# panthuncia/BasicRenderer

Measured on AMD Instinct MI355X. Metric: shaded Mpixels/s @4K (vis-buffer+resolve), higher is better.
Workload: dtype f32; 1 GPU; bistro-class procedural frame, 3840x2160, 1 directional + 256 point lights, 22669824 instanced tris, 2017 instances (2614016 in 150 meshes), LOD DAGs from the library's cluster-LOD builder, relief slope 1.5; pixels_per_gpu=8294400, visible_clusters_rank0=10118, occlusion_culling=True, visible_clusters_phase2_rank0=0, meshlets_tested_rank0=26713, partition=single GPU, frames_in_flight=3

## Files before the change

basicrenderer_amd/capi.py:

```python
import ctypes as C
import os

_HERE = os.path.dirname(os.path.abspath(__file__))
LIB_DIR = os.path.join(_HERE, "lib")

u32, u64, f32, vp = C.c_uint32, C.c_uint64, C.c_float, C.c_void_p


class SceneParams(C.Structure):
    _fields_ = [("preset", u32), ("seed", u32), ("width", u32), ("height", u32), ("numPointLights", u32),
                ("withDirectionalLight", u32), ("lodLevels", u32), ("sizeScale", f32), ("skinnedFraction1024", u32),
                ("materialFeatures", u32), ("cameraStep", u32), ("lodBuilder", u32), ("spotLightEvery", u32), ("detail", f32), ("uniqueTriangleBudget", u32), ("reliefSlope", f32)]


class MeshInput(C.Structure):
    _fields_ = [("positions", vp), ("normals", vp), ("uvs", vp), ("colors", vp), ("vertexCount", C.c_size_t), ("indices", vp), ("indexCount", C.c_size_t),
                ("material", u32), ("reserved", u32 * 3)]


class InstanceInput(C.Structure):
    _fields_ = [("mesh", u32), ("reverseWinding", u32), ("model", (f32 * 4) * 4)]


class ViewInput(C.Structure):
# ... 39 lines not shown
        ("perMesh", vp), ("perMeshCount", u32),
        ("perMeshInstance", vp), ("perMeshInstanceCount", u32),
        ("clodOffsets", vp),
        ("meshMetadata", vp), ("meshMetadataCount", u32),
        ("lodNodes", vp), ("lodNodeCount", u32),
        ("lodGroups", vp), ("lodGroupCount", u32),
        ("lodSegments", vp), ("lodSegmentCount", u32),
        ("groupPageMap", vp), ("groupPageMapCount", u32),
        ("materials", vp), ("materialCount", u32),
        ("openpbrMaterials", vp), ("openpbrMaterialCount", u32),
        ("lights", vp), ("lightCount", u32),
        ("activeLightIndices", vp),
        ("cameras", vp), ("cameraCount", u32),
        ("cullingCameras", vp),
        ("viewRasterInfo", vp),
        ("perFrame", vp),
        ("activeDraws", vp), ("activeDrawCount", u32),
        ("skinningMatrices", vp), ("skinningMatrixCount", u32),
        ("lutOpaqueDielectricEnergyComplement", vp),
        ("lutOpaqueDielectricAvgEnergyComplement", vp),
        ("lutIdealMetalEnergyComplement", vp),
        ("lutIdealMetalAvgEnergyComplement", vp),
        ("lutFuzzLTC", vp),
        ("textures", vp), ("textureCount", u32),
        ("samplers", vp), ("samplerCount", u32),
        ("srgbToLinear", vp),
    ]


class Config(C.Structure):
    _fields_ = [("structSize", u32), ("width", u32), ("height", u32), ("maxVisibleClusters", u32),
                ("maxTraversalRecords", u32), ("enableOcclusionCulling", u32), ("enableClusteredLighting", u32),
                ("enablePunctualLights", u32), ("lightClusterSize", u32 * 3), ("phase2ExpansionFactor", u32),
                ("collectPassStatistics", u32), ("maxBvhLevels", u32), ("bandY0", u32), ("bandY1", u32),
                ("keepUniformLayerPlanes", u32), ("stripeRows", u32), ("stripeCount", u32), ("stripeIndex", u32), ("fullHeight", u32), ("dynamicBand", u32), ("reserved", u32 * 2)]


class ResourceDesc(C.Structure):
    _fields_ = [("id", u32), ("name", C.c_char_p), ("bytes", u64), ("usage", u32), ("width", u32), ("height", u32),
                ("bytesPerPixel", u32), ("tileW", u32), ("tileH", u32)]


class ResourceBinding(C.Structure):
    _fields_ = [("id", u32), ("ptr", vp), ("bytes", u64)]


class FrameUpdate(C.Structure):
    _fields_ = [("mainCameraHost", vp), ("perFrameHost", vp), ("frameIndex", u32)]


class Counters(C.Structure):
    _fields_ = [(n, u32) for n in ("instancesTested instancesVisible nodesVisited bucketRecords meshletsTested "
                                   "visibleClusters visibleClustersPhase2 droppedRecords droppedClusters "
                                   "lightPagesUsed replayNodes replayMeshlets").split()] + [("reserved", u32 * 6)]


class ComposeConfig(C.Structure):
    _fields_ = [("structSize", u32), ("width", u32), ("bandY0", u32), ("bandY1", u32), ("bytesPerPixel", u32), ("transport", u32), ("depth", u32),
                ("rank", u32), ("nRanks", u32), ("device", C.c_int32), ("path", u32), ("waitTimeoutMs", u32), ("frameHeight", u32), ("reserved", u32 * 3)]


COMPOSE_EXPORTS = ["brmi_compose_unique_id", "brmi_compose_create", "brmi_compose_staging_bytes", "brmi_compose_output_bytes", "brmi_compose_bind",
                   "brmi_compose_submit", "brmi_compose_finish", "brmi_compose_destroy", "brmi_compose_last_error",
                   "brmi_compose_alloc_shared", "brmi_compose_export", "brmi_compose_import", "brmi_compose_last_wait_status", "brmi_compose_submit_rows", "brmi_compose_wait_source", "brmi_compose_set_bounds", "brmi_compose_balance_rows"]
COMPOSE_HANDLE_BYTES = 160
_compose_lib = None


def compose_lib():
    global _compose_lib
    if _compose_lib is None:
        import torch
        path = os.path.join(LIB_DIR, "libbrmi_compose.so")
        if not os.path.exists(path):
            raise RuntimeError(f"{path} is missing: run `make compose` (or __graft_entry__.build())")
        try:
            C.CDLL(os.path.join(os.path.dirname(torch.__file__), "lib", "librccl.so"), mode=C.RTLD_GLOBAL)
        except OSError:
            pass
        lib = C.CDLL(path)
        lib.brmi_compose_unique_id.argtypes = [vp]
        lib.brmi_compose_create.argtypes = [C.POINTER(ComposeConfig), C.c_char_p, C.POINTER(vp)]
        lib.brmi_compose_staging_bytes.argtypes = [vp]
        lib.brmi_compose_staging_bytes.restype = u64
        lib.brmi_compose_output_bytes.argtypes = [vp]
        lib.brmi_compose_output_bytes.restype = u64
        lib.brmi_compose_bind.argtypes = [vp, vp, u64, vp, u64]
        lib.brmi_compose_submit.argtypes = [vp, vp, vp]
        lib.brmi_compose_finish.argtypes = [vp, vp, C.POINTER(vp)]
        lib.brmi_compose_destroy.argtypes = [vp]
        lib.brmi_compose_alloc_shared.argtypes = [vp]
        lib.brmi_compose_export.argtypes = [vp, C.c_char_p]
        lib.brmi_compose_import.argtypes = [vp, C.c_char_p, u32]
        lib.brmi_compose_last_wait_status.argtypes = [vp]
        lib.brmi_compose_submit_rows.argtypes = [vp, vp, u32, u32, vp]
        lib.brmi_compose_wait_source.argtypes = [vp, vp, vp]; lib.brmi_compose_wait_source.restype = C.c_int
        lib.brmi_compose_destroy.restype = None
        lib.brmi_compose_last_error.argtypes = [vp]
        lib.brmi_compose_last_error.restype = C.c_char_p
        _compose_lib = lib
    return _compose_lib


DECLARE_CB = C.CFUNCTYPE(None, vp, C.POINTER(ResourceDesc))

RES_NAMES = ["VISIBILITY", "LINEAR_DEPTH", "GBUF_NORMALS", "GBUF_ALBEDO", "GBUF_COAT", "GBUF_EMISSIVE", "GBUF_FUZZ",
             "GBUF_METALLIC_ROUGHNESS", "GBUF_MOTION_VECTORS", "HDR_COLOR", "VISIBLE_CLUSTERS", "LIGHT_CLUSTERS",
             "LIGHT_PAGES", "HZB", "WORKSPACE"]
RES = {n: i for i, n in enumerate(RES_NAMES)}
STAGE_NAMES = ["clear", "cull", "raster", "depth_copy", "hzb", "cull2", "raster2", "gbuffer", "light_cluster", "shade"]

_scene_lib = None
_brmi_lib = None


def scene_lib():
    global _scene_lib
    if _scene_lib is None:
        path = os.path.join(LIB_DIR, "libbrmi_scene.so")
        if not os.path.exists(path):
            raise RuntimeError(f"{path} is missing: run `make scene` (or __graft_entry__.build())")
        lib = C.CDLL(path)
        lib.brmi_scene_create.restype = vp
        lib.brmi_scene_create.argtypes = [C.POINTER(SceneParams)]
        lib.brmi_scene_create_with_dag_builder.restype = vp
        lib.brmi_scene_create_with_dag_builder.argtypes = [C.POINTER(SceneParams), vp, vp, vp]
        lib.brmi_scene_create_from_meshes.restype = vp
        lib.brmi_scene_create_from_meshes.argtypes = [C.POINTER(SceneParams), C.POINTER(MeshInput), u32, C.POINTER(InstanceInput), u32, C.POINTER(ViewInput), vp, vp, vp]
        lib.brmi_lod_build.argtypes = [vp, vp, C.c_size_t, vp, C.c_size_t, vp, C.POINTER(Dag)]
        lib.brmi_lod_release.argtypes = [vp, C.POINTER(Dag)]
        lib.brmi_lod_release.restype = None
        lib.brmi_scene_create_from_cache.restype = vp
        lib.brmi_scene_create_from_cache.argtypes = [C.POINTER(SceneParams), C.c_char_p]
        lib.brmi_scene_export_cache.argtypes = [vp, C.c_char_p]
        lib.brmi_scene_destroy.argtypes = [vp]
        lib.brmi_scene_array.argtypes = [vp, u32, C.POINTER(vp), C.POINTER(u64), C.POINTER(u32)]
        lib.brmi_scene_slab_count.argtypes = [vp]
        lib.brmi_scene_slab_count.restype = u32
        lib.brmi_scene_slab.argtypes = [vp, u32, C.POINTER(vp), C.POINTER(u64)]
        lib.brmi_scene_get_stats.argtypes = [vp, C.POINTER(SceneStats)]
        lib.brmi_scene_camera_at.argtypes = [C.POINTER(SceneParams), C.c_double, C.c_double, vp, vp]
        _scene_lib = lib
    return _scene_lib


BRMI_EXPORTS = ["brmi_abi_version", "brmi_default_config", "brmi_create", "brmi_declare", "brmi_set_scene", "brmi_setup", "brmi_set_band",
                "brmi_update", "brmi_execute", "brmi_execute_split", "brmi_destroy", "brmi_last_error", "brmi_clear_visibility", "brmi_cull",
                "brmi_raster", "brmi_depth_copy", "brmi_build_hzb", "brmi_invalidate_hzb", "brmi_set_history_source", "brmi_gbuffer", "brmi_light_clustering",
                "brmi_shade", "brmi_set_shade_slabs", "brmi_read_counters", "brmi_stage_times", "brmi_set_timed_stages", "brmi_algorithmic_bytes", "brmi_algorithmic_bytes_launched", "brmi_debug_arith", "brmi_debug_arith_in_range", "brmi_debug_read_bin_records", "brmi_debug_wide_triangles", "brmi_debug_lean_clusters", "brmi_debug_read_lean_queue", "brmi_debug_read_held"]


def brmi_lib():
    global _brmi_lib
    if _brmi_lib is None:
        import torch
        path = os.environ.get("BRMI_LIB_PATH") or os.path.join(LIB_DIR, "libbrmi.so")
        if not os.path.exists(path):
            raise RuntimeError(f"{path} is missing: the HIP extension must be built (make hip); there is no CPU fallback")
        lib = C.CDLL(path)
        lib.brmi_abi_version.restype = u32
        lib.brmi_default_config.argtypes = [C.POINTER(Config), u32, u32]
        lib.brmi_default_config.restype = None
        lib.brmi_create.argtypes = [C.POINTER(Config), C.POINTER(vp)]
        lib.brmi_declare.argtypes = [vp, DECLARE_CB, vp]
        lib.brmi_set_scene.argtypes = [vp, C.POINTER(SceneBuffers)]
        lib.brmi_setup.argtypes = [vp, C.POINTER(ResourceBinding), u32, vp]
        lib.brmi_update.argtypes = [vp, C.POINTER(FrameUpdate), vp]
        lib.brmi_execute.argtypes = [vp, vp]
        lib.brmi_execute_split.argtypes = [vp, vp, vp]
        lib.brmi_destroy.argtypes = [vp]
        lib.brmi_destroy.restype = None
        lib.brmi_last_error.argtypes = [vp]
        lib.brmi_last_error.restype = C.c_char_p
        for n in ("brmi_clear_visibility", "brmi_depth_copy", "brmi_build_hzb", "brmi_gbuffer", "brmi_light_clustering", "brmi_shade"):
            getattr(lib, n).argtypes = [vp, vp]
        lib.brmi_invalidate_hzb.argtypes = [vp]
        lib.brmi_set_history_source.argtypes = [vp, vp]
        lib.brmi_set_shade_slabs.argtypes = [vp, u32, vp, vp]
        lib.brmi_cull.argtypes = [vp, u32, vp]
        lib.brmi_raster.argtypes = [vp, u32, vp]
        lib.brmi_read_counters.argtypes = [vp, C.POINTER(Counters), vp]
        lib.brmi_stage_times.argtypes = [vp, C.POINTER(f32)]
        lib.brmi_set_timed_stages.argtypes = [vp, u32]
        lib.brmi_algorithmic_bytes.argtypes = [vp, C.POINTER(u64), C.POINTER(u64)]
        lib.brmi_algorithmic_bytes_launched.argtypes = [vp, C.POINTER(u64), C.POINTER(u64)]
        lib.brmi_debug_arith.argtypes = [vp, vp, vp, vp, vp, u32, vp]
        lib.brmi_debug_arith_in_range.argtypes = [vp, vp, vp, vp, u32, vp]
        _brmi_lib = lib
    return _brmi_lib
```

basicrenderer_amd/csrc/brmi_api.hip:

```cpp
#include <hip/hip_runtime.h>

#include <algorithm>
#include <cmath>
#include <cstdarg>
#include <cstdio>
#include <cstdlib>
#include <cstring>

#include "brmi_device.h"
#include "brmi_internal.h"

namespace brmi {

__global__ void k_debug_arith(const float* a, const float* b, float* outDiv, float* outSqrt, uint32_t* outHalf, uint32_t n) {
    const uint32_t i = blockIdx.x * blockDim.x + threadIdx.x;
    if (i >= n) return;
    outDiv[i] = a[i] / b[i];
    outSqrt[i] = sqrtf(fabsf(a[i]));
    outHalf[i] = f32_to_f16_bits(a[i]);
}

__global__ void k_debug_arith_in_range(const float* a, float* outRcp, float* outSqrt, float* outNorm, uint32_t n) {
    const uint32_t i = blockIdx.x * blockDim.x + threadIdx.x;
    if (i >= n) return;
// ... 14 lines not shown
static uint64_t align_up(uint64_t v, uint64_t a) { return (v + a - 1) / a * a; }

static const char* kResNames[BRMI_RES_COUNT] = {
    "Builtin::PrimaryCamera::VisibilityTexture", "Builtin::PrimaryCamera::LinearDepthMap", "Builtin::GBuffer::Normals", "Builtin::GBuffer::Albedo",
    "Builtin::GBuffer::Coat", "Builtin::GBuffer::Emissive", "Builtin::GBuffer::Fuzz", "Builtin::GBuffer::MetallicRoughness", "Builtin::GBuffer::MotionVectors",
    "Builtin::Color::HDRColorTarget", "Builtin::CLod::VisibleClusters", "Builtin::Light::ClusterBuffer", "Builtin::Light::PagesBuffer",
    "Builtin::PrimaryCamera::LinearDepthMap(mips)", "brmi::Workspace"};
static const uint32_t kResBpp[BRMI_RES_COUNT] = {8, 4, 16, 4, 8, 8, 8, 4, 4, 8, 0, 0, 0, 4, 0};

static void compute_sizes(brmi_pass* p) {
    const brmi_config& c = p->cfg;
    p->tilesX = (c.width + 7) / 8; p->tilesY = (c.height + 7) / 8;
    p->paddedPixels = (uint64_t)p->tilesX * p->tilesY * 64;
    p->bandY0 = c.bandY0; p->bandY1 = (c.bandY1 == 0 || c.bandY1 > c.height) ? c.height : c.bandY1;
    if (p->bandY0 >= p->bandY1) p->bandY0 = 0;
    p->stripes = c.stripeCount > 1u ? StripeMap{c.stripeRows, c.stripeCount, c.stripeIndex, c.fullHeight} : StripeMap{0u, 0u, 0u, c.height};
    { const uint32_t t0 = p->bandY0 / 8, t1 = (p->bandY1 + 7) / 8; p->bandFirstPixel = (uint64_t)t0 * p->tilesX * 64; p->bandPixelCount = (uint64_t)(t1 - t0) * p->tilesX * 64; }
    p->numLightClusters = c.lightClusterSize[0] * c.lightClusterSize[1] * c.lightClusterSize[2];
    p->lightPagePool = p->numLightClusters * BRMI_LIGHT_PAGES_PER_CLUSTER;
    if (const long v = tuning("light_page_pool", 0)) p->lightPagePool = (uint32_t)std::max(1l, v);
    for (int i = 0; i < BRMI_RES_COUNT; i++) p->resNeed[i] = 0;
    for (int i = BRMI_RES_VISIBILITY; i <= BRMI_RES_HDR_COLOR; i++) p->resNeed[i] = p->paddedPixels * kResBpp[i];
    p->resNeed[BRMI_RES_VISIBLE_CLUSTERS] = (uint64_t)c.maxVisibleClusters * 16;
    p->resNeed[BRMI_RES_LIGHT_CLUSTERS] = (uint64_t)p->numLightClusters * sizeof(brmi_light_cluster);
    p->resNeed[BRMI_RES_LIGHT_PAGES] = (uint64_t)p->lightPagePool * sizeof(brmi_light_page);
    p->hzbMipOffsets.clear(); p->hzbMipW.clear(); p->hzbMipH.clear();
    uint64_t hzbFloats = 0;
    if (c.enableOcclusionCulling) {
        uint32_t w = 1, h = 1; while (w < c.width) w <<= 1; while (h < c.height) h <<= 1;
        for (uint32_t mip = 0;; mip++) {
            p->hzbMipOffsets.push_back(hzbFloats); p->hzbMipW.push_back(w); p->hzbMipH.push_back(h);
            if (mip > 0) hzbFloats += (uint64_t)w * h;
            if (w == 1 && h == 1) break;
            w = std::max(1u, w >> 1); h = std::max(1u, h >> 1);
        }
    }
    p->hzbMipCount = (uint32_t)p->hzbMipOffsets.size();
    p->resNeed[BRMI_RES_HZB] = std::max<uint64_t>(16, hzbFloats * 4);
    Workspace& w = p->ws; uint64_t off = 0;
    auto take = [&](uint64_t bytes) { uint64_t o = off; off = align_up(off + bytes, 256); return o; };
    w.counters = take((uint64_t)(CNT_WORDS + 64) * 4);
    w.bitmask1 = take((uint64_t)p->totalWords * 4);
    w.bitmask2 = take((uint64_t)p->totalWords * 4);
    w.blockDirty = take((uint64_t)2 * (p->scanBlocks + 1));
    w.chainDirty = take(4ull + (uint64_t)((c.width + 31u) / 32u) * ((c.height + 31u) / 32u));
    w.frameClearBytes = off - w.counters;
    w.frontierA = take((uint64_t)c.maxTraversalRecords * sizeof(NodeRecord));
    w.frontierB = take((uint64_t)c.maxTraversalRecords * sizeof(NodeRecord));
    w.buckets = take((uint64_t)c.maxTraversalRecords * sizeof(BucketRecord));
    w.tempVisible = take((uint64_t)c.maxVisibleClusters * sizeof(TempVisible));
    w.wordPrefix = take((uint64_t)p->totalWords * 4);
    w.blockSums = take((uint64_t)(p->scanBlocks + 1) * 4);
    w.scanAgg = take(65 * 8);
    w.instanceBitBase = take((uint64_t)std::max<size_t>(1, p->hostInstanceBitBase.size()) * 4);
    w.segPrefix = take((uint64_t)std::max<size_t>(1, p->hostSegPrefix.size()) * 4);
    w.meshLevelWidth = take((uint64_t)std::max<size_t>(1, p->hostMeshLevelWidth.size()) * 4);
    w.flatNodes = take((uint64_t)std::max<size_t>(1, p->hostFlatNodes.size()) * sizeof(FlatNode));
    w.flatLeaves = take((uint64_t)std::max<size_t>(1, p->hostFlatLeaves.size()) * sizeof(FlatLeaf));
    w.instanceWalk = take((uint64_t)std::max<size_t>(1, p->hostInstanceWalk.size()) * sizeof(InstanceWalk));
    w.planes = take((uint64_t)2 * c.lightClusterSize[2] * 4);
    w.replayNodes = take(c.enableOcclusionCulling ? (uint64_t)c.maxTraversalRecords * sizeof(NodeRecord) : 16);
    w.replayBuckets = take(c.enableOcclusionCulling ? (uint64_t)c.maxTraversalRecords * sizeof(BucketRecord) : 16);
    w.lightVS = take((uint64_t)std::max(1u, p->scene.lightCount) * 16);
    w.lightMeta = take((uint64_t)std::max(1u, p->scene.lightCount) * 4);
    w.clusterPages = take((uint64_t)p->numLightClusters * 4);
    w.clusterHits = take((uint64_t)p->numLightClusters * 4);
    w.pageTotal = take(16);
    w.lightHitMasks = take((uint64_t)p->numLightClusters * ((std::max(1u, p->scene.lightCount) + 63u) / 64u) * 8);
    p->binsX = (c.width + 255) / 256; p->binsY = (c.height + 15) / 16;
    w.binCounts = take((uint64_t)p->binsX * p->binsY * 4 * BRMI_BIN_COUNT_STRIDE);
    w.binRecords = take((uint64_t)p->binsX * p->binsY * p->binCapacity * 64);
    w.binOverflow = take((uint64_t)CNT_STRIPE_COUNT * p->binOverflowPerStripe * 64);
    p->binItemCapacity = p->binsX * p->binsY * std::max(1u, (p->binCapacity + 31u) / 32u > 256u ? 256u : (p->binCapacity + 31u) / 32u);
    p->binItemCapacity = std::min<uint32_t>(p->binItemCapacity, 1u << 22);
    p->binScratchTiles = (uint32_t)std::max(0l, tuning("bin_scratch_tiles", p->binScratchTiles));
    w.binPlan = take((uint64_t)(16 + 3 * p->binsX * p->binsY) * 4);
    w.binItems = take((uint64_t)p->binItemCapacity * 4);
    w.binScratch = take((uint64_t)std::max(1u, p->binScratchTiles) * 4096 * 8);
    w.clusterSetup = take((uint64_t)c.maxVisibleClusters * sizeof(ClusterSetup));
    p->resolveCapacity = (uint32_t)std::min<uint64_t>((uint64_t)c.maxVisibleClusters, 1ull << 20) * BRMI_MESHLET_MAX_TRIS;
    if (const long v = tuning("resolve_capacity", 0)) p->resolveCapacity = (uint32_t)std::max(1l, v);
    w.resolveVerts = take((uint64_t)p->resolveCapacity * sizeof(ResolveVertex));
    w.resolveTris = take((uint64_t)p->resolveCapacity * sizeof(ResolveTriangle));
    w.shadeTables = take(((uint64_t)2 * c.width + 2 * c.height + 64) * 4);
    w.matWords = take((uint64_t)std::max(1u, p->scene.materialCount) * sizeof(MaterialWords));
    w.layerUniform = take(sizeof(LayerUniform));
    w.frameConst = take(4 * 64);
    w.frameSnapshot = take(sizeof(FrameSnapshot));
    w.matConst = take((uint64_t)std::max(1u, p->scene.openpbrMaterialCount) * sizeof(MatConst));
    w.objConst = take((uint64_t)std::max(1u, p->scene.perObjectCount) * OBJ_CONST_FLOATS * 4);
    p->deferredStripeCapacity = (uint32_t)((((c.dynamicBand ? p->paddedPixels : p->bandPixelCount) / 4096 + CNT_STRIPE_COUNT) / CNT_STRIPE_COUNT) * 4096);
    w.deferredPixels = take((uint64_t)3 * CNT_STRIPE_COUNT * p->deferredStripeCapacity * 4);
    w.lutF = take((uint64_t)(32768 + 1024 + 1024 + 32 + 256) * 4);
    w.shadeRows = take((uint64_t)std::max(1u, p->scene.openpbrMaterialCount) * 256 * 512);
    w.shadeAvgs = take((uint64_t)std::max(1u, p->scene.openpbrMaterialCount) * 256 * 8);
    w.ggxQuads = take(256 * 48);
    w.shadeLights = take((uint64_t)std::max(1u, p->scene.lightCount) * 64);
    w.clusterList = take((uint64_t)p->numLightClusters * 8);
    w.listEntries = take((uint64_t)p->lightPagePool * BRMI_LIGHTS_PER_PAGE * 4 + 256);
    w.listRecords = take((uint64_t)p->lightPagePool * BRMI_LIGHTS_PER_PAGE * 64 + 4096);
    const bool uvs = p->sceneHasTextures || p->sceneHasAlphaTest || p->sceneHasVertexColors;
    w.clusterUv = take(uvs ? (uint64_t)c.maxVisibleClusters * 32 : 16);
    w.resolveColors = take(p->sceneHasVertexColors ? (uint64_t)p->resolveCapacity * 4 : 16);
    w.resolveUVs = take(p->sceneHasTextures ? (uint64_t)p->resolveCapacity * 8 * p->sceneUvSets : 16);
    w.binAlpha = take(p->sceneHasAlphaTest ? (uint64_t)p->binsX * p->binsY * p->binCapacity * 48 : 16);
    w.overflowAlpha = take(p->sceneHasAlphaTest ? (uint64_t)CNT_STRIPE_COUNT * p->binOverflowPerStripe * 48 : 16);
// ... 44 lines not shown
    std::memset(cfg, 0, sizeof(*cfg));
    cfg->structSize = sizeof(brmi_config);
    cfg->width = width; cfg->height = height;
    cfg->maxVisibleClusters = 1u << 22;
    cfg->maxTraversalRecords = 1u << 22;
    cfg->enableOcclusionCulling = 0;
    cfg->enableClusteredLighting = 1;
    cfg->enablePunctualLights = 1;
    cfg->lightClusterSize[0] = 12; cfg->lightClusterSize[1] = 12; cfg->lightClusterSize[2] = 24;
    cfg->phase2ExpansionFactor = 2;
    cfg->collectPassStatistics = 0;
    cfg->maxBvhLevels = 64;
    cfg->keepUniformLayerPlanes = 0;
}

}
namespace brmi {
static bool tuning_lookup(const char* key, long* out) {
    const char* e = std::getenv("BRMI_TUNING");
    if (!e) return false;
    const size_t n = std::strlen(key);
    for (const char* q = e; *q; ) {
        while (*q == ',' || *q == ' ') q++;
        const char* end = std::strchr(q, ',');
        const size_t len = end ? (size_t)(end - q) : std::strlen(q);
        if (len > n && std::strncmp(q, key, n) == 0 && q[n] == '=') { *out = std::strtol(q + n + 1, nullptr, 0); return true; }
        q += len;
    }
    return false;
}
long tuning(const char* key, long def) { long v; return tuning_lookup(key, &v) ? v : def; }
}
extern "C" {

int brmi_create(const brmi_config* cfg, brmi_pass** out) {
    if (!cfg || !out || cfg->structSize != sizeof(brmi_config) || cfg->width == 0 || cfg->height == 0) return BRMI_ERR_INVALID;
    if (cfg->maxVisibleClusters == 0 || cfg->maxVisibleClusters > (1u << 25) - 1u || cfg->maxTraversalRecords == 0) return BRMI_ERR_INVALID;
    if (cfg->lightClusterSize[0] == 0 || cfg->lightClusterSize[1] == 0 || cfg->lightClusterSize[2] == 0) return BRMI_ERR_INVALID;
    if (cfg->lightClusterSize[2] > 62u) return BRMI_ERR_INVALID;
    if ((uint64_t)((cfg->width + 255u) / 256u) * ((cfg->height + 15u) / 16u) > 65535ull) return BRMI_ERR_INVALID;
    if (cfg->stripeCount > 1u) {
        if (cfg->stripeRows == 0u || cfg->stripeRows % 16u || cfg->stripeIndex >= cfg->stripeCount || cfg->bandY0 != 0u || (cfg->bandY1 != 0u && cfg->bandY1 != cfg->height)) return BRMI_ERR_INVALID;
        if (cfg->fullHeight == 0u || cfg->fullHeight % (cfg->stripeRows * cfg->stripeCount) || cfg->height != cfg->fullHeight / cfg->stripeCount) return BRMI_ERR_INVALID;
        if (cfg->dynamicBand) return BRMI_ERR_INVALID;
    }
    if (cfg->dynamicBand && (cfg->bandY0 % 8u || (cfg->bandY1 % 8u && cfg->bandY1 < cfg->height))) return BRMI_ERR_INVALID;
    brmi_pass* p = new brmi_pass();
    p->cfg = *cfg;
    p->totalWords = 1; p->scanBlocks = 1;
    p->forceLevelKernels = tuning("cull_level_kernels", 0) != 0;
    p->packedFlat = tuning("flat_packed", 1) != 0;
    p->flatLevelsMinDraws = (uint32_t)std::max(0l, tuning("flat_levels_min_draws", p->flatLevelsMinDraws));
    p->phase2DirectMax = (uint32_t)std::max(0l, tuning("phase2_direct_max", p->phase2DirectMax));
    p->resolveInlineMode = (int)tuning("resolve_inline", -1);
    p->wideCapacity = (uint32_t)std::min(1l << 20, std::max(0l, tuning("wide_capacity", p->wideCapacity)));
    p->wideMinTriangles = (uint32_t)std::max(0l, tuning("wide_min_triangles", p->wideMinTriangles));
    p->leanMinClusters = (uint32_t)std::max(0l, tuning("lean_min_clusters", p->leanMinClusters));
    if (p->leanMinClusters > cfg->maxVisibleClusters) p->leanMinClusters = 0u;
    p->leanMaxGeneralPct = (uint32_t)std::max(0l, std::min(100l, tuning("lean_max_general_pct", p->leanMaxGeneralPct)));
    p->leanGrid = (uint32_t)std::max(64l, tuning("lean_grid", p->leanGrid));
    p->leanQueue = (uint32_t)std::max(64l, std::min(1l << 24, tuning("lean_queue", p->leanQueue))) & ~63u;
    p->leanWideEntries = (uint32_t)std::max(1l, tuning("lean_wide_entries", p->leanWideEntries));
    p->leanEmitGrid = (uint32_t)std::max(64l, std::min(65536l, tuning("lean_emit_grid", p->leanEmitGrid))) & ~63u;
    p->wideEntries = (uint32_t)std::max(1l, tuning("wide_entries", p->wideEntries));
    p->binMinSlice = (uint32_t)std::max(32l, tuning("bin_min_slice", p->binMinSlice));
    p->binSharedSlice = (uint32_t)std::max(32l, tuning("bin_shared_slice", p->binSharedSlice));
    p->binGrid = (uint32_t)std::min(65535l, std::max(1l, tuning("bin_grid", p->binGrid)));
    p->binOverflowPerStripe = (uint32_t)std::max(0l, tuning("bin_overflow", p->binOverflowPerStripe));
    p->binCapacity = (uint32_t)std::min(65536l, std::max(1l, tuning("bin_capacity", p->binCapacity)));
    if (const long v = tuning("big_tri_area", 0)) p->bigTriArea = p->bigTriAreaAlpha = p->bigTriAreaDense = (int)std::max(1l, v);
    compute_sizes(p);
    *out = p;
    return BRMI_OK;
}

void brmi_destroy(brmi_pass* p) {
    if (!p) return;
    if (p->eventsCreated) for (int i = 0; i < BRMI_STAGE_COUNT; i++) for (uint32_t k = 0; k < brmi_pass::kEventRing; k++) { (void)hipEventDestroy(p->evStart[i][k]); (void)hipEventDestroy(p->evStop[i][k]); }
    (void)brmi_set_history_source(p, nullptr);
    for (brmi_pass* user : p->historyUsers) user->history = nullptr;
    if (p->chainReady) (void)hipEventDestroy(p->chainReady);
    if (p->geometryDone) (void)hipEventDestroy(p->geometryDone);
    if (p->cullDone) (void)hipEventDestroy(p->cullDone);
    if (p->frameDone) (void)hipEventDestroy(p->frameDone);
    if (p->phase2FeedbackHost) (void)hipHostFree(p->phase2FeedbackHost);
    delete p;
}

const char* brmi_last_error(const brmi_pass* p) { return p ? p->err.c_str() : "null pass"; }

int brmi_set_scene(brmi_pass* p, const brmi_scene_buffers* scene) {
    if (!p || !scene) return BRMI_ERR_INVALID;
    p->scene = *scene; p->haveScene = false; p->setupDone = false;
    const brmi_scene_buffers& sc = p->scene;
    if (!sc.slabs || !sc.perObject || !sc.perMesh || !sc.perMeshInstance || !sc.clodOffsets || !sc.meshMetadata || !sc.lodNodes || !sc.lodGroups ||
        !sc.lodSegments || !sc.groupPageMap || !sc.materials || !sc.openpbrMaterials || !sc.cameras || !sc.cullingCameras || !sc.viewRasterInfo || !sc.perFrame ||
        !sc.normalMatrices || (sc.activeDrawCount && !sc.activeDraws) || (sc.lightCount && (!sc.lights || !sc.activeLightIndices)))
        return fail(p, BRMI_ERR_INVALID, "brmi_set_scene: a required scene buffer is null");
    if (!sc.lutOpaqueDielectricEnergyComplement || !sc.lutOpaqueDielectricAvgEnergyComplement || !sc.lutIdealMetalEnergyComplement || !sc.lutIdealMetalAvgEnergyComplement || !sc.lutFuzzLTC)
        return fail(p, BRMI_ERR_INVALID, "brmi_set_scene: OpenPBR lookup tables must be provided");
    std::vector<brmi_clod_mesh_metadata> md; std::vector<brmi_mesh_instance_clod_offsets> offs; std::vector<brmi_lod_node> nodes; std::vector<brmi_lod_segment> segs;
    int rc;
    if ((rc = read_back(p, md, sc.meshMetadata, sc.meshMetadataCount))) return rc;
    if ((rc = read_back(p, offs, sc.clodOffsets, sc.perMeshInstanceCount))) return rc;
    if ((rc = read_back(p, nodes, sc.lodNodes, sc.lodNodeCount))) return rc;
    if ((rc = read_back(p, segs, sc.lodSegments, sc.lodSegmentCount))) return rc;
// ... 486 lines not shown
        BRMI_HIP(p, hipEventRecord(p->chainReady, static_cast<hipStream_t>(stream)));
        p->chainRecorded = true; p->chainStream = stream;
    }
    if (split) {
        if ((rc = launch_resolve_setup(p, static_cast<hipStream_t>(stream), 2u))) return rc;
        p->resolveSetupDone = true;
        if (!p->geometryDone) BRMI_HIP(p, hipEventCreateWithFlags(&p->geometryDone, hipEventDisableTiming));
        if (!p->frameDone) BRMI_HIP(p, hipEventCreateWithFlags(&p->frameDone, hipEventDisableTiming));
        BRMI_HIP(p, hipEventRecord(p->geometryDone, static_cast<hipStream_t>(stream)));
        BRMI_HIP(p, hipStreamWaitEvent(static_cast<hipStream_t>(shadeStream), p->geometryDone, 0));
        stream = shadeStream;
    }
    const bool lightsDone = p->lightGridDone;
    p->lightGridDone = false;
    p->depthFinal = p->cfg.enableOcclusionCulling != 0;
    p->shadeSharesChip = split;
    rc = brmi_gbuffer(p, stream);
    p->shadeSharesChip = false;
    p->depthFinal = false;
    if (rc) return rc;
    if (!lightsDone && (rc = brmi_light_clustering(p, stream))) return rc;
    p->shadeSharesChip = split;
    rc = brmi_shade(p, stream);
    p->shadeSharesChip = false;
    if (rc) return rc;
    if (split) { BRMI_HIP(p, hipEventRecord(p->frameDone, static_cast<hipStream_t>(stream))); p->frameDoneRecorded = true; }
    p->splitFrame = false;
    return BRMI_OK;
}

int brmi_read_counters(brmi_pass* p, brmi_counters* out, brmi_stream stream) {
    if (!p || !out) return BRMI_ERR_INVALID;
    if (!p->setupDone) return brmi::fail(p, BRMI_ERR_STATE, "brmi_read_counters: setup not done");
    hipStream_t s = static_cast<hipStream_t>(stream);
    uint32_t c[CNT_WORDS];
    BRMI_HIP(p, hipMemcpyAsync(c, p->counters(), sizeof(c), hipMemcpyDeviceToHost, s));
    BRMI_HIP(p, hipStreamSynchronize(s));
    std::memset(out, 0, sizeof(*out));
    out->instancesTested = c[CNT_INSTANCES_TESTED]; out->instancesVisible = c[CNT_INSTANCES_VISIBLE];
    out->nodesVisited = c[CNT_NODES_VISITED];
    uint32_t overflowQueued = 0;
    for (uint32_t st = 0; st < CNT_STRIPE_COUNT; st++) {
        const uint32_t* sp = c + CNT_STRIPES + st * CNT_STRIPE_WORDS;
        out->instancesTested += sp[0]; out->instancesVisible += sp[1]; out->nodesVisited += sp[2];
        overflowQueued += sp[STRIPE_OVERFLOW];
    } out->bucketRecords = c[CNT_BUCKETS]; out->meshletsTested = c[CNT_MESHLETS_TESTED];
    for (uint32_t st = 0; st < CNT_STRIPE_COUNT; st++) out->meshletsTested += c[CNT_STRIPES + st * CNT_STRIPE_WORDS + STRIPE_MESHLETS_TESTED];
    out->visibleClusters = c[CNT_VISIBLE]; out->visibleClustersPhase2 = c[CNT_VISIBLE2];
    out->droppedRecords = c[CNT_DROPPED_RECORDS]; out->droppedClusters = c[CNT_DROPPED_CLUSTERS]; out->lightPagesUsed = c[CNT_LIGHT_PAGES];
    out->reserved[0] = c[CNT_SUM_VERTS_LO]; out->reserved[2] = c[CNT_SUM_VERTS_HI];
    out->reserved[1] = std::min(c[CNT_HELD1], p->cfg.maxVisibleClusters); out->reserved[3] = std::min(c[CNT_LATE1], p->cfg.maxVisibleClusters);
    out->reserved[4] = c[CNT_RASTER_CLUSTERS]; out->reserved[5] = c[CNT_BIN_OVERFLOW] + overflowQueued;
    out->replayNodes = c[CNT_REPLAY_NODES]; out->replayMeshlets = c[CNT_REPLAY_MESHLETS];
    return BRMI_OK;
}

int brmi_set_timed_stages(brmi_pass* p, uint32_t stageMask) {
    if (!p) return BRMI_ERR_INVALID;
    p->timedStages = stageMask;
    return BRMI_OK;
}

int brmi_stage_times(brmi_pass* p, float* ms) {
    if (!p || !ms) return BRMI_ERR_INVALID;
    if (!p->eventsCreated) return brmi::fail(p, BRMI_ERR_STATE, "brmi_stage_times: collectPassStatistics is off");
    for (int i = 0; i < BRMI_STAGE_COUNT; i++) {
        ms[i] = 0.0f;
        const uint32_t perFrame = (i == BRMI_STAGE_HZB && p->executesSinceTimes != 0u && p->evCount[i] == 2u * p->executesSinceTimes) ? 2u : 1u;
        uint32_t n = std::min(p->evCount[i], brmi_pass::kEventRing);
        n -= n % perFrame;
        if (n == 0) continue;
        double sum = 0.0;
        for (uint32_t k = 0; k < n; k++) {
            const uint32_t slot = (p->evCount[i] - 1 - k) % brmi_pass::kEventRing;
            float t = 0.0f;
            BRMI_HIP(p, hipEventSynchronize(p->evStop[i][slot]));
            BRMI_HIP(p, hipEventElapsedTime(&t, p->evStart[i][slot], p->evStop[i][slot]));
            sum += t;
        }
        ms[i] = (float)(sum / (n / perFrame));
        p->evCount[i] = 0;
    }
    p->executesSinceTimes = 0;
    return BRMI_OK;
}

int brmi_algorithmic_bytes(brmi_pass* p, uint64_t* perStage, uint64_t* total) {
    if (!p || !perStage || !total) return BRMI_ERR_INVALID;
    BRMI_HIP(p, hipDeviceSynchronize());
    brmi_counters c; int rc = brmi_read_counters(p, &c, nullptr); if (rc) return rc;
    const uint64_t P = (uint64_t)p->cfg.width * (p->bandY1 - p->bandY0);
    uint64_t sumV = c.reserved[0], sumT = c.reserved[2], nClusters = c.reserved[4];
    if (c.reserved[1] != 0u) {
        uint32_t vt[2];
        BRMI_HIP(p, hipMemcpy(vt, p->counters() + CNT_DRAWN_VT, 8, hipMemcpyDeviceToHost));
        sumV = vt[0]; sumT = vt[1]; nClusters -= c.reserved[1] - c.reserved[3];
    }
    for (int i = 0; i < BRMI_STAGE_COUNT; i++) perStage[i] = 0;
    perStage[BRMI_STAGE_CLEAR] = 8 * P;
    perStage[BRMI_STAGE_CULL] = 64ull * c.meshletsTested + 16ull * (c.visibleClusters + c.visibleClustersPhase2) + 64ull * c.nodesVisited;
    perStage[BRMI_STAGE_RASTER] = 8 * P + 144ull * nClusters + 12ull * sumV + 3ull * sumT;
    if (p->cfg.enableOcclusionCulling) {
        perStage[BRMI_STAGE_DEPTH_COPY] = 12 * P;
        perStage[BRMI_STAGE_HZB] = 2 * (4 * P + 4 * P / 3);
    }
    perStage[BRMI_STAGE_GBUFFER] = (8 + 52 + 4) * P;
// ... 1 lines not shown
    *total = 0; for (int i = 0; i < BRMI_STAGE_COUNT; i++) *total += perStage[i];
    return BRMI_OK;
}

int brmi_algorithmic_bytes_launched(brmi_pass* p, uint64_t* perStage, uint64_t* total) {
    if (int rc = brmi_algorithmic_bytes(p, perStage, total)) return rc;
    if (!p->sceneHasCoat && !p->sceneHasFuzz) {
        const uint64_t P = (uint64_t)p->cfg.width * (p->bandY1 - p->bandY0);
        *total -= perStage[BRMI_STAGE_SHADE]; perStage[BRMI_STAGE_SHADE] = 44ull * P; *total += perStage[BRMI_STAGE_SHADE];
    }
    return BRMI_OK;
}

int brmi_debug_read_held(brmi_pass* p, uint32_t* held, uint32_t heldCapacity, uint32_t* heldCount, uint32_t* late, uint32_t lateCapacity, uint32_t* lateCount) {
    if (!p || !heldCount || !lateCount || !p->setupDone) return BRMI_ERR_INVALID;
    BRMI_HIP(p, hipDeviceSynchronize());
    uint32_t nh = 0, nl = 0;
    BRMI_HIP(p, hipMemcpy(&nh, p->counters() + CNT_HELD1, 4, hipMemcpyDeviceToHost));
    BRMI_HIP(p, hipMemcpy(&nl, p->counters() + CNT_LATE1, 4, hipMemcpyDeviceToHost));
    if (!p->holdEnabled) nh = nl = 0;
    nh = std::min(nh, p->cfg.maxVisibleClusters); nl = std::min(nl, p->cfg.maxVisibleClusters);
    *heldCount = nh; *lateCount = nl;
    if (held && nh) {
        std::vector<HeldRecord> rec(std::min(nh, heldCapacity));
        if (!rec.empty()) BRMI_HIP(p, hipMemcpy(rec.data(), p->wsPtr<HeldRecord>(p->ws.heldRecords), rec.size() * sizeof(HeldRecord), hipMemcpyDeviceToHost));
        for (size_t i = 0; i < rec.size(); i++) held[i] = rec[i].clusterIndex;
    }
    if (late && nl && lateCapacity) BRMI_HIP(p, hipMemcpy(late, p->wsPtr<uint32_t>(p->ws.lateList), (size_t)std::min(nl, lateCapacity) * 4, hipMemcpyDeviceToHost));
    return BRMI_OK;
}

int brmi_debug_wide_triangles(brmi_pass* p, uint32_t out[3]) {
    if (!p || !out || !p->setupDone) return BRMI_ERR_INVALID;
    BRMI_HIP(p, hipDeviceSynchronize());
    uint32_t c[3] = {0u, 0u, 0u};
    BRMI_HIP(p, hipMemcpy(&c[0], p->counters() + CNT_WIDE1, 4, hipMemcpyDeviceToHost));
    BRMI_HIP(p, hipMemcpy(&c[1], p->counters() + CNT_WIDE1B, 4, hipMemcpyDeviceToHost));
    BRMI_HIP(p, hipMemcpy(&c[2], p->counters() + CNT_WIDE2, 4, hipMemcpyDeviceToHost));
    out[0] = c[0]; out[1] = c[1]; out[2] = c[2];
    return BRMI_OK;
}

int brmi_debug_lean_clusters(brmi_pass* p, uint32_t out[4]) {
    if (!p || !out || !p->setupDone) return BRMI_ERR_INVALID;
    BRMI_HIP(p, hipDeviceSynchronize());
    uint32_t c = 0u, heads[64 * 32];
    BRMI_HIP(p, hipMemcpy(&c, p->counters() + CNT_GENERAL1, 4, hipMemcpyDeviceToHost));
    BRMI_HIP(p, hipMemcpy(heads, p->counters() + CNT_BIG1, sizeof(heads), hipMemcpyDeviceToHost));
    out[0] = p->leanLastLaunch ? 1u : 0u; out[1] = c; out[2] = out[3] = 0u;
    for (uint32_t s = 0; s < 64u; s++) { out[2] += heads[s * 32u]; out[3] += heads[s * 32u + 1u]; }
    return BRMI_OK;
}

int brmi_debug_read_lean_queue(brmi_pass* p, uint32_t stripe, uint32_t* runs, uint32_t maxRuns, void* entries, uint32_t maxEntries, uint32_t counts[2]) {
    if (!p || !counts || !p->setupDone || stripe >= 64u || p->leanMinClusters == 0u) return BRMI_ERR_INVALID;
    BRMI_HIP(p, hipDeviceSynchronize());
    uint32_t head[2];
    BRMI_HIP(p, hipMemcpy(head, p->counters() + CNT_BIG1 + stripe * 32u, 8, hipMemcpyDeviceToHost));
    const uint32_t cap = p->leanQueue / 64u;
    counts[0] = std::min(head[0], cap); counts[1] = std::min(head[1], cap);
    if (runs) BRMI_HIP(p, hipMemcpy(runs, p->wsPtr<uint8_t>(p->ws.bigRuns) + (size_t)stripe * cap * 8u, (size_t)std::min(maxRuns, counts[1]) * 8u, hipMemcpyDeviceToHost));
    if (entries) BRMI_HIP(p, hipMemcpy(entries, p->wsPtr<uint8_t>(p->ws.bigQueue) + (size_t)stripe * cap * 96u, (size_t)std::min(maxEntries, counts[0]) * 96u, hipMemcpyDeviceToHost));
    return BRMI_OK;
}

int brmi_debug_read_bin_records(brmi_pass* p, void* dst, uint64_t bytes) {
    if (!p || !dst || !p->setupDone) return BRMI_ERR_INVALID;
    BRMI_HIP(p, hipDeviceSynchronize());
    if ((bytes >> 62) & 1ull) { bytes &= ~(1ull << 62); BRMI_HIP(p, hipMemset(p->wsPtr<uint8_t>(p->ws.binRecords), 0, bytes)); return BRMI_OK; }
    BRMI_HIP(p, hipMemcpy(dst, p->wsPtr<uint8_t>(p->ws.binRecords), bytes, hipMemcpyDeviceToHost));
    return BRMI_OK;
}

int brmi_debug_arith(const float* a, const float* b, float* outDiv, float* outSqrt, uint32_t* outHalfBits, uint32_t n, brmi_stream stream) {
    if (!a || !b || !outDiv || !outSqrt || !outHalfBits) return BRMI_ERR_INVALID;
    if (n == 0) return BRMI_OK;
    hipLaunchKernelGGL(k_debug_arith, dim3((n + 255) / 256), dim3(256), 0, static_cast<hipStream_t>(stream), a, b, outDiv, outSqrt, outHalfBits, n);
    return hipGetLastError() == hipSuccess ? BRMI_OK : BRMI_ERR_HIP;
}

int brmi_debug_arith_in_range(const float* a, float* outRcp, float* outSqrt, float* outRsqrt, uint32_t n, brmi_stream stream) {
    if (!a || !outRcp || !outSqrt || !outRsqrt) return BRMI_ERR_INVALID;
    if (n == 0) return BRMI_OK;
    hipLaunchKernelGGL(k_debug_arith_in_range, dim3((n + 255) / 256), dim3(256), 0, static_cast<hipStream_t>(stream), a, outRcp, outSqrt, outRsqrt, n);
    return hipGetLastError() == hipSuccess ? BRMI_OK : BRMI_ERR_HIP;
}

}
```

basicrenderer_amd/csrc/brmi_cull.hip:

```cpp
#include <type_traits>
#include "brmi_device.h"
#include "brmi_internal.h"
#include "brmi_lightgrid.h"
#include "brmi_texture.h"

namespace brmi {

struct CullArgs {
    brmi_scene_buffers sc;
    uint32_t* counters;
    const uint32_t* instanceBitBase;
    const uint32_t* segPrefix;
    uint32_t recordCapacity, visibleCapacity, factor, phase;
    uint32_t occlusion;
    uint32_t frontier0Counter, bucketCounter;
    NodeRecord* replayNodes; BucketRecord* replayBuckets;
    HzbDesc hzb;
    uint32_t bandActive; float bandTop[3], bandBottom[3];
    const float4* bandPlanes;
    StripeMap stripes;
    const uint32_t* meshLevelWidth; uint32_t levelKernelsWidthLo;
    const FlatNode* flatNodes; const FlatLeaf* flatLeaves; const InstanceWalk* instanceWalk;
    uint32_t* feedback;
    uint32_t wideFlat;
// ... 243 lines not shown
#pragma unroll
            for (int o = 32; o > 0; o >>= 1) waveMax = max(waveMax, (uint32_t)__shfl_xor((int)waveMax, o));
            for (uint32_t k = 0; k < waveMax; k++) {
                const bool emit = k < nChunks;
                const uint32_t slot = wave_append(&a.counters[a.bucketCounter], emit);
                if (emit) {
                    if (slot < a.recordCapacity) {
                        const uint32_t first = segFirst + k * a.factor;
                        const uint32_t cnt = min(a.factor, segCount - k * a.factor);
                        BucketRecord b;
                        b.instanceIndex = instIndex; b.groupIdPacked = (replay ? 0x80000000u : 0u) | (ownerGroup & 0x7FFFFFFFu);
                        b.meshletIndexAndCount = (cnt << 16) | (first & 0xFFFFu);
                        b.pageSlabDescriptorIndex = slabDesc; b.pageSlabByteOffset = slabOff;
                        b.firstBit = firstBit + k * a.factor; b.pad0 = 0; b.pad1 = 0;
                        buckets[slot] = b;
                    } else atomicAdd(&a.counters[CNT_DROPPED_RECORDS], 1u);
                }
            }
        }
        {
            uint32_t waveMax = isInternal ? childCount : 0u;
#pragma unroll
            for (int o = 32; o > 0; o >>= 1) waveMax = max(waveMax, (uint32_t)__shfl_xor((int)waveMax, o));
            for (uint32_t k = 0; k < waveMax; k++) {
                bool emit = false;
                uint32_t childId = 0;
                if (isInternal && k < childCount) {
                    childId = childBase + k;
                    const brmi_lod_node* ch = sc.lodNodes + (lodNodesBase + childId);
                    const f3 cc = skinned ? instC : f3{ch->cullCenterAndRadius[0], ch->cullCenterAndRadius[1], ch->cullCenterAndRadius[2]};
                    const float cr = skinned ? instR : ch->cullCenterAndRadius[3];
                    const f3 ccVS = to_view_space(cc, model, view);
                    emit = replay || !sphere_culled(a, cam, ccVS, cr * scale);
                    if (emit && ch->isLeaf == BRMI_NODE_INTERNAL) {
                        const f3 wc = xyz(mul_point(f3{ch->lodCenterAndRadius[0], ch->lodCenterAndRadius[1], ch->lodCenterAndRadius[2]}, model));
                        const float e = projected_error(wc, ch->lodCenterAndRadius[3] * scale, ch->maxQuadricError, scale, camPos, zNear, ortho);
                        if (e < threshold) emit = false;
                    }
                }
                const uint32_t slot = wave_append(nextCount, emit);
                if (emit) {
                    if (slot < a.recordCapacity) frontierOut[slot] = NodeRecord{instIndex, (replay ? 0x80000000u : 0u) | (1u << 30) | (childId & 0x3FFFFFFFu)};
                    else atomicAdd(&a.counters[CNT_DROPPED_RECORDS], 1u);
                }
            }
        }
    }
}

#ifndef BRMI_HIER_STAGE_WIDE
#define BRMI_HIER_STAGE_WIDE 128
#endif
constexpr uint32_t HIER_CAP_MAX = 1024;
struct NoSide {};
struct SideJobs { ulonglong2* vis2; uint64_t n2; uint32_t walkBlocks, clearBlocks; ClusterArgs lc; };
template <bool REPLAY, uint32_t HIER_CAP, uint32_t HIER_STAGE, bool SIDE = false>
__global__ void __launch_bounds__(64) k_cull_hierarchy(CullArgs a, BucketRecord* buckets, const uint32_t* meshLevelWidth, uint32_t widthLo, uint32_t widthHi, uint32_t spillAbove, NodeRecord* spillOut,
                                                    typename std::conditional<SIDE, SideJobs, NoSide>::type sj) {
    uint32_t walkBlocks = gridDim.x;
    if constexpr (SIDE) {
        walkBlocks = sj.walkBlocks;
        if (blockIdx.x >= sj.walkBlocks + sj.clearBlocks) { lc_count_wave(sj.lc, blockIdx.x - sj.walkBlocks - sj.clearBlocks, threadIdx.x); return; }
        if (blockIdx.x >= sj.walkBlocks) {
            const uint64_t stride = (uint64_t)sj.clearBlocks * 64u;
            for (uint64_t i = (uint64_t)(blockIdx.x - sj.walkBlocks) * 64u + threadIdx.x; i < sj.n2; i += stride) sj.vis2[i] = make_ulonglong2(BRMI_VIS_EMPTY, BRMI_VIS_EMPTY);
            return;
        }
    }
    __shared__ uint32_t frontier[2][HIER_CAP];
    __shared__ uint32_t counts[2];
    __shared__ uint32_t childOff[65], childFirst[64];
    __shared__ BucketRecord stage[HIER_STAGE];
    const brmi_scene_buffers& sc = a.sc;
    const uint32_t lane = threadIdx.x;
    const uint32_t viewId = sc.perFrame->mainCameraIndex;
    const brmi_camera* cam = sc.cameras + viewId;
    const brmi_culling_camera* lodCam = sc.cullingCameras + viewId;
    const bool ortho = cam->isOrtho != 0;
    const f3 camPos{lodCam->positionWorldSpace[0], lodCam->positionWorldSpace[1], lodCam->positionWorldSpace[2]};
    const float zNear = lodCam->zNear, threshold = lodCam->errorOverDistanceThreshold;
    const m4 view = load_m4(&cam->view[0][0]);
    const uint32_t seeds = REPLAY ? min(a.counters[CNT_REPLAY_NODES], a.recordCapacity) : sc.activeDrawCount;
    uint32_t nTested = 0, nVisible = 0, nNodes = 0;
    uint32_t staged = 0;
    auto flush = [&]() {
        if (staged == 0u) return;
        uint32_t baseSlot = 0;
        if (lane == 0) baseSlot = atomicAdd(&a.counters[a.bucketCounter], staged);
        baseSlot = (uint32_t)__shfl((int)baseSlot, 0);
        __syncthreads();
        for (uint32_t k = lane; k < staged; k += 64u) {
            if (baseSlot + k < a.recordCapacity) buckets[baseSlot + k] = stage[k];
            else atomicAdd(&a.counters[CNT_DROPPED_RECORDS], 1u);
        }
        __syncthreads();
        staged = 0u;
    };
    uint32_t firstSeed = blockIdx.x, seedStride = walkBlocks;
    if (!REPLAY && a.packedFlat) {
        const uint32_t packedWaves = (seeds + 7u) >> 3;
        if (blockIdx.x < packedWaves) {
            const uint32_t g8 = lane & ~7u, j = lane & 7u;
            const uint32_t seed = blockIdx.x * 8u + (lane >> 3);
            const bool haveSeed = seed < seeds;
            const uint32_t instIndex = haveSeed ? sc.activeDraws[seed] : 0u;
            brmi_per_mesh_instance inst{}; InstanceWalk iw{0u, 0u, 0u, 0u};
            if (haveSeed) { inst = sc.perMeshInstance[instIndex]; iw = a.instanceWalk[instIndex]; }
            const bool small = haveSeed && iw.flatCount >= 1u && iw.flatCount <= 8u;
            const brmi_per_object* obj = sc.perObject + (small ? inst.perObjectBufferIndex : 0u);
            const bool mine = small && j < iw.flatCount;
            FlatNode fn{}; FlatLeaf fl{};
            if (mine) { fn = a.flatNodes[iw.flatBase + j]; fl = a.flatLeaves[iw.flatBase + j]; }
            m4 model = load_m4(&obj->model[0][0]);
            m4 prevModel = model;
            if (a.occlusion && mine && ((fn.info & 1u))) prevModel = load_m4(&obj->prevModel[0][0]);
            const float scale = max_axis_scale(model);
            const f3 instC{inst.boundingSphere[0], inst.boundingSphere[1], inst.boundingSphere[2]}; const float instR = inst.boundingSphere[3];
            bool instVisible = false;
            {
                const f3 c = to_view_space(instC, model, view);
                const float r = instR * scale;
                const bool bad = isnan(c.x) || isnan(c.y) || isnan(c.z) || isinf(c.x) || isinf(c.y) || isinf(c.z) || isnan(r) || isinf(r);
                instVisible = small && !bad && !sphere_culled(a, cam, c, r);
            }
            nTested += (uint32_t)__popcll(__ballot(small && j == 0u)); nVisible += (uint32_t)__popcll(__ballot(instVisible && j == 0u));
            const bool skinned = iw.skinned != 0u;
            const bool internal = (fn.info & 1u);
            const f3 cullC = skinned ? instC : f3{fn.cull[0], fn.cull[1], fn.cull[2]};
            const float cullR = skinned ? instR : fn.cull[3];
            const f3 cVS = to_view_space(cullC, model, view);
            const float rW = cullR * scale;
            const bool inFrustum = mine && instVisible && !sphere_culled(a, cam, cVS, rW);
            bool pre = inFrustum, expand = false, hidden = false, leafOk = false;
            uint32_t slabDesc = 0, slabOff = 0;
            if (inFrustum && internal) {
                const f3 lc = xyz(mul_point(f3{fn.lod[0], fn.lod[1], fn.lod[2]}, model));
                const float e = projected_error(lc, fn.lod[3] * scale, fn.maxQuadricError, scale, camPos, zNear, ortho);
                pre = e >= threshold;
                if (pre) { hidden = a.occlusion && occlusion_test_prev(a, cam, cullC, cullR, prevModel); expand = !hidden; }
            } else if (inFrustum) {
                const f3 gc = xyz(mul_point(f3{fl.group[0], fl.group[1], fl.group[2]}, model));
                const float eod = projected_error(gc, fl.group[3] * scale, fn.maxQuadricError, scale, camPos, zNear, ortho);
                bool ok = eod >= threshold;
                if (ok && ((fn.info >> 1) & 1u)) {
                    const f3 cc = xyz(mul_point(f3{fl.child[0], fl.child[1], fl.child[2]}, model));
                    const float ce = projected_error(cc, fl.child[3] * scale, fl.childParentError, scale, camPos, zNear, ortho);
                    if (!(ce < threshold)) ok = false;
                }
                if (ok && ((fn.info >> 2) & 1u)) {
                    const brmi_group_page_map_entry pe = sc.groupPageMap[fn.pageMapIndex];
                    slabDesc = pe.slabDescriptorIndex; slabOff = pe.slabByteOffset;
                    leafOk = slabDesc != 0u;
                }
            }
            const uint64_t expandM = __ballot(expand);
            const uint32_t parentLane = g8 | ((fn.info >> 8) & 7u);
            uint64_t reached = __ballot(mine && instVisible && j == 0u);
            for (;;) {
                const bool r = mine && instVisible && (j == 0u || (pre && ((reached >> parentLane) & 1ull) && ((expandM >> parentLane) & 1ull)));
                const uint64_t next = __ballot(r);
                if (next == reached) break;
                reached = next;
            }
            const bool here = (reached >> lane) & 1ull;
            nNodes += here ? 1u : 0u;
            const bool replayIt = a.occlusion && here && hidden;
            const uint64_t replayM = __ballot(replayIt);
            const bool emitLeaf = here && leafOk;
            const uint32_t segFirst = fn.segFirstCount & 0xFFFFu, segCount = fn.segFirstCount >> 16;
            const uint32_t nChunks = emitLeaf ? (segCount + a.factor - 1u) / a.factor : 0u;
            uint32_t incl = nChunks;
#pragma unroll
            for (int o = 1; o < 64; o <<= 1) { const uint32_t v = (uint32_t)__shfl_up((int)incl, o); if (lane >= (uint32_t)o) incl += v; }
            const uint32_t nBuckets = (uint32_t)__shfl((int)incl, 63), nReplay = (uint32_t)__popcll(replayM);
            uint32_t replayBase = 0, bucketBase = 0;
            if (lane == 0) {
                if (nReplay != 0u) replayBase = atomicAdd(&a.counters[CNT_REPLAY_NODES], nReplay);
                if (nBuckets != 0u) bucketBase = atomicAdd(&a.counters[a.bucketCounter], nBuckets);
            }
            replayBase = (uint32_t)__shfl((int)replayBase, 0); bucketBase = (uint32_t)__shfl((int)bucketBase, 0);
            if (replayIt) {
                const uint32_t slot = replayBase + (uint32_t)__popcll(replayM & ((1ull << lane) - 1ull));
                if (slot < a.recordCapacity) a.replayNodes[slot] = NodeRecord{instIndex, 0x80000000u | (1u << 30) | (fn.nodeId & 0x3FFFFFFFu)};
                else atomicAdd(&a.counters[CNT_DROPPED_RECORDS], 1u);
            }
            for (uint32_t k = 0; k < nChunks; k++) {
                const uint32_t slot = bucketBase + (incl - nChunks) + k;
                if (slot >= a.recordCapacity) { atomicAdd(&a.counters[CNT_DROPPED_RECORDS], 1u); continue; }
                BucketRecord b;
                b.instanceIndex = instIndex; b.groupIdPacked = fn.ownerGroup & 0x7FFFFFFFu;
                b.meshletIndexAndCount = (min(a.factor, segCount - k * a.factor) << 16) | ((segFirst + k * a.factor) & 0xFFFFu);
                b.pageSlabDescriptorIndex = slabDesc; b.pageSlabByteOffset = slabOff;
                b.firstBit = iw.bitBase + fn.firstBitRel + k * a.factor; b.pad0 = 0; b.pad1 = 0;
                buckets[slot] = b;
            }
            firstSeed = seeds;
        } else { firstSeed = blockIdx.x - packedWaves; seedStride = walkBlocks - packedWaves; }
    }
    for (uint32_t seed = firstSeed; seed < seeds; seed += seedStride) {
        uint32_t instIndex, startNode;
        if (REPLAY) { const NodeRecord rec = a.replayNodes[seed]; instIndex = rec.instanceIndex; startNode = rec.nodeIdPacked & 0x3FFFFFFFu; }
        else instIndex = sc.activeDraws[seed];
        const brmi_per_mesh_instance inst = sc.perMeshInstance[instIndex];
        if (!REPLAY) {
            const InstanceWalk iw = a.instanceWalk[instIndex];
            if (a.packedFlat && iw.flatCount >= 1u && iw.flatCount <= 8u) continue;
            if (iw.flatCount > 256u && a.wideFlat) continue;
            if (iw.flatCount != 0u && iw.flatCount <= 256u) {
                constexpr uint32_t FLAT_CHUNKS = 4;
                const uint32_t chunks = (iw.flatCount + 63u) >> 6;
                const brmi_per_object* obj = sc.perObject + inst.perObjectBufferIndex;
                uint32_t nodeIdA[FLAT_CHUNKS] = {}, parentA[FLAT_CHUNKS] = {}, ownerGroupA[FLAT_CHUNKS] = {}, segFirstCountA[FLAT_CHUNKS] = {}, firstBitRelA[FLAT_CHUNKS] = {};
                const m4 model = load_m4(&obj->model[0][0]);
                const m4 prevModel = a.occlusion ? load_m4(&obj->prevModel[0][0]) : model;
                const float scale = max_axis_scale(model);
                const f3 instC{inst.boundingSphere[0], inst.boundingSphere[1], inst.boundingSphere[2]}; const float instR = inst.boundingSphere[3];
                {
                    const f3 c = to_view_space(instC, model, view);
                    const float r = instR * scale;
                    const bool bad = isnan(c.x) || isnan(c.y) || isnan(c.z) || isinf(c.x) || isinf(c.y) || isinf(c.z) || isnan(r) || isinf(r);
                    nTested++;
                    if (bad || sphere_culled(a, cam, c, r)) continue;
                    nVisible++;
                }
                const bool skinned = iw.skinned != 0u;
                uint64_t preM[FLAT_CHUNKS] = {}, expandM[FLAT_CHUNKS] = {}, hiddenM[FLAT_CHUNKS] = {}, leafM[FLAT_CHUNKS] = {}, reached[FLAT_CHUNKS] = {};
                uint32_t slabDescA[FLAT_CHUNKS] = {}, slabOffA[FLAT_CHUNKS] = {};
#pragma unroll
                for (uint32_t c = 0; c < FLAT_CHUNKS; c++) if (c < chunks) {
                    const bool mine = c * 64u + lane < iw.flatCount;
                    FlatNode fn{}; FlatLeaf fl{};
                    if (mine) { fn = a.flatNodes[iw.flatBase + c * 64u + lane]; fl = a.flatLeaves[iw.flatBase + c * 64u + lane]; }
                    nodeIdA[c] = fn.nodeId; parentA[c] = fn.info >> 8; ownerGroupA[c] = fn.ownerGroup; segFirstCountA[c] = fn.segFirstCount; firstBitRelA[c] = fn.firstBitRel;
                    const bool internal = (fn.info & 1u);
                    const f3 cullC = skinned ? instC : f3{fn.cull[0], fn.cull[1], fn.cull[2]};
                    const float cullR = skinned ? instR : fn.cull[3];
                    const f3 cVS = to_view_space(cullC, model, view);
                    const float rW = cullR * scale;
                    const bool inFrustum = mine && !sphere_culled(a, cam, cVS, rW);
                    bool pre = inFrustum, expand = false, hidden = false, leafOk = false;
                    if (inFrustum && internal) {
                        const f3 lc = xyz(mul_point(f3{fn.lod[0], fn.lod[1], fn.lod[2]}, model));
                        const float e = projected_error(lc, fn.lod[3] * scale, fn.maxQuadricError, scale, camPos, zNear, ortho);
                        pre = e >= threshold;
                        if (pre) { hidden = a.occlusion && occlusion_test_prev(a, cam, cullC, cullR, prevModel); expand = !hidden; }
                    } else if (inFrustum) {
                        const f3 gc = xyz(mul_point(f3{fl.group[0], fl.group[1], fl.group[2]}, model));
                        const float eod = projected_error(gc, fl.group[3] * scale, fn.maxQuadricError, scale, camPos, zNear, ortho);
                        bool ok = eod >= threshold;
                        if (ok && ((fn.info >> 1) & 1u)) {
// ... 40 lines not shown
                    for (int o = 1; o < 64; o <<= 1) { const uint32_t v = (uint32_t)__shfl_up((int)incl, o); if (lane >= (uint32_t)o) incl += v; }
                    bucketRank[c] = nBuckets + incl - chunksOfLeaf[c];
                    nBuckets += (uint32_t)__shfl((int)incl, 63);
                }
                uint32_t replayBase = 0, bucketBase = 0;
                if (lane == 0) {
                    if (nReplay != 0u) replayBase = atomicAdd(&a.counters[CNT_REPLAY_NODES], nReplay);
                    if (nBuckets != 0u) bucketBase = atomicAdd(&a.counters[a.bucketCounter], nBuckets);
                }
                replayBase = (uint32_t)__shfl((int)replayBase, 0); bucketBase = (uint32_t)__shfl((int)bucketBase, 0);
#pragma unroll
                for (uint32_t c = 0; c < FLAT_CHUNKS; c++) if (c < chunks) {
                    if (a.occlusion && ((reached[c] & hiddenM[c]) >> lane) & 1ull) {
                        const uint32_t slot = replayBase + replayRank[c];
                        if (slot < a.recordCapacity) a.replayNodes[slot] = NodeRecord{instIndex, 0x80000000u | (1u << 30) | (nodeIdA[c] & 0x3FFFFFFFu)};
                        else atomicAdd(&a.counters[CNT_DROPPED_RECORDS], 1u);
                    }
                    const uint32_t segFirst = segFirstCountA[c] & 0xFFFFu, segCount = segFirstCountA[c] >> 16;
                    for (uint32_t k = 0; k < chunksOfLeaf[c]; k++) {
                        const uint32_t slot = bucketBase + bucketRank[c] + k;
                        if (slot >= a.recordCapacity) { atomicAdd(&a.counters[CNT_DROPPED_RECORDS], 1u); continue; }
                        BucketRecord b;
                        b.instanceIndex = instIndex; b.groupIdPacked = ownerGroupA[c] & 0x7FFFFFFFu;
                        b.meshletIndexAndCount = (min(a.factor, segCount - k * a.factor) << 16) | ((segFirst + k * a.factor) & 0xFFFFu);
                        b.pageSlabDescriptorIndex = slabDescA[c]; b.pageSlabByteOffset = slabOffA[c];
                        b.firstBit = iw.bitBase + firstBitRelA[c] + k * a.factor; b.pad0 = 0; b.pad1 = 0;
                        buckets[slot] = b;
                    }
                }
                continue;
            }
        }
        const uint32_t mdIndex = sc.clodOffsets[instIndex].clodMeshMetadataIndex;
        const uint32_t width = meshLevelWidth[mdIndex];
        if (width < widthLo || width > widthHi) continue;
        const bool spill = width > spillAbove;
        const brmi_clod_mesh_metadata md = sc.meshMetadata[mdIndex];
        const brmi_per_object* obj = sc.perObject + inst.perObjectBufferIndex;
        const m4 model = load_m4(&obj->model[0][0]);
        const float scale = max_axis_scale(model);
        const f3 instC{inst.boundingSphere[0], inst.boundingSphere[1], inst.boundingSphere[2]}; const float instR = inst.boundingSphere[3];
        if (!REPLAY) {
            const f3 c = to_view_space(instC, model, view);
            const float r = instR * scale;
            const bool bad = isnan(c.x) || isnan(c.y) || isnan(c.z) || isinf(c.x) || isinf(c.y) || isinf(c.z) || isnan(r) || isinf(r);
            const bool visible = !bad && !sphere_culled(a, cam, c, r);
            nTested++;
            if (!visible) continue;
            nVisible++;
            startNode = md.rootNode;
        }
        const bool skinned = (sc.perMesh[inst.perMeshBufferIndex].vertexFlags & BRMI_VERTEX_SKINNED) != 0;
        const uint32_t bitBase = a.instanceBitBase[instIndex];
        __syncthreads();
        if (lane == 0) { frontier[0][0] = startNode; counts[0] = 1u; counts[1] = 0u; }
        __syncthreads();
        for (uint32_t level = 0; level < 64u; level++) {
            const uint32_t cur = level & 1u, nxt = cur ^ 1u;
            const uint32_t n = min(counts[cur], HIER_CAP);
            if (n == 0u) break;
            if (spill && n > HIER_CAP / BRMI_BVH_MAX_CHILDREN) {
                uint32_t baseSlot = 0;
                if (lane == 0) baseSlot = atomicAdd(&a.counters[CNT_FRONTIER0], n);
                baseSlot = (uint32_t)__shfl((int)baseSlot, 0);
                for (uint32_t k = lane; k < n; k += 64u) {
                    if (baseSlot + k < a.recordCapacity) spillOut[baseSlot + k] = NodeRecord{instIndex, (REPLAY ? 0x80000000u : 0u) | (1u << 30) | (frontier[cur][k] & 0x3FFFFFFFu)};
                    else atomicAdd(&a.counters[CNT_DROPPED_RECORDS], 1u);
                }
                break;
            }
            for (uint32_t base = 0; base < n; base += 64u) {
                const bool have = base + lane < n;
                bool isInternal = false, emitLeaf = false, occluded = false;
                uint32_t nodeId = 0, childBase = 0, childCount = 0, segFirst = 0, segCount = 0, ownerGroup = 0, slabDesc = 0, slabOff = 0, firstBit = 0;
                if (have) {
                    nodeId = frontier[cur][base + lane];
                    nNodes++;
                    const brmi_lod_node node = sc.lodNodes[md.lodNodesBase + nodeId];
                    const f3 cullC = skinned ? instC : f3{node.cullCenterAndRadius[0], node.cullCenterAndRadius[1], node.cullCenterAndRadius[2]};
                    const float cullR = skinned ? instR : node.cullCenterAndRadius[3];
                    const f3 cVS = to_view_space(cullC, model, view);
                    const float rW = cullR * scale;
                    const bool culled = !REPLAY && sphere_culled(a, cam, cVS, rW);
                    if (!culled) {
                        if (node.isLeaf != BRMI_NODE_INTERNAL) {
                            const brmi_lod_group* g = sc.lodGroups + (md.groupsBase + node.ownerGroupId);
                            const f3 gc = xyz(mul_point(f3{g->centerAndRadius[0], g->centerAndRadius[1], g->centerAndRadius[2]}, model));
                            const float gr = g->centerAndRadius[3] * scale;
                            const float eod = projected_error(gc, gr, node.maxQuadricError, scale, camPos, zNear, ortho);
                            bool ok = eod >= threshold;
                            if (ok && refined_child_suppresses(sc, md.groupsBase, node.countMinusOne - 1u, node.countMinusOne != 0u, model, scale, camPos, zNear, threshold, ortho)) ok = false;
                            if (ok) {
                                const brmi_lod_segment seg = sc.lodSegments[md.segmentsBase + node.indexOrOffset];
                                const brmi_group_page_map_entry pe = sc.groupPageMap[md.pageMapBase + seg.pageIndex];
                                if (seg.meshletCount != 0u && pe.slabDescriptorIndex != 0u) {
                                    emitLeaf = true;
                                    segFirst = seg.firstMeshletInPage; segCount = seg.meshletCount; ownerGroup = node.ownerGroupId;
                                    slabDesc = pe.slabDescriptorIndex; slabOff = pe.slabByteOffset;
                                    firstBit = bitBase + a.segPrefix[md.segmentsBase + node.indexOrOffset];
                                }
                            }
                        } else {
                            const f3 lc = xyz(mul_point(f3{node.lodCenterAndRadius[0], node.lodCenterAndRadius[1], node.lodCenterAndRadius[2]}, model));
                            const float lr = node.lodCenterAndRadius[3] * scale;
                            const float nodeEod = projected_error(lc, lr, node.maxQuadricError, scale, camPos, zNear, ortho);
                            if (nodeEod >= threshold) {
                                if (a.occlusion && occlusion_test(a, cam, REPLAY, cullC, cullR, cVS, rW, obj)) occluded = !REPLAY;
                                else { isInternal = true; childBase = node.indexOrOffset; childCount = min(node.countMinusOne + 1u, BRMI_BVH_MAX_CHILDREN); }
                            }
// ... 7 lines not shown
                        else atomicAdd(&a.counters[CNT_DROPPED_RECORDS], 1u);
                    }
                }
                {
                    const uint32_t nChunks = emitLeaf ? (segCount + a.factor - 1u) / a.factor : 0u;
                    uint32_t incl = nChunks;
#pragma unroll
                    for (int o = 1; o < 64; o <<= 1) { const uint32_t v = (uint32_t)__shfl_up((int)incl, o); if (lane >= (uint32_t)o) incl += v; }
                    const uint32_t total = (uint32_t)__shfl((int)incl, 63);
                    if (total != 0u) {
                        if (staged + total > HIER_STAGE) flush();
                        if (total <= HIER_STAGE) {
                            const uint32_t baseSlot = staged + (incl - nChunks);
                            for (uint32_t k = 0; k < nChunks; k++) {
                                const uint32_t first = segFirst + k * a.factor;
                                const uint32_t cnt = min(a.factor, segCount - k * a.factor);
                                BucketRecord b;
                                b.instanceIndex = instIndex; b.groupIdPacked = (REPLAY ? 0x80000000u : 0u) | (ownerGroup & 0x7FFFFFFFu);
                                b.meshletIndexAndCount = (cnt << 16) | (first & 0xFFFFu);
                                b.pageSlabDescriptorIndex = slabDesc; b.pageSlabByteOffset = slabOff;
                                b.firstBit = firstBit + k * a.factor; b.pad0 = 0; b.pad1 = 0;
                                stage[baseSlot + k] = b;
                            }
                            staged += total;
                        } else {
                            uint32_t baseSlot = 0;
                            if (lane == 0) baseSlot = atomicAdd(&a.counters[a.bucketCounter], total);
                            baseSlot = (uint32_t)__shfl((int)baseSlot, 0) + (incl - nChunks);
                            for (uint32_t k = 0; k < nChunks; k++) {
                                const uint32_t slot = baseSlot + k;
                                if (slot < a.recordCapacity) {
                                    const uint32_t first = segFirst + k * a.factor;
                                    const uint32_t cnt = min(a.factor, segCount - k * a.factor);
                                    BucketRecord b;
                                    b.instanceIndex = instIndex; b.groupIdPacked = (REPLAY ? 0x80000000u : 0u) | (ownerGroup & 0x7FFFFFFFu);
                                    b.meshletIndexAndCount = (cnt << 16) | (first & 0xFFFFu);
                                    b.pageSlabDescriptorIndex = slabDesc; b.pageSlabByteOffset = slabOff;
                                    b.firstBit = firstBit + k * a.factor; b.pad0 = 0; b.pad1 = 0;
                                    buckets[slot] = b;
                                } else atomicAdd(&a.counters[CNT_DROPPED_RECORDS], 1u);
                            }
                        }
                    }
                }
                {
                    const uint32_t myChildren = isInternal ? childCount : 0u;
                    uint32_t incl = myChildren;
#pragma unroll
                    for (int o = 1; o < 64; o <<= 1) { const uint32_t v = (uint32_t)__shfl_up((int)incl, o); if (lane >= (uint32_t)o) incl += v; }
                    const uint32_t total = (uint32_t)__shfl((int)incl, 63);
                    if (total != 0u) {
                        childOff[lane] = incl - myChildren; childFirst[lane] = childBase;
                        if (lane == 63) childOff[64] = total;
                        __syncthreads();
                        for (uint32_t task = lane; task < ((total + 63u) & ~63u); task += 64u) {
                            bool emit = false;
                            uint32_t childId = 0;
                            if (task < total) {
                                uint32_t parent = 0;
#pragma unroll
                                for (uint32_t step = 32; step > 0; step >>= 1) if (childOff[parent + step] <= task) parent += step;
                                childId = childFirst[parent] + (task - childOff[parent]);
                                const brmi_lod_node* ch = sc.lodNodes + (md.lodNodesBase + childId);
                                const f3 cc = skinned ? instC : f3{ch->cullCenterAndRadius[0], ch->cullCenterAndRadius[1], ch->cullCenterAndRadius[2]};
                                const float cr = skinned ? instR : ch->cullCenterAndRadius[3];
                                const f3 ccVS = to_view_space(cc, model, view);
                                emit = REPLAY || !sphere_culled(a, cam, ccVS, cr * scale);
                                if (emit && ch->isLeaf == BRMI_NODE_INTERNAL) {
                                    const f3 wc = xyz(mul_point(f3{ch->lodCenterAndRadius[0], ch->lodCenterAndRadius[1], ch->lodCenterAndRadius[2]}, model));
                                    const float e = projected_error(wc, ch->lodCenterAndRadius[3] * scale, ch->maxQuadricError, scale, camPos, zNear, ortho);
                                    if (e < threshold) emit = false;
                                }
                            }
                            const uint32_t slot = wave_append(&counts[nxt], emit);
                            if (emit) {
                                if (slot < HIER_CAP) frontier[nxt][slot] = childId;
                                else atomicAdd(&a.counters[CNT_DROPPED_RECORDS], 1u);
                            }
                        }
                        __syncthreads();
                    }
                }
            }
            __syncthreads();
            if (lane == 0) counts[cur] = 0u;
            __syncthreads();
        }
    }
    flush();
#pragma unroll
    for (int o = 32; o > 0; o >>= 1) nNodes += (uint32_t)__shfl_xor((int)nNodes, o);
    if (lane == 0) {
        uint32_t* stripe = a.counters + CNT_STRIPES + (blockIdx.x & (CNT_STRIPE_COUNT - 1u)) * CNT_STRIPE_WORDS;
        if (nTested) atomicAdd(&stripe[0], nTested);
        if (nVisible) atomicAdd(&stripe[1], nVisible);
        if (nNodes) atomicAdd(&stripe[2], nNodes);
    }
}

constexpr uint32_t FLAT_WIDE_MAX = 8192;
__global__ void __launch_bounds__(1024) k_cull_flat_wide(CullArgs a, BucketRecord* buckets) {
    __shared__ uint8_t verdict[FLAT_WIDE_MAX];
    __shared__ uint16_t parentOf[FLAT_WIDE_MAX], recordsOf[FLAT_WIDE_MAX];
    __shared__ uint32_t waveSum[2][16], changed, bases[2];
    const brmi_scene_buffers& sc = a.sc;
    const uint32_t t = threadIdx.x, lane = t & 63u, wave = t >> 6;
    const uint32_t viewId = sc.perFrame->mainCameraIndex;
    const brmi_camera* cam = sc.cameras + viewId;
    const brmi_culling_camera* lodCam = sc.cullingCameras + viewId;
    const bool ortho = cam->isOrtho != 0;
    const f3 camPos{lodCam->positionWorldSpace[0], lodCam->positionWorldSpace[1], lodCam->positionWorldSpace[2]};
    const float zNear = lodCam->zNear, threshold = lodCam->errorOverDistanceThreshold;
    const m4 view = load_m4(&cam->view[0][0]);
    uint32_t nTested = 0, nVisible = 0, nNodes = 0;
    for (uint32_t seed = blockIdx.x; seed < sc.activeDrawCount; seed += gridDim.x) {
        const uint32_t instIndex = sc.activeDraws[seed];
        const InstanceWalk iw = a.instanceWalk[instIndex];
        if (iw.flatCount <= 256u || iw.flatCount > FLAT_WIDE_MAX) continue;
        const brmi_per_mesh_instance inst = sc.perMeshInstance[instIndex];
        const brmi_per_object* obj = sc.perObject + inst.perObjectBufferIndex;
        const m4 model = load_m4(&obj->model[0][0]);
        const m4 prevModel = a.occlusion ? load_m4(&obj->prevModel[0][0]) : model;
        const float scale = max_axis_scale(model);
        const f3 instC{inst.boundingSphere[0], inst.boundingSphere[1], inst.boundingSphere[2]}; const float instR = inst.boundingSphere[3];
        {
            const f3 c = to_view_space(instC, model, view);
            const float r = instR * scale;
            const bool bad = isnan(c.x) || isnan(c.y) || isnan(c.z) || isinf(c.x) || isinf(c.y) || isinf(c.z) || isnan(r) || isinf(r);
            if (t == 0) nTested++;
            if (bad || sphere_culled(a, cam, c, r)) continue;
            if (t == 0) nVisible++;
        }
        const bool skinned = iw.skinned != 0u;
        __syncthreads();
        for (uint32_t node = t; node < iw.flatCount; node += 1024u) {
            const FlatNode fn = a.flatNodes[iw.flatBase + node];
            const bool internal = (fn.info & 1u);
            const f3 cullC = skinned ? instC : f3{fn.cull[0], fn.cull[1], fn.cull[2]};
            const float cullR = skinned ? instR : fn.cull[3];
            const f3 cVS = to_view_space(cullC, model, view);
            const float rW = cullR * scale;
            const bool inFrustum = !sphere_culled(a, cam, cVS, rW);
            bool pre = inFrustum, expand = false, hidden = false, leafOk = false;
            uint32_t records = 0;
            if (inFrustum && internal) {
                const f3 lc = xyz(mul_point(f3{fn.lod[0], fn.lod[1], fn.lod[2]}, model));
                const float e = projected_error(lc, fn.lod[3] * scale, fn.maxQuadricError, scale, camPos, zNear, ortho);
                pre = e >= threshold;
                if (pre) { hidden = a.occlusion && occlusion_test_prev(a, cam, cullC, cullR, prevModel); expand = !hidden; }
            } else if (inFrustum) {
// ... 197 lines not shown
        if (nChunks != 0u) {
            const uint32_t segFirst = fn.segFirstCount & 0xFFFFu, segCount = fn.segFirstCount >> 16;
            for (uint32_t k = 0; k < nChunks; k++, slot[1]++) {
                if (slot[1] >= a.recordCapacity) { atomicAdd(&a.counters[CNT_DROPPED_RECORDS], 1u); continue; }
                BucketRecord b;
                b.instanceIndex = instIndex; b.groupIdPacked = fn.ownerGroup & 0x7FFFFFFFu;
                b.meshletIndexAndCount = (min(a.factor, segCount - k * a.factor) << 16) | ((segFirst + k * a.factor) & 0xFFFFu);
                b.pageSlabDescriptorIndex = slabDesc; b.pageSlabByteOffset = slabOff;
                b.firstBit = iw.bitBase + fn.firstBitRel + k * a.factor; b.pad0 = 0; b.pad1 = 0;
                buckets[slot[1]] = b;
            }
        }
        if (hidden) {
            if (slot[2] < a.recordCapacity) a.replayNodes[slot[2]] = NodeRecord{instIndex, 0x80000000u | (1u << 30) | (fn.nodeId & 0x3FFFFFFFu)};
            else atomicAdd(&a.counters[CNT_DROPPED_RECORDS], 1u);
        }
    }
#pragma unroll
    for (int o = 32; o > 0; o >>= 1) { nNodes += (uint32_t)__shfl_xor((int)nNodes, o); nTested += (uint32_t)__shfl_xor((int)nTested, o); nVisible += (uint32_t)__shfl_xor((int)nVisible, o); }
    if (lane == 0) {
        uint32_t* stripe = a.counters + CNT_STRIPES + ((blockIdx.x * 4u + wave) & (CNT_STRIPE_COUNT - 1u)) * CNT_STRIPE_WORDS;
        if (nTested) atomicAdd(&stripe[0], nTested);
        if (nVisible) atomicAdd(&stripe[1], nVisible);
        if (nNodes) atomicAdd(&stripe[2], nNodes);
    }
}

BRMI_DEV float4 skinned_meshlet_bounds(const brmi_scene_buffers& sc, const brmi_meshlet_descriptor* desc, const brmi_page_header* hdr, const uint8_t* page, uint32_t slot, float4 staticBounds) {
    const uint32_t boneCount = desc->boneCount;
    if (slot == 0xFFFFFFFFu || boneCount == 0u || sc.skinningMatrices == nullptr) return staticBounds;
    const uint32_t* boneList = reinterpret_cast<const uint32_t*>(page + hdr->boneIndexStreamOffset + desc->boneListOffset * 4u);
    const f3 c0{staticBounds.x, staticBounds.y, staticBounds.z};
    f3 mc{0.0f, 0.0f, 0.0f}; float mr = 0.0f; bool init = false;
    for (uint32_t b = 0; b < boneCount; b++) {
        const m4 m = load_bone_skin_matrix(sc.skinningMatrices, slot, boneList[b]);
        const f3 tc = xyz(mul_point(c0, m));
        const float tr = staticBounds.w * max_axis_scale(m);
        if (!init) { mc = tc; mr = tr; init = true; continue; }
        const f3 delta = tc - mc;
        const float dist = length3(delta);
        if (dist + tr <= mr) continue;
        if (dist + mr <= tr) { mc = tc; mr = tr; continue; }
        const float newRadius = 0.5f * (dist + mr + tr);
        const float t = (newRadius - mr) / max2(dist, 1e-12f);
        mc = mc + delta * t;
        mr = newRadius;
    }
    if (!init) return staticBounds;
    return make_float4(mc.x, mc.y, mc.z, mr * (1.0f + 1e-5f));
}

struct LcRide { uint32_t mainBlocks; ClusterArgs lc; };
struct ClearRide { uint32_t mainBlocks; ulonglong2* vis2; uint64_t n2; uint32_t clearBlocks; };
template <int SIDE>
__global__ void __launch_bounds__(256) k_cull_clusters(CullArgs a, const BucketRecord* buckets, TempVisible* temp, uint32_t* bitmask, uint8_t* blockDirty,
                                                       typename std::conditional<SIDE == 1, LcRide, typename std::conditional<SIDE == 2, ClearRide, NoSide>::type>::type ride) {
    uint32_t mainBlocks = gridDim.x;
    if constexpr (SIDE == 1) {
        mainBlocks = ride.mainBlocks;
        if (blockIdx.x >= ride.mainBlocks) { lc_fill_block(ride.lc, blockIdx.x - ride.mainBlocks, threadIdx.x); return; }
    }
    if constexpr (SIDE == 2) {
        mainBlocks = ride.mainBlocks;
        if (blockIdx.x >= ride.mainBlocks) {
            const uint64_t stride = (uint64_t)ride.clearBlocks * 256u;
            for (uint64_t i = (uint64_t)(blockIdx.x - ride.mainBlocks) * 256u + threadIdx.x; i < ride.n2; i += stride) ride.vis2[i] = make_ulonglong2(BRMI_VIS_EMPTY, BRMI_VIS_EMPTY);
            return;
        }
    }
    const brmi_scene_buffers& sc = a.sc;
    const uint32_t bucketCount = min(a.counters[a.bucketCounter], a.recordCapacity);
    if (a.feedback && blockIdx.x == 0u && threadIdx.x == 0u) __hip_atomic_store(a.feedback + (a.phase == 1u ? 2 : 4), bucketCount, __ATOMIC_RELAXED, __HIP_MEMORY_SCOPE_SYSTEM);
    const uint32_t viewId = sc.perFrame->mainCameraIndex;
    const brmi_camera* cam = sc.cameras + viewId;
    const brmi_culling_camera* lodCam = sc.cullingCameras + viewId;
    const bool ortho = cam->isOrtho != 0;
    const f3 camPos{lodCam->positionWorldSpace[0], lodCam->positionWorldSpace[1], lodCam->positionWorldSpace[2]};
    const float zNear = lodCam->zNear, threshold = lodCam->errorOverDistanceThreshold;
    const m4 view = load_m4(&cam->view[0][0]);
    uint32_t* tempCount = &a.counters[a.phase == 2 ? CNT_TEMP_VISIBLE2 : CNT_TEMP_VISIBLE];
    const uint64_t totalLanes = (uint64_t)bucketCount * a.factor;
    const uint64_t rounded = (totalLanes + 255ull) & ~255ull;
    __shared__ uint32_t waveSurv[4], waveOccl[4], blockSlots[2];
    for (uint64_t idx = (uint64_t)blockIdx.x * blockDim.x + threadIdx.x; idx < rounded; idx += (uint64_t)mainBlocks * blockDim.x) {
        bool survives = false, occluded = false, tested = false;
        uint4 packed = make_uint4(0, 0, 0, 0);
        uint32_t bit = 0;
        uint4 againLo = make_uint4(0u, 0u, 0u, 0u); uint2 againHi = make_uint2(0u, 0u);
        if (idx < totalLanes) {
            const uint32_t bi = (uint32_t)(idx / a.factor), m = (uint32_t)(idx % a.factor);
            const BucketRecord b = buckets[bi];
            const uint32_t count = b.meshletIndexAndCount >> 16, first = b.meshletIndexAndCount & 0xFFFFu;
            if (m < count && b.pageSlabDescriptorIndex != 0u) {
                tested = true;
                const bool replay = (b.groupIdPacked >> 31) != 0;
                const uint32_t lm = first + m;
                const uint8_t* slab = sc.slabs[b.pageSlabDescriptorIndex];
                const brmi_page_header* hdr = reinterpret_cast<const brmi_page_header*>(slab + b.pageSlabByteOffset);
                if (lm < hdr->meshletCount) {
                    const brmi_meshlet_descriptor* desc = reinterpret_cast<const brmi_meshlet_descriptor*>(slab + b.pageSlabByteOffset + hdr->descriptorOffset + lm * 64u);
                    float4 bounds = *reinterpret_cast<const float4*>(desc->bounds);
                    const uint32_t triAndRefined = desc->triangleCountAndRefinedGroup;
                    const brmi_per_mesh_instance inst = sc.perMeshInstance[b.instanceIndex];
                    if ((sc.perMesh[inst.perMeshBufferIndex].vertexFlags & BRMI_VERTEX_SKINNED) != 0u)
                        bounds = skinned_meshlet_bounds(sc, desc, hdr, slab + b.pageSlabByteOffset, inst.skinningInstanceSlot, bounds);
                    const brmi_clod_mesh_metadata* md = sc.meshMetadata + sc.clodOffsets[b.instanceIndex].clodMeshMetadataIndex;
                    const m4 model = load_m4(&sc.perObject[inst.perObjectBufferIndex].model[0][0]);
                    const float scale = max_axis_scale(model);
                    const f3 cVS = to_view_space(f3{bounds.x, bounds.y, bounds.z}, model, view);
                    const float rW = bounds.w * scale;
                    survives = replay || !sphere_outside_frustum(cVS, rW, cam->clippingPlanes);
                    if (survives) {
                        const int refined = (int)(triAndRefined >> 16) - 1;
                        if (refined_child_suppresses(sc, md->groupsBase, (uint32_t)refined, refined >= 0, model, scale, camPos, zNear, threshold, ortho)) survives = false;
                    }
                    if (survives && a.bandActive) {
                        if (dot3(f3{a.bandTop[0], a.bandTop[1], a.bandTop[2]}, cVS) < -rW || dot3(f3{a.bandBottom[0], a.bandBottom[1], a.bandBottom[2]}, cVS) < -rW) survives = false;
                    }
                    if (survives && stripe_on(a.stripes) && stripe_rejects(a.stripes, cam, cVS, rW)) survives = false;
                    if (survives && a.occlusion &&
                        occlusion_test(a, cam, replay, f3{bounds.x, bounds.y, bounds.z}, bounds.w, cVS, rW, sc.perObject + inst.perObjectBufferIndex)) {
                        survives = false;
                        if (!replay) {
                            occluded = true;
                            againLo = make_uint4(b.instanceIndex, 0x80000000u | (b.groupIdPacked & 0x7FFFFFFFu), (1u << 16) | (lm & 0xFFFFu), b.pageSlabDescriptorIndex);
                            againHi = make_uint2(b.pageSlabByteOffset, b.firstBit + m);
                        }
                    }
                    if (survives) {
                        packed = pack_visible_cluster(viewId, b.instanceIndex, lm, b.groupIdPacked & 0x7FFFFFFFu, b.pageSlabDescriptorIndex, b.pageSlabByteOffset);
                        bit = b.firstBit + m;
                    }
                }
            }
        }
        {
            const uint64_t tm = __ballot(tested);
            if (tm != 0ull && (threadIdx.x & 63u) == 0u) atomicAdd(&a.counters[CNT_STRIPES + (blockIdx.x & (CNT_STRIPE_COUNT - 1u)) * CNT_STRIPE_WORDS + STRIPE_MESHLETS_TESTED], (uint32_t)__popcll(tm));
        }
        occluded = occluded && a.occlusion && a.phase == 1u;
        const uint64_t survM = __ballot(survives), occlM = __ballot(occluded);
        const uint32_t wv = threadIdx.x >> 6;
        __syncthreads();
        if ((threadIdx.x & 63u) == 0u) { waveSurv[wv] = (uint32_t)__popcll(survM); waveOccl[wv] = (uint32_t)__popcll(occlM); }
        __syncthreads();
        if (threadIdx.x < 2u) {
            const uint32_t* ws = threadIdx.x == 0u ? waveSurv : waveOccl;
            const uint32_t total = ws[0] + ws[1] + ws[2] + ws[3];
            blockSlots[threadIdx.x] = total ? atomicAdd(threadIdx.x == 0u ? tempCount : &a.counters[CNT_REPLAY_MESHLETS], total) : 0u;
        }
        __syncthreads();
        uint32_t slot = blockSlots[0] + lane_rank(survM), rs = blockSlots[1] + lane_rank(occlM);
        for (uint32_t w = 0; w < wv; w++) { slot += waveSurv[w]; rs += waveOccl[w]; }
        if (occluded) {
            if (rs < a.recordCapacity) { uint4* dst = reinterpret_cast<uint4*>(&a.replayBuckets[rs]); dst[0] = againLo; dst[1] = make_uint4(againHi.x, againHi.y, 0u, 0u); }
            else atomicAdd(&a.counters[CNT_DROPPED_RECORDS], 1u);
        }
        if (survives) {
            if (slot < a.visibleCapacity) {
                TempVisible t; t.packed = packed; t.bit = bit; t.pad0 = t.pad1 = t.pad2 = 0;
                temp[slot] = t;
                atomicOr(&bitmask[bit >> 5], 1u << (bit & 31u));
                blockDirty[bit >> 16] = 1;
            } else atomicAdd(&a.counters[CNT_DROPPED_CLUSTERS], 1u);
        }
    }
}

constexpr uint32_t SCAN_BLOCK_WORDS = 2048;

__global__ void __launch_bounds__(256) k_scan_reduce(const uint32_t* bitmask, uint32_t totalWords, uint32_t* blockSums, const uint8_t* blockDirty) {
    __shared__ uint32_t partial[4];
    if (blockDirty[blockIdx.x] == 0) { if (threadIdx.x == 0) blockSums[blockIdx.x] = 0u; return; }
    const uint32_t base = blockIdx.x * SCAN_BLOCK_WORDS;
    uint32_t s = 0;
    for (uint32_t i = threadIdx.x; i < SCAN_BLOCK_WORDS; i += 256) { const uint32_t w = base + i; if (w < totalWords) s += __popc(bitmask[w]); }
#pragma unroll
    for (int o = 32; o > 0; o >>= 1) s += __shfl_xor((int)s, o);
    if ((threadIdx.x & 63u) == 0) partial[threadIdx.x >> 6] = s;
    __syncthreads();
    if (threadIdx.x == 0) blockSums[blockIdx.x] = partial[0] + partial[1] + partial[2] + partial[3];
}

__global__ void __launch_bounds__(1024) k_scan_blocks(uint32_t* blockSums, uint32_t nBlocks, uint32_t* counters, uint32_t outIndex, uint32_t capacity, uint32_t usedIndex, uint32_t* hostFeedback) {
    __shared__ uint32_t waveTotals[16];
    __shared__ uint32_t carry;
    if (threadIdx.x == 0) carry = 0;
    __syncthreads();
    for (uint32_t base = 0; base < nBlocks; base += 1024) {
        const uint32_t i = base + threadIdx.x;
        const uint32_t v = i < nBlocks ? blockSums[i] : 0u;
        uint32_t incl = v;
#pragma unroll
        for (int o = 1; o < 64; o <<= 1) { const uint32_t t = (uint32_t)__shfl_up((int)incl, o); if ((threadIdx.x & 63u) >= (uint32_t)o) incl += t; }
        if ((threadIdx.x & 63u) == 63u) waveTotals[threadIdx.x >> 6] = incl;
        __syncthreads();
        uint32_t waveBase = 0;
        for (uint32_t w = 0; w < (threadIdx.x >> 6); w++) waveBase += waveTotals[w];
        const uint32_t c = carry;
        if (i < nBlocks) blockSums[i] = c + waveBase + incl - v;
        __syncthreads();
        if (threadIdx.x == 1023) carry = c + waveBase + incl;
        __syncthreads();
    }
    if (threadIdx.x == 0) {
        const uint32_t placed = min(carry, capacity - (usedIndex == 0xFFFFFFFFu ? 0u : min(counters[usedIndex], capacity)));
        counters[outIndex] = placed;
        if (hostFeedback) __hip_atomic_store(hostFeedback, placed, __ATOMIC_RELAXED, __HIP_MEMORY_SCOPE_SYSTEM);
    }
}

__global__ void __launch_bounds__(256) k_scan_words(const uint32_t* bitmask, uint32_t totalWords, const uint32_t* blockSums, uint32_t* wordPrefix, const uint8_t* blockDirty) {
    __shared__ uint32_t waveTotals[4];
    __shared__ uint32_t carry;
    if (blockDirty[blockIdx.x] == 0) return;
    if (threadIdx.x == 0) carry = blockSums[blockIdx.x];
    __syncthreads();
    const uint32_t base = blockIdx.x * SCAN_BLOCK_WORDS;
    for (uint32_t chunk = 0; chunk < SCAN_BLOCK_WORDS; chunk += 256) {
        const uint32_t w = base + chunk + threadIdx.x;
        const uint32_t v = w < totalWords ? __popc(bitmask[w]) : 0u;
        uint32_t incl = v;
#pragma unroll
        for (int o = 1; o < 64; o <<= 1) { const uint32_t t = (uint32_t)__shfl_up((int)incl, o); if ((threadIdx.x & 63u) >= (uint32_t)o) incl += t; }
        if ((threadIdx.x & 63u) == 63u) waveTotals[threadIdx.x >> 6] = incl;
        __syncthreads();
        uint32_t waveBase = 0;
        for (uint32_t k = 0; k < (threadIdx.x >> 6); k++) waveBase += waveTotals[k];
        const uint32_t c = carry;
        if (w < totalWords) wordPrefix[w] = c + waveBase + incl - v;
        __syncthreads();
        if (threadIdx.x == 255) carry = c + waveBase + incl;
        __syncthreads();
    }
}

constexpr uint32_t SCAN_CHAIN_BLOCKS = 64;
__global__ void __launch_bounds__(256) k_scan_chained(const uint32_t* bitmask, uint32_t totalWords, unsigned long long* agg, uint32_t epoch, uint32_t* wordPrefix,
                                                     uint32_t* counters, uint32_t outIndex, uint32_t capacity, uint32_t usedIndex, uint32_t* hostFeedback) {
    __shared__ uint32_t waveTotals[4];
    __shared__ uint32_t blockPrefix, ticket;
    if (threadIdx.x == 0) ticket = (uint32_t)__hip_atomic_fetch_add(&agg[SCAN_CHAIN_BLOCKS], 1ull, __ATOMIC_RELAXED, __HIP_MEMORY_SCOPE_AGENT);
    __syncthreads();
    const uint32_t block = ticket;
    const uint32_t base = block * SCAN_BLOCK_WORDS + threadIdx.x * 8u;
    uint32_t pc[8], sum = 0;
#pragma unroll
    for (uint32_t k = 0; k < 8u; k++) { const uint32_t w = base + k; pc[k] = w < totalWords ? (uint32_t)__popc(bitmask[w]) : 0u; sum += pc[k]; }
    uint32_t incl = sum;
#pragma unroll
    for (int o = 1; o < 64; o <<= 1) { const uint32_t t = (uint32_t)__shfl_up((int)incl, o); if ((threadIdx.x & 63u) >= (uint32_t)o) incl += t; }
    if ((threadIdx.x & 63u) == 63u) waveTotals[threadIdx.x >> 6] = incl;
    __syncthreads();
    uint32_t waveBase = 0, blockSum = 0;
    for (uint32_t k = 0; k < 4u; k++) { if (k < (threadIdx.x >> 6)) waveBase += waveTotals[k]; blockSum += waveTotals[k]; }
    if (threadIdx.x == 0) __hip_atomic_store(&agg[block], ((unsigned long long)epoch << 32) | blockSum, __ATOMIC_RELAXED, __HIP_MEMORY_SCOPE_AGENT);
    if (threadIdx.x < 64u) {
        uint32_t mine = 0;
        if (threadIdx.x < block) {
            unsigned long long v;
            do { v = __hip_atomic_load(&agg[threadIdx.x], __ATOMIC_RELAXED, __HIP_MEMORY_SCOPE_AGENT); } while ((uint32_t)(v >> 32) != epoch);
            mine = (uint32_t)v;
        }
#pragma unroll
        for (int o = 32; o > 0; o >>= 1) mine += (uint32_t)__shfl_xor((int)mine, o);
        if (threadIdx.x == 0) blockPrefix = mine;
    }
    __syncthreads();
    uint32_t run = blockPrefix + waveBase + incl - sum;
#pragma unroll
    for (uint32_t k = 0; k < 8u; k++) { const uint32_t w = base + k; if (w < totalWords) wordPrefix[w] = run; run += pc[k]; }
    if (block == gridDim.x - 1u && threadIdx.x == 0) {
        __hip_atomic_store(&agg[SCAN_CHAIN_BLOCKS], 0ull, __ATOMIC_RELAXED, __HIP_MEMORY_SCOPE_AGENT);
        const uint32_t placed = min(blockPrefix + blockSum, capacity - (usedIndex == 0xFFFFFFFFu ? 0u : min(counters[usedIndex], capacity)));
        counters[outIndex] = placed;
        if (hostFeedback) __hip_atomic_store(hostFeedback, placed, __ATOMIC_RELAXED, __HIP_MEMORY_SCOPE_SYSTEM);
    }
}

#ifndef BRMI_LOCAL_RANK_WORDS
#define BRMI_LOCAL_RANK_WORDS 8192
#endif
constexpr uint32_t LOCAL_RANK_WORDS = BRMI_LOCAL_RANK_WORDS;
struct LocalRank { uint32_t totalWords, outIndex, usedIndex; uint32_t* hostFeedback; };
struct DrawLists {
    uint32_t* drawList; HeldRecord* held; uint32_t countAll;
    const MeshletBox* boxes; const uint32_t* pageBoxBase; const float* objConst; uint32_t maxTexels; BoxViewport vp; HzbDesc hzb;
};
template <bool LOCAL_RANK, bool HOLD>
__global__ void __launch_bounds__(256) k_scatter_visible(const TempVisible* temp, uint32_t* counters, uint32_t tempCountIndex, const uint32_t* bitmask,
                                                        const uint32_t* wordPrefix, uint4* visible, uint32_t baseIndexCounter, uint32_t capacity, uint32_t visibleCapacity,
                                                        brmi_scene_buffers sc, ClusterSetup* setup, uint32_t resolveCapacity, ClusterUv* clusterUv, LocalRank lr, DrawLists dl) {
    const uint8_t* const* slabs = sc.slabs;
    const uint32_t n = min(counters[tempCountIndex], visibleCapacity);
    const uint32_t base = baseIndexCounter == 0xFFFFFFFFu ? 0u : counters[baseIndexCounter];
    const uint32_t rounded = (n + 63u) & ~63u;
    __shared__ uint32_t prefixLds[LOCAL_RANK ? LOCAL_RANK_WORDS : 1];
    __shared__ uint32_t waveTotals[4];
    if (LOCAL_RANK) {
        if (blockIdx.x != 0u && blockIdx.x * blockDim.x >= rounded) return;
        const uint32_t span = (lr.totalWords + 255u) / 256u;
        const uint32_t w0 = threadIdx.x * span, w1 = min(w0 + span, lr.totalWords);
        uint32_t sum = 0;
        for (uint32_t w = w0; w < w1; w++) sum += __popc(bitmask[w]);
        uint32_t incl = sum;
#pragma unroll
        for (int o = 1; o < 64; o <<= 1) { const uint32_t t = (uint32_t)__shfl_up((int)incl, o); if ((threadIdx.x & 63u) >= (uint32_t)o) incl += t; }
        if ((threadIdx.x & 63u) == 63u) waveTotals[threadIdx.x >> 6] = incl;
        __syncthreads();
        uint32_t waveBase = 0, all = 0;
        for (uint32_t w = 0; w < 4; w++) { if (w < (threadIdx.x >> 6)) waveBase += waveTotals[w]; all += waveTotals[w]; }
        uint32_t run = waveBase + incl - sum;
        for (uint32_t w = w0; w < w1; w++) { prefixLds[w] = run; run += __popc(bitmask[w]); }
        if (blockIdx.x == 0u && threadIdx.x == 0u) {
            const uint32_t placed = min(all, capacity - (lr.usedIndex == 0xFFFFFFFFu ? 0u : min(counters[lr.usedIndex], capacity)));
            counters[lr.outIndex] = placed;
            if (lr.hostFeedback) __hip_atomic_store(lr.hostFeedback, placed, __ATOMIC_RELAXED, __HIP_MEMORY_SCOPE_SYSTEM);
        }
        __syncthreads();
    }
    __shared__ unsigned long long blockBase;
    __shared__ uint32_t waveV[4], waveT[4], waveD[4], waveH[4], blockDraw, blockHeld;
    unsigned long long drawnVT = 0ull;
    if (blockIdx.x == 0u && threadIdx.x == 0u) { const uint32_t room = base < capacity ? capacity - base : 0u; atomicAdd(&counters[CNT_RASTER_CLUSTERS], min(n, room)); if (resolveCapacity == 0u && n != 0u) atomicOr(&counters[CNT_RESOLVE_SPILL], 1u); }
    const uint32_t rounded256 = (n + 255u) & ~255u;
    for (uint32_t i = blockIdx.x * blockDim.x + threadIdx.x; i < rounded256; i += gridDim.x * blockDim.x) {
        uint32_t verts = 0, tris = 0, placed = 0, dst = 0;
        TempVisible t{};
        const uint8_t* slab = nullptr; uint32_t pageOff = 0;
        const brmi_page_header* hdr = nullptr; const brmi_meshlet_descriptor* desc = nullptr;
        uint32_t held = 0u, boxIndex = 0xFFFFFFFFu, perObject = 0u;
        if (i < n) {
            t = temp[i];
            const uint32_t w = t.bit >> 5, b = t.bit & 31u;
            const uint32_t rank = (LOCAL_RANK ? prefixLds[w] : wordPrefix[w]) + __popc(bitmask[w] & ((1u << b) - 1u));
            dst = base + rank;
            if (dst < capacity) {
                visible[dst] = t.packed;
                slab = slabs[vc_slab(t.packed)];
                pageOff = vc_page_offset(t.packed);
                hdr = reinterpret_cast<const brmi_page_header*>(slab + pageOff);
                desc = reinterpret_cast<const brmi_meshlet_descriptor*>(slab + pageOff + hdr->descriptorOffset + vc_meshlet(t.packed) * 64u);
                verts = min((desc->bitsAndVertexCount >> 24) & 0xFFu, BRMI_MESHLET_MAX_VERTS);
                tris = min(desc->triangleCountAndRefinedGroup & 0xFFFFu, BRMI_MESHLET_MAX_TRIS);
                placed = 1;
                if (HOLD) {
                    const brmi_per_mesh_instance inst = sc.perMeshInstance[vc_instance(t.packed)];
                    perObject = inst.perObjectBufferIndex;
                    const uint32_t boxBase = dl.pageBoxBase[(size_t)vc_slab(t.packed) * 1024u + (pageOff >> 18)];
                    if (boxBase != 0xFFFFFFFFu && (sc.perMesh[inst.perMeshBufferIndex].vertexFlags & BRMI_VERTEX_SKINNED) == 0u) {
                        boxIndex = boxBase + vc_meshlet(t.packed);
                        const MeshletBox bx = dl.boxes[boxIndex];
                        const float* oc = dl.objConst + (size_t)perObject * OBJ_CONST_FLOATS;
                        if (bx.valid && box_behind_chain(dl.hzb, bx, oc + 36, oc + 52, dl.vp, dl.maxTexels)) held = 1u;
                    }
                }
            }
        }
        uint32_t inclV = verts, inclT = tris;
#pragma unroll
        for (int o = 1; o < 64; o <<= 1) {
            const uint32_t v = (uint32_t)__shfl_up((int)inclV, o), tt = (uint32_t)__shfl_up((int)inclT, o);
            if ((threadIdx.x & 63u) >= (uint32_t)o) { inclV += v; inclT += tt; }
        }
        const bool isHeld = HOLD && placed != 0u && held != 0u, isDraw = HOLD && placed != 0u && !isHeld;
        const uint64_t drawM = __ballot(isDraw), heldM = __ballot(isHeld);
        __syncthreads();
        if ((threadIdx.x & 63u) == 63u) { waveV[threadIdx.x >> 6] = inclV; waveT[threadIdx.x >> 6] = inclT; waveD[threadIdx.x >> 6] = (uint32_t)__popcll(drawM); waveH[threadIdx.x >> 6] = (uint32_t)__popcll(heldM); }
        __syncthreads();
        if (threadIdx.x == 0u) {
            const unsigned long long totV = (unsigned long long)waveV[0] + waveV[1] + waveV[2] + waveV[3], totT = (unsigned long long)waveT[0] + waveT[1] + waveT[2] + waveT[3];
            blockBase = (totV | totT) ? atomicAdd(reinterpret_cast<unsigned long long*>(&counters[CNT_SUM_VERTS_LO]), totV | (totT << 32)) : 0ull;
        }
        if (HOLD && threadIdx.x == 64u) { const uint32_t tot = waveD[0] + waveD[1] + waveD[2] + waveD[3]; blockDraw = tot ? atomicAdd(&counters[CNT_DRAW1], tot) : 0u; }
        if (HOLD && threadIdx.x == 128u) { const uint32_t tot = waveH[0] + waveH[1] + waveH[2] + waveH[3]; blockHeld = tot ? atomicAdd(&counters[CNT_HELD1], tot) : 0u; }
        __syncthreads();
        if (dl.countAll && placed) drawnVT += (unsigned long long)verts | ((unsigned long long)tris << 32);
        if (isDraw || isHeld) {
            uint32_t slot = (isDraw ? blockDraw : blockHeld) + lane_rank(isDraw ? drawM : heldM);
            for (uint32_t w = 0; w < (threadIdx.x >> 6); w++) slot += isDraw ? waveD[w] : waveH[w];
            if (isDraw) { dl.drawList[slot] = dst; drawnVT += (unsigned long long)verts | ((unsigned long long)tris << 32); }
            else dl.held[slot] = HeldRecord{dst, boxIndex, perObject, verts | (tris << 16)};
        }
        unsigned long long baseV = (uint32_t)blockBase, baseT = blockBase >> 32;
        for (uint32_t w = 0; w < (threadIdx.x >> 6); w++) { baseV += waveV[w]; baseT += waveT[w]; }
        if (placed) {
            const uint32_t instanceIndex = vc_instance(t.packed);
            const brmi_per_mesh_instance inst = sc.perMeshInstance[instanceIndex];
            const brmi_per_object* obj = sc.perObject + inst.perObjectBufferIndex;
            ClusterSetup cs;
            cs.posBase = slab + pageOff + hdr->positionBitstreamOffset + desc->positionBitOffset;
            cs.triBase = slab + pageOff + hdr->triangleStreamOffset + desc->triangleByteOffset;
            cs.nrmBase = slab + pageOff + hdr->normalArrayOffset + desc->vertexAttributeOffset * 4u;
            const brmi_per_mesh* pm = sc.perMesh + inst.perMeshBufferIndex;
            cs.counts = verts | (tris << 8) | ((hdr->compressedPositionQuantExp & 0xFFu) << 16) | (((obj->objectFlags & BRMI_OBJECT_FLAG_REVERSE_WINDING) != 0 ? 1u : 0u) << 24)
                      | ((pm->vertexFlags & BRMI_VERTEX_SKINNED) ? BRMI_CS_SKINNED : 0u) | ((hdr->attributeMask & BRMI_PAGE_ATTRIBUTE_JOINTS) ? BRMI_CS_JOINTS : 0u)
                      | ((hdr->attributeMask & BRMI_PAGE_ATTRIBUTE_WEIGHTS) ? BRMI_CS_WEIGHTS : 0u);
            if (clusterUv) {
                const uint32_t mflags = sc.materials[pm->materialDataIndex].materialFlags;
                const bool layerTextures = openpbr_has_textures(sc.openpbrMaterials + sc.materials[pm->materialDataIndex].openPBRMaterialDataIndex);
                cs.counts |= ((mflags & BRMI_MATERIAL_ALPHA_TEST) ? BRMI_CS_ALPHA : 0u) | (((mflags & BRMI_MATERIAL_ANY_TEXTURE) || layerTextures) ? BRMI_CS_TEXTURED : 0u);
                ClusterUv cu{nullptr, nullptr, nullptr, 0, 0u};
                if (hdr->attributeMask & BRMI_PAGE_ATTRIBUTE_COLOR) { cs.counts |= BRMI_CS_COLOR; cu.color = slab + pageOff + hdr->colorArrayOffset + desc->vertexAttributeOffset * 4u; }
                if (hdr->uvSetCount != 0u) {
                    cu.desc = slab + pageOff + hdr->uvDescriptorOffset + (vc_meshlet(t.packed) * hdr->uvSetCount) * 32u;
                    cu.stream = slab + pageOff + *reinterpret_cast<const uint32_t*>(slab + pageOff + hdr->uvBitstreamDirectoryOffset);
                    cu.directory = (int32_t)hdr->uvBitstreamDirectoryOffset - (int32_t)(hdr->uvDescriptorOffset + (vc_meshlet(t.packed) * hdr->uvSetCount) * 32u);
                    cu.setCount = hdr->uvSetCount;
                }
                clusterUv[dst] = cu;
            }
            cs.jointDelta = (int32_t)(hdr->jointArrayOffset + desc->vertexAttributeOffset * 32u) - (int32_t)(hdr->normalArrayOffset + desc->vertexAttributeOffset * 4u);
            cs.weightDelta = (int32_t)(hdr->weightArrayOffset + desc->vertexAttributeOffset * 32u) - (int32_t)(hdr->normalArrayOffset + desc->vertexAttributeOffset * 4u);
            cs.perObjectIndex = inst.perObjectBufferIndex; cs.instanceIndex = instanceIndex; cs.viewId = vc_view(t.packed);
            cs.materialDataIndex = pm->materialDataIndex; cs.normalMatrixIndex = obj->normalMatrixBufferIndex;
            const unsigned long long v0 = baseV + (inclV - verts), t0 = baseT + (inclT - tris);
            const bool fits = v0 + verts <= resolveCapacity && t0 + tris <= resolveCapacity;
            cs.vertBase = fits ? (uint32_t)v0 : BRMI_ARENA_NONE; cs.triBase32 = fits ? (uint32_t)t0 : BRMI_ARENA_NONE;
            if (!fits && resolveCapacity != 0u) atomicOr(&counters[CNT_RESOLVE_SPILL], 1u);
            setup[dst] = cs;
        }
    }
    if (HOLD || dl.countAll) {
#pragma unroll
        for (int o = 32; o > 0; o >>= 1) drawnVT += (unsigned long long)__shfl_xor((long long)drawnVT, o);
        if ((threadIdx.x & 63u) == 0u && drawnVT != 0ull) atomicAdd(reinterpret_cast<unsigned long long*>(&counters[CNT_DRAWN_VT]), drawnVT);
    }
}

static inline uint32_t grid_for(uint64_t items, uint32_t block, uint32_t maxBlocks) {
    uint64_t g = (items + block - 1) / block;
    if (g < 1) g = 1;
    if (g > maxBlocks) g = maxBlocks;
    return (uint32_t)g;
}

__global__ void k_seed_phase2(uint32_t* counters, uint32_t capacity) { seed_phase2(counters, capacity, threadIdx.x); }

int launch_cull(brmi_pass* p, uint32_t phase, hipStream_t s) {
    if (int rc = ensure_frame_constants(p, s)) return rc;
    if (phase != 1 && phase != 2) return fail(p, BRMI_ERR_INVALID, "brmi_cull: phase %u (1 or 2)", phase);
    if (phase == 2 && !p->cfg.enableOcclusionCulling) return fail(p, BRMI_ERR_STATE, "brmi_cull: phase 2 needs a pass created with enableOcclusionCulling");
    if (phase == 2 && !p->hzbValid) return fail(p, BRMI_ERR_STATE, "brmi_cull: phase 2 needs brmi_build_hzb on the phase-1 depth first");
    CullArgs a;
    a.sc = p->scene; a.counters = p->counters();
    a.instanceBitBase = p->wsPtr<uint32_t>(p->ws.instanceBitBase); a.segPrefix = p->wsPtr<uint32_t>(p->ws.segPrefix);
    a.flatNodes = p->wsPtr<FlatNode>(p->ws.flatNodes); a.flatLeaves = p->wsPtr<FlatLeaf>(p->ws.flatLeaves); a.instanceWalk = p->wsPtr<InstanceWalk>(p->ws.instanceWalk);
    a.recordCapacity = p->cfg.maxTraversalRecords; a.visibleCapacity = p->cfg.maxVisibleClusters;
    uint32_t f = p->cfg.phase2ExpansionFactor; f = f < 1 ? 1 : (f > 64 ? 64 : f);
    { uint32_t n = 1; for (uint32_t c = 2; c <= 64; c <<= 1) if (c <= f) n = c; f = n; }
    a.factor = f; a.phase = phase; a.packedFlat = 0u; a.wideFlat = 0u;
    a.feedback = p->ensureFeedback() ? p->phase2FeedbackDev : nullptr;

    const bool symmetricPerspective = p->camHost.isOrtho == 0 && p->camHost.projection[2][0] == 0.0f && p->camHost.projection[2][1] == 0.0f &&
                                      p->camHost.projection[3][0] == 0.0f && p->camHost.projection[3][1] == 0.0f;
    a.bandActive = ((p->bandY0 != 0 || p->bandY1 != p->cfg.height) && symmetricPerspective) ? 1u : 0u;
    for (int k = 0; k < 3; k++) { a.bandTop[k] = p->bandPlaneTop[k]; a.bandBottom[k] = p->bandPlaneBottom[k]; }
    a.bandPlanes = reinterpret_cast<const float4*>(p->wsPtr<m4>(p->ws.frameConst) + 3);
    a.stripes = p->stripes;
    const brmi_pass* chain = p->chainOwner(phase);
    a.occlusion = (p->cfg.enableOcclusionCulling && chain->hzbValid && p->camHost.isOrtho == 0) ? 1u : 0u;
    a.replayNodes = p->wsPtr<NodeRecord>(p->ws.replayNodes); a.replayBuckets = p->wsPtr<BucketRecord>(p->ws.replayBuckets);
    a.hzb = chain->hzbDesc();
    if (phase == 1) {
        const uint32_t lastVisible = p->phase2FeedbackHost ? reinterpret_cast<volatile uint32_t*>(p->phase2FeedbackHost)[3] : 0u;
        const uint32_t lastPhase2 = p->phase2FeedbackHost ? reinterpret_cast<volatile uint32_t*>(p->phase2FeedbackHost)[0] : 0xFFFFFFFFu;
        p->holdThisFrame = p->holdEnabled && a.occlusion != 0u && (p->holdMinClusters == 0u || (lastVisible != 0xFFFFFFFFu && lastVisible >= p->holdMinClusters) ||
                                                                  (p->holdStillMax != 0u && lastPhase2 < p->holdStillMax && lastVisible != 0xFFFFFFFFu && lastVisible >= p->holdFloor));
    }
    a.frontier0Counter = phase == 1 ? (uint32_t)CNT_FRONTIER0 : (uint32_t)CNT_REPLAY_NODES;
    a.bucketCounter = CNT_BUCKETS;
    NodeRecord* fa = p->wsPtr<NodeRecord>(p->ws.frontierA); NodeRecord* fb = p->wsPtr<NodeRecord>(p->ws.frontierB);
    BucketRecord* buckets = phase == 1 ? p->wsPtr<BucketRecord>(p->ws.buckets) : a.replayBuckets;
    TempVisible* temp = p->wsPtr<TempVisible>(p->ws.tempVisible);
    uint32_t* bitmask = p->wsPtr<uint32_t>(phase == 1 ? p->ws.bitmask1 : p->ws.bitmask2);
    uint8_t* blockDirty = p->wsPtr<uint8_t>(p->ws.blockDirty) + (phase == 1 ? 0u : p->scanBlocks + 1u);
    uint32_t* wordPrefix = p->wsPtr<uint32_t>(p->ws.wordPrefix); uint32_t* blockSums = p->wsPtr<uint32_t>(p->ws.blockSums);

    const uint32_t maxBlocks = 1024;
    bool lightGridRides = false;
    bool flatLevels = false;
    const bool hierarchy = p->minLevelWidth <= HIER_CAP_MAX && !p->forceLevelKernels;
    const bool levelKernels = p->maxLevelWidth > p->spillWidth || p->forceLevelKernels;
    const uint32_t* meshWidth = p->wsPtr<uint32_t>(p->ws.meshLevelWidth);
    const bool spillMode = hierarchy && levelKernels;
    a.meshLevelWidth = meshWidth; a.levelKernelsWidthLo = 0u;
    if (spillMode) a.frontier0Counter = CNT_FRONTIER0;
    const uint32_t widthAll = spillMode ? 0xFFFFFFFFu : 0u, spillAbove = spillMode ? p->spillWidth : 0xFFFFFFFFu;
    if (phase == 1) {
        if (!p->frameStateCleared) BRMI_HIP(p, hipMemsetAsync(p->counters(), 0, p->ws.frameClearBytes, s));
        p->frameStateCleared = false;
        a.packedFlat = (hierarchy && !p->hostFlatNodes.empty() && p->packedFlat) ? 1u : 0u;
        a.wideFlat = (hierarchy && p->anyWideFlat && !p->splitFrame) ? 1u : 0u;
        const uint32_t draws = p->scene.activeDrawCount, minDraws = std::max(1u, p->flatLevelsMinDraws);
        flatLevels = hierarchy && p->allMeshesFlat && !p->forceLevelKernels && (draws >= minDraws || (p->splitFrame && p->maxLevelWidth > 256u && draws >= std::max(1u, minDraws / 4u)));
        if (flatLevels) {
            if (p->clearVisibilityWithTraversal && (p->bandPixelCount & 1ull) == 0ull) { p->clearVisibilityWithTraversal = false; p->clearVisibilityWithClusterCull = true; }
            else if (p->clearVisibilityWithTraversal) flatLevels = false;
        }
        if (flatLevels) {
            hipLaunchKernelGGL(k_cull_flat_level<true>, dim3(grid_for(p->scene.activeDrawCount, 256, 8192)), dim3(256), 0, s, a, 0u, (const NodeRecord*)nullptr, fb, buckets);
            for (uint32_t level = 1; level < p->flatMaxDepth; level++)
                hipLaunchKernelGGL(k_cull_flat_level<false>, dim3(2048), dim3(256), 0, s, a, level, (level & 1u) ? fb : fa, (level & 1u) ? fa : fb, buckets);
            BRMI_LAUNCH_CHECK(p, "k_cull_flat_level");
        }
        const dim3 hgrid(std::min(std::max(1u, p->scene.activeDrawCount), 16384u) + (a.packedFlat ? (p->scene.activeDrawCount + 7u) / 8u : 0u));
        if (hierarchy && !flatLevels) {
            const bool wide = p->maxLevelWidth > 256u;
            const uint32_t widthHi = spillMode ? widthAll : (wide ? HIER_CAP_MAX : 256u);
            if (p->clearVisibilityWithTraversal) {
                SideJobs sj{reinterpret_cast<ulonglong2*>(static_cast<unsigned long long*>(p->res[BRMI_RES_VISIBILITY]) + p->bandFirstPixel), p->bandPixelCount >> 1, hgrid.x, p->clearRiderBlocks, cluster_args_of(p)};
                const dim3 grid(hgrid.x + sj.clearBlocks + p->numLightClusters);
                if (wide) hipLaunchKernelGGL((k_cull_hierarchy<false, 1024, BRMI_HIER_STAGE_WIDE, true>), grid, dim3(64), 0, s, a, buckets, meshWidth, 0u, widthHi, spillAbove, fa, sj);
                else hipLaunchKernelGGL((k_cull_hierarchy<false, 256, 128, true>), grid, dim3(64), 0, s, a, buckets, meshWidth, 0u, widthHi, spillAbove, fa, sj);
                p->clearVisibilityWithTraversal = false; lightGridRides = true;
            } else if (wide) hipLaunchKernelGGL((k_cull_hierarchy<false, 1024, BRMI_HIER_STAGE_WIDE>), hgrid, dim3(64), 0, s, a, buckets, meshWidth, 0u, widthHi, spillAbove, fa, NoSide{});
            else hipLaunchKernelGGL((k_cull_hierarchy<false, 256, 128>), hgrid, dim3(64), 0, s, a, buckets, meshWidth, 0u, widthHi, spillAbove, fa, NoSide{});
        }
        if (a.wideFlat && !flatLevels) hipLaunchKernelGGL(k_cull_flat_wide, dim3(std::min(std::max(1u, p->scene.activeDrawCount), 4096u)), dim3(1024), 0, s, a, buckets);
        if (levelKernels && !spillMode && !flatLevels) hipLaunchKernelGGL(k_cull_instances, dim3(grid_for(p->scene.activeDrawCount, 256, maxBlocks)), dim3(256), 0, s, a, fa);
        BRMI_LAUNCH_CHECK(p, "k_cull_instances");
    } else {
        if (!p->phase2Seeded) hipLaunchKernelGGL(k_seed_phase2, dim3(1), dim3(128), 0, s, p->counters(), a.recordCapacity);
        p->phase2Seeded = false;
        const NoSide none{};
        if (hierarchy && p->maxLevelWidth <= 256u) hipLaunchKernelGGL((k_cull_hierarchy<true, 256, 128>), dim3(2048), dim3(64), 0, s, a, buckets, meshWidth, 0u, 256u, spillAbove, fa, none);
        else if (hierarchy) hipLaunchKernelGGL((k_cull_hierarchy<true, 1024, BRMI_HIER_STAGE_WIDE>), dim3(2048), dim3(64), 0, s, a, buckets, meshWidth, 0u, spillMode ? widthAll : HIER_CAP_MAX, spillAbove, fa, none);
    }
    const uint32_t travGrid = grid_for(std::min<uint64_t>(p->cfg.maxTraversalRecords, (uint64_t)p->scene.lodNodeCount * 4 + 4096), 256, maxBlocks);
    const uint32_t levelLaunches = spillMode ? std::min(p->maxLevels, std::max(1u, p->spillLevels)) : p->maxLevels;
    const bool flatCoversPhase1 = phase == 1 && hierarchy && spillMode && p->allMeshesFlat && a.wideFlat != 0u && !p->forceLevelKernels;
    for (uint32_t level = 0; level < levelLaunches && levelKernels && !flatCoversPhase1 && !flatLevels; level++) {
        const NodeRecord* in = level == 0 ? ((phase == 1 || spillMode) ? fa : a.replayNodes) : ((level & 1u) ? fb : fa);
        hipLaunchKernelGGL(k_traverse, dim3(travGrid), dim3(256), 0, s, a, level, in, (level & 1u) ? fa : fb, buckets);
        BRMI_LAUNCH_CHECK(p, "k_traverse");
    }
    uint32_t smallGrid = phase == 1 ? 512u : 128u, scatterGrid = smallGrid;
    if (p->phase2FeedbackHost) {
        const uint32_t lastBuckets = reinterpret_cast<volatile uint32_t*>(p->phase2FeedbackHost)[phase == 1 ? 2 : 4];
        const uint32_t lastVisible = reinterpret_cast<volatile uint32_t*>(p->phase2FeedbackHost)[phase == 1 ? 3 : 0];
        smallGrid = std::max(smallGrid, grid_for((uint64_t)std::min<uint32_t>(lastBuckets, p->cfg.maxTraversalRecords) * f, 256, 8192));
        scatterGrid = std::max(scatterGrid, grid_for(std::min<uint32_t>(lastVisible, p->cfg.maxVisibleClusters), 256, 8192));
    }
    if (lightGridRides) {
        hipLaunchKernelGGL(k_cull_clusters<1>, dim3(smallGrid + (p->numLightClusters + 3u) / 4u), dim3(256), 0, s, a, buckets, temp, bitmask, blockDirty, LcRide{smallGrid, cluster_args_of(p)});
        p->lightGridDone = true;
    } else if (phase == 1 && p->clearVisibilityWithClusterCull) {
        const uint32_t clearBlocks = 2048;
        hipLaunchKernelGGL(k_cull_clusters<2>, dim3(smallGrid + clearBlocks), dim3(256), 0, s, a, buckets, temp, bitmask, blockDirty,
                           ClearRide{smallGrid, reinterpret_cast<ulonglong2*>(static_cast<unsigned long long*>(p->res[BRMI_RES_VISIBILITY]) + p->bandFirstPixel), p->bandPixelCount >> 1, clearBlocks});
        p->clearVisibilityWithClusterCull = false;
    } else hipLaunchKernelGGL(k_cull_clusters<0>, dim3(smallGrid), dim3(256), 0, s, a, buckets, temp, bitmask, blockDirty, NoSide{});
    BRMI_LAUNCH_CHECK(p, "k_cull_clusters");
    const uint32_t outIndex = phase == 1 ? CNT_VISIBLE : CNT_VISIBLE2, usedIndex = phase == 1 ? 0xFFFFFFFFu : (uint32_t)CNT_VISIBLE;
    if (phase == 2 && p->phase2DirectMax != 0u) (void)p->ensureFeedback();
    uint32_t* feedback = phase == 2 ? p->phase2FeedbackDev : (p->phase2FeedbackDev ? p->phase2FeedbackDev + 3 : nullptr);
    const bool localRank = p->totalWords <= LOCAL_RANK_WORDS && !p->forceLevelKernels;
    if (localRank) {
    } else {
        if (p->scanBlocks <= SCAN_CHAIN_BLOCKS) {
            if (++p->scanEpoch == 0u) p->scanEpoch = 1u;
            hipLaunchKernelGGL(k_scan_chained, dim3(p->scanBlocks), dim3(256), 0, s, bitmask, p->totalWords, p->wsPtr<unsigned long long>(p->ws.scanAgg), p->scanEpoch, wordPrefix,
                               p->counters(), outIndex, p->cfg.maxVisibleClusters, usedIndex, feedback);
        } else {
            hipLaunchKernelGGL(k_scan_reduce, dim3(p->scanBlocks), dim3(256), 0, s, bitmask, p->totalWords, blockSums, blockDirty);
            hipLaunchKernelGGL(k_scan_blocks, dim3(1), dim3(1024), 0, s, blockSums, p->scanBlocks, p->counters(), outIndex, p->cfg.maxVisibleClusters, usedIndex, feedback);
            hipLaunchKernelGGL(k_scan_words, dim3(p->scanBlocks), dim3(256), 0, s, bitmask, p->totalWords, blockSums, wordPrefix, blockDirty);
        }
    }
    if (phase == 1) p->inlineResolve = resolve_inline_frame(p);
    const uint32_t arenaCapacity = p->inlineResolve ? 0u : p->resolveCapacity;
    auto scatter = [&](auto kernel) {
        hipLaunchKernelGGL(kernel, dim3(scatterGrid), dim3(256), 0, s, temp, p->counters(), (uint32_t)(phase == 1 ? CNT_TEMP_VISIBLE : CNT_TEMP_VISIBLE2), bitmask, wordPrefix,
                           static_cast<uint4*>(p->res[BRMI_RES_VISIBLE_CLUSTERS]), phase == 1 ? 0xFFFFFFFFu : (uint32_t)CNT_VISIBLE, p->cfg.maxVisibleClusters, p->cfg.maxVisibleClusters, p->scene, p->wsPtr<ClusterSetup>(p->ws.clusterSetup), arenaCapacity,
                           (p->sceneHasTextures || p->sceneHasAlphaTest || p->sceneHasVertexColors) ? p->wsPtr<ClusterUv>(p->ws.clusterUv) : nullptr, LocalRank{p->totalWords, outIndex, usedIndex, feedback},
                           (phase == 1 && p->holdThisFrame) ? DrawLists{p->wsPtr<uint32_t>(p->ws.drawList), p->wsPtr<HeldRecord>(p->ws.heldRecords), 0u, p->wsPtr<MeshletBox>(p->ws.meshletBoxes), p->wsPtr<uint32_t>(p->ws.pageBoxBase),
                                                                      p->wsPtr<float>(p->ws.objConst), p->holdMaxTexels, BoxViewport{(float)p->cfg.width, (float)p->cfg.height, 0.0f, 0.0f, 0, (int)p->bandY0, (int)p->cfg.width - 1, (int)p->bandY1 - 1}, a.hzb}
                                                          : DrawLists{nullptr, nullptr, p->holdThisFrame ? 1u : 0u, nullptr, nullptr, nullptr, 0u, BoxViewport{}, HzbDesc{}});
// ... 45 lines not shown
```

basicrenderer_amd/csrc/brmi_internal.h:

```cpp
#ifndef BRMI_INTERNAL_H
#define BRMI_INTERNAL_H

#include <hip/hip_runtime.h>

#include <string>
#include <vector>

#include "brmi.h"
#include "brmi_device.h"

#ifndef BRMI_BIN_COUNT_STRIDE
#define BRMI_BIN_COUNT_STRIDE 32
#endif
namespace brmi {

enum CounterIndex : uint32_t {
    CNT_VISIBLE = 3,
    CNT_VISIBLE2,
    CNT_DROPPED_RECORDS,
    CNT_DROPPED_CLUSTERS,
    CNT_INSTANCES_TESTED,
    CNT_INSTANCES_VISIBLE,
    CNT_NODES_VISITED,
    CNT_MESHLETS_TESTED,
    CNT_LIGHT_PAGES,
    CNT_SUM_VERTS_LO = 14, CNT_SUM_VERTS_HI,
    CNT_SUM_TRIS_LO, CNT_SUM_TRIS_HI,
    CNT_RASTER_CLUSTERS,
    CNT_BIN_OVERFLOW,
    CNT_DEFERRED_PIXELS_B,
    CNT_DEFERRED_PIXELS,
    CNT_RESOLVE_SPILL,
    CNT_RESERVED_37,
    CNT_DEFERRED_DROPPED,
    CNT_TILE_OVERFLOW,
    CNT_FRONTIER0 = 32,
    CNT_STRIPES = 128,
    CNT_STRIPE_COUNT = 64, CNT_STRIPE_WORDS = 32,
    STRIPE_DEFERRED_A = 4, STRIPE_DEFERRED_B = 8,
    STRIPE_OVERFLOW = 3,
    STRIPE_MESHLETS_TESTED = 12,
    CNT_BUCKETS = 128 + 64 * 32,
    CNT_TEMP_VISIBLE = CNT_BUCKETS + 32,
    CNT_TEMP_VISIBLE2 = CNT_BUCKETS + 64,
    CNT_REPLAY_NODES = CNT_BUCKETS + 96,
    CNT_REPLAY_MESHLETS = CNT_BUCKETS + 128,
    CNT_DRAW1 = CNT_BUCKETS + 160,
    CNT_HELD1 = CNT_BUCKETS + 192,
    CNT_LATE1 = CNT_BUCKETS + 224,
    CNT_DRAWN_VT = CNT_BUCKETS + 256,
    CNT_WIDE1 = CNT_BUCKETS + 288, CNT_WIDE1B = CNT_BUCKETS + 320, CNT_WIDE2 = CNT_BUCKETS + 352,
    CNT_GENERAL1 = CNT_BUCKETS + 384,
    CNT_BIG1 = CNT_BUCKETS + 416,
    CNT_WORDS = CNT_BUCKETS + 416 + 64 * 32
};
static_assert((CNT_DRAWN_VT & 1u) == 0u, "64-bit counter");

__device__ inline void seed_phase2(uint32_t* counters, uint32_t capacity, uint32_t t) {
    if (t == 0) { counters[CNT_REPLAY_NODES] = min(counters[CNT_REPLAY_NODES], capacity); counters[CNT_BUCKETS] = min(counters[CNT_REPLAY_MESHLETS], capacity); counters[CNT_TEMP_VISIBLE2] = 0; counters[CNT_VISIBLE2] = 0; }
    if (t < CNT_STRIPES - CNT_FRONTIER0) counters[CNT_FRONTIER0 + t] = 0;
    if (t < CNT_STRIPE_COUNT) {
        uint32_t* q = &counters[CNT_STRIPES + t * CNT_STRIPE_WORDS + STRIPE_OVERFLOW];
        if (*q) atomicAdd(&counters[CNT_BIN_OVERFLOW], *q);
        *q = 0u;
    }
}

struct FlatNode {
    float cull[4], lod[4]; float maxQuadricError;
    uint32_t nodeId;
    uint32_t info;
    uint32_t ownerGroup;
    uint32_t segFirstCount;
    uint32_t pageMapIndex;
    uint32_t firstBitRel;
    uint32_t children;
};
struct FlatLeaf { float group[4], child[4]; float childParentError, pad[3]; };
// ... 55 lines not shown
#pragma unroll
    for (int s = 0; s < 2; s++) {
        const float px = s ? bx.hi[0] : bx.lo[0], py = s ? bx.hi[1] : bx.lo[1], pz = s ? bx.hi[2] : bx.lo[2];
#pragma unroll
        for (int c = 0; c < 3; c++) {
            X[s][c] = px * mvpRows[0 + col[c]]; Y[s][c] = py * mvpRows[4 + col[c]]; Z[s][c] = pz * mvpRows[8 + col[c]] + mvpRows[12 + col[c]];
            magC = fmaxf(magC, fmaxf(fmaxf(fabsf(X[s][c]), fabsf(Y[s][c])), fmaxf(fabsf(pz * mvpRows[8 + col[c]]), fabsf(mvpRows[12 + col[c]]))));
        }
        X[s][3] = px * mvzRow[0]; Y[s][3] = py * mvzRow[1]; Z[s][3] = pz * mvzRow[2] + mvzRow[3];
        mag = fmaxf(mag, fmaxf(fmaxf(fabsf(X[s][3]), fabsf(Y[s][3])), fabsf(pz * mvzRow[2])));
    }
    float sx0 = 3.0e38f, sy0 = 3.0e38f, sx1 = -3.0e38f, sy1 = -3.0e38f, d = 3.0e38f, w = 3.0e38f;
#pragma unroll
    for (int k = 0; k < 8; k++) {
        const int i = k & 1, j = (k >> 1) & 1, l = k >> 2;
        const float cx = (X[i][0] + Y[j][0]) + Z[l][0], cy = (X[i][1] + Y[j][1]) + Z[l][1], cw = (X[i][2] + Y[j][2]) + Z[l][2];
        const float inv = __builtin_amdgcn_rcpf(cw);
        const float sx = (cx * inv + 1.0f) * 0.5f * vp.width + vp.minX, sy = (1.0f - cy * inv) * 0.5f * vp.height + vp.minY;
        sx0 = fminf(sx0, sx); sx1 = fmaxf(sx1, sx); sy0 = fminf(sy0, sy); sy1 = fmaxf(sy1, sy);
        d = fminf(d, -((X[i][3] + Y[j][3]) + Z[l][3])); w = fminf(w, cw);
    }
    if (!(w > 1e-6f && d > 0.0f && fabsf(sx0) < 1.0e9f && fabsf(sx1) < 1.0e9f && fabsf(sy0) < 1.0e9f && fabsf(sy1) < 1.0e9f)) return false;
    const float guard = 0.25f + magC * __builtin_amdgcn_rcpf(w) * 9.5367431640625e-7f * (vp.width + vp.height);
    const int x0 = max((int)floorf(fmaxf(sx0 - guard, -1.0e9f)), vp.x0), y0 = max((int)floorf(fmaxf(sy0 - guard, -1.0e9f)), vp.y0);
    const int x1 = min((int)floorf(fminf(sx1 + guard, 1.0e9f)), vp.x1), y1 = min((int)floorf(fminf(sy1 + guard, 1.0e9f)), vp.y1);
    const float nearSafe = d - (d * 7.62939453125e-6f + mag * 3.814697265625e-6f);
    if (!(nearSafe > 0.0f)) return false;
    if (x0 > x1 || y0 > y1) return true;
    uint32_t mip = 1u;
    while (mip + 1u < hzb.mipCount && (((x1 >> mip) - (x0 >> mip) + 1) > (int)maxTexels || ((y1 >> mip) - (y0 >> mip) + 1) > (int)maxTexels)) mip++;
    if (mip >= hzb.mipCount) return false;
    const uint32_t mw = max(hzb.paddedW >> mip, 1u), mh = max(hzb.paddedH >> mip, 1u);
    if (((x1 >> mip) - (x0 >> mip) + 1) > (int)maxTexels || ((y1 >> mip) - (y0 >> mip) + 1) > (int)maxTexels) return false;
    const float* m = hzb.mips + hzb.mipOffset[mip];
    const int tx0 = x0 >> mip, tx1 = min(x1 >> mip, (int)mw - 1), ty1 = min(y1 >> mip, (int)mh - 1);
    for (int y = y0 >> mip; y <= ty1; y += BRMI_BOX_ROWS) {
        float farthest = 0.0f;
#pragma unroll
        for (int r = 0; r < BRMI_BOX_ROWS; r++) {
            const int yy = min(y + r, ty1);
            for (int x = tx0; x <= tx1; x++) farthest = fmaxf(farthest, m[(size_t)yy * mw + (uint32_t)x]);
        }
        if (!(farthest < nearSafe)) return false;
    }
    return true;
}

struct FrameSnapshot { brmi_per_frame perFrame; brmi_camera camera; };

struct LayerUniform { unsigned long long coatWord, fuzzWord, coatFilledWord, fuzzFilledWord; uint32_t coatUniform, fuzzUniform, coatFilled, fuzzFilled; };

struct Workspace {
    uint64_t counters, frontierA, frontierB, buckets, tempVisible, bitmask1, bitmask2, blockDirty, chainDirty, wordPrefix, blockSums,
             instanceBitBase, segPrefix, meshLevelWidth, scanAgg, flatNodes, flatLeaves, instanceWalk, planes, replayNodes, replayBuckets, lightVS, lightMeta, clusterPages, clusterHits, pageTotal, lightHitMasks, binCounts, binRecords, binOverflow, binPlan, binItems, binScratch, clusterSetup, resolveVerts, resolveTris, matWords, shadeTables, lutF, frameConst, objConst, matConst, deferredPixels,
             frameSnapshot, clusterUv, binAlpha, overflowAlpha, resolveUVs, resolveColors, alphaMats, shadeRows, shadeAvgs, ggxQuads, shadeLights, clusterList, listEntries, listRecords, layerUniform,
             meshletBoxes, pageBoxBase, pageRefs, drawList, heldRecords, lateList, wideQueue, wideAlpha, generalList, bigQueue, bigRuns, frameClearBytes, total;
};

}

struct brmi_pass {
    brmi_config cfg{};
    brmi_scene_buffers scene{};
    bool haveScene = false, setupDone = false, updated = false;
    void* res[BRMI_RES_COUNT] = {};
    uint64_t resBytes[BRMI_RES_COUNT] = {};
    uint64_t resNeed[BRMI_RES_COUNT] = {};
    uint32_t tilesX = 0, tilesY = 0;
    uint64_t paddedPixels = 0;
    uint32_t bandY0 = 0, bandY1 = 0;
    brmi::StripeMap stripes{0, 0, 0, 0};
    uint32_t frameHeight() const { return stripes.count > 1u ? stripes.fullHeight : cfg.height; }
    float bandPlaneTop[3] = {0, 0, 0}, bandPlaneBottom[3] = {0, 0, 0};
    uint64_t bandFirstPixel = 0, bandPixelCount = 0;
    uint32_t maxLevels = 1;
    static constexpr uint32_t spillWidth = 1024;
    uint32_t spillLevels = 0;
    uint32_t minLevelWidth = 0;
    std::vector<uint32_t> hostMeshLevelWidth;
    uint32_t maxLevelWidth = 0;
    std::vector<brmi::PageRef> hostPageRefs; std::vector<uint32_t> hostPageBoxBase; uint32_t totalBoxes = 0;
    bool holdEnabled = false;
    bool holdThisFrame = false;
    uint32_t holdMinClusters = 16384;
    uint32_t lateDirectMax = 128;
    uint32_t holdFloor = 512;
    uint32_t holdStillMax = 8;
    uint32_t holdMaxTexels = 8;
    uint32_t retestMaxTexels = 8;
    uint32_t chainStripLo = 0xFFFFFFFFu, chainStripHi = 0u;
    uint32_t wideCapacity = 16384;
    uint32_t wideEntries = 128;
    uint32_t leanMinClusters = 32768, leanMaxGeneralPct = 40, leanGrid = 24576, leanEmitGrid = 4096, leanWideEntries = 16, leanQueue = 1u << 20;
    bool leanActive = false, leanLastLaunch = false; uint32_t leanRetryIn = 0;
    uint32_t wideMinTriangles = 4;
    bool chainBuiltInRaster = false;
    bool sceneHasVertexColors = false;
    uint32_t sceneUvSets = 1;
    bool sceneHasAlphaTest = false, sceneHasTextures = false, sceneHasParallax = false;
    bool sceneHasCoat = true, sceneHasFuzz = true;
    std::vector<float> sliceStartHost; float sliceKey[3] = {0, 0, 0}; uint32_t sliceKeyN[2] = {0, 0};
    uint32_t* phase2FeedbackHost = nullptr; uint32_t* phase2FeedbackDev = nullptr;
    bool ensureFeedback() {
        if (phase2FeedbackHost) return true;
        if (hipHostMalloc(reinterpret_cast<void**>(&phase2FeedbackHost), 64, hipHostMallocMapped) != hipSuccess) { phase2FeedbackHost = nullptr; return false; }
        phase2FeedbackHost[0] = 0xFFFFFFFFu; phase2FeedbackHost[1] = 0u;
        for (int k = 2; k < 16; k++) phase2FeedbackHost[k] = 0u;
        if (hipHostGetDevicePointer(reinterpret_cast<void**>(&phase2FeedbackDev), phase2FeedbackHost, 0) != hipSuccess) { (void)hipHostFree(phase2FeedbackHost); phase2FeedbackHost = nullptr; phase2FeedbackDev = nullptr; return false; }
        return true;
    }
    uint32_t phase2DirectMax = 128;
    static constexpr uint32_t clearRiderBlocks = 8192;
    bool splitFrame = false;
    uint32_t shadeSlabs = 0; brmi_slab_fn shadeSlabFn = nullptr; void* shadeSlabUser = nullptr;
    bool frameWaitsIssued = false;
    bool anyWideFlat = false, allMeshesFlat = false;
    uint32_t flatMaxDepth = 1;
    uint32_t flatLevelsMinDraws = 16384;
    uint32_t scanEpoch = 0;
    bool packedFlat = true;
    static constexpr uint32_t shadeGridShared = 10240;
    static constexpr uint32_t gbufferGridShared = 4096;
    bool shadeSharesChip = false;
    bool lightGridDone = false;
    bool clearVisibilityWithClusterCull = false;
    bool clearFrameStateWithConstants = false, clearVisibilityWithTraversal = false;
    bool seedInHzbTail = false, phase2Seeded = false;
    bool fuseFrameClear = false, frameStateCleared = false;
    bool forceLevelKernels = false;
    uint64_t totalBits = 0; uint32_t totalWords = 0, scanBlocks = 0;
    uint32_t numLightClusters = 0, lightPagePool = 0;
    uint32_t binOverflowPerStripe = 1u << 14;
    uint32_t binMinSlice = 1024, binSharedSlice = 512, binGrid = 1024;
    uint32_t binScratchTiles = 2048, binItemCapacity = 0;
    uint32_t binsX = 0, binsY = 0, binCapacity = 16384;
    uint32_t deferredStripeCapacity = 0;
    uint32_t resolveCapacity = 0;
    static constexpr uint32_t rasterGrid = 8192;
    int bigTriAreaDense = 32; uint32_t denseClusterCount = 6144;
    int bigTriArea = 32, bigTriAreaAlpha = 32;
    uint32_t hzbMipCount = 0; std::vector<uint64_t> hzbMipOffsets; std::vector<uint32_t> hzbMipW, hzbMipH;
    bool hzbValid = false;
    brmi_pass* history = nullptr;
    hipEvent_t chainReady = nullptr;
    bool chainRecorded = false;
    brmi_stream chainStream = nullptr;
    hipEvent_t cullDone = nullptr;
    hipEvent_t geometryDone = nullptr, frameDone = nullptr;
    bool frameDoneRecorded = false;
    std::vector<brmi_pass*> historyUsers;
    bool layerPlanesDirty = false;
    bool layerPlanesUniform = false;
    bool chainDirtyTracked = false;
    int resolveInlineMode = -1;
    bool inlineResolve = false;
    bool resolveSetupDone = false;
    bool depthFinal = false;
    const brmi_pass* chainOwner(uint32_t phase) const { return (phase == 1 && history) ? history : this; }
    brmi::HzbDesc hzbDesc() const;
    std::vector<uint32_t> hostInstanceBitBase, hostSegPrefix;
    std::vector<brmi::FlatNode> hostFlatNodes; std::vector<brmi::FlatLeaf> hostFlatLeaves; std::vector<brmi::InstanceWalk> hostInstanceWalk;
    brmi::Workspace ws{};
    brmi_camera camHost{};
    brmi_per_frame pfHost{};
// ... 42 lines not shown
```

basicrenderer_amd/renderer.py:

```python
import ctypes as C

import numpy as np

from . import capi


class BrmiError(RuntimeError):
    pass


def detile(flat, width, height, tile=8):
    tx, ty = (width + tile - 1) // tile, (height + tile - 1) // tile
    rest = flat.shape[1:]
    a = flat.reshape((ty, tx, tile, tile) + rest)
    a = np.transpose(a, (0, 3, 1, 2) + tuple(range(4, 4 + len(rest)))).reshape((ty * tile, tx * tile) + rest)
    return np.ascontiguousarray(a[:height, :width])


def tile(img, tile=8):
    height, width = img.shape[:2]
    tx, ty = (width + tile - 1) // tile, (height + tile - 1) // tile
    rest = img.shape[2:]
    pad = np.zeros((ty * tile, tx * tile) + rest, dtype=img.dtype)
    pad[:height, :width] = img
# ... 96 lines not shown
        src = getattr(self, "_cam_scene", self.scene)
        cam, pf = src.camera_host(), src.per_frame_host()
        upd = capi.FrameUpdate(cam.ctypes.data, pf.ctypes.data, frame_index)
        self._check(self.lib.brmi_update(self._h, C.byref(upd), self._s()), "brmi_update")

    def execute(self, shading_stream=None):
        if shading_stream is None:
            self._check(self.lib.brmi_execute(self._h, self._s()), "brmi_execute")
        else:
            self._check(self.lib.brmi_execute_split(self._h, self._s(), C.c_void_p(shading_stream.cuda_stream)), "brmi_execute_split")
        err, self._slab_error = getattr(self, "_slab_error", None), None
        if err is not None:
            raise BrmiError(f"the shade-slab hook raised during execute: {err!r}") from err

    def stage(self, name, *args):
        fn = getattr(self.lib, "brmi_" + name)
        self._check(fn(self._h, *[capi.u32(a) for a in args], self._s()), "brmi_" + name)
        err, self._slab_error = getattr(self, "_slab_error", None), None
        if err is not None:
            raise BrmiError(f"the shade-slab hook raised during brmi_{name}: {err!r}") from err

    def counters(self):
        c = capi.Counters()
        self._check(self.lib.brmi_read_counters(self._h, C.byref(c), self._s()), "brmi_read_counters")
        return c

    def stage_times(self):
        ms = (capi.f32 * len(capi.STAGE_NAMES))()
        self._check(self.lib.brmi_stage_times(self._h, ms), "brmi_stage_times")
        return dict(zip(capi.STAGE_NAMES, [float(x) for x in ms]))

    def set_timed_stages(self, names=None):
        mask = 0xFFFFFFFF if names is None else sum(1 << capi.STAGE_NAMES.index(n) for n in names)
        self._check(self.lib.brmi_set_timed_stages(self._h, mask), "brmi_set_timed_stages")

    def algorithmic_bytes(self):
        per = (capi.u64 * len(capi.STAGE_NAMES))()
        total = capi.u64()
        self._check(self.lib.brmi_algorithmic_bytes(self._h, per, C.byref(total)), "brmi_algorithmic_bytes")
        return dict(zip(capi.STAGE_NAMES, [int(x) for x in per])), int(total.value)

    def held_clusters(self):
        nh, nl = capi.u32(), capi.u32()
        self._check(self.lib.brmi_debug_read_held(self._h, None, 0, C.byref(nh), None, 0, C.byref(nl)), "brmi_debug_read_held")
        held, late = np.zeros(max(1, nh.value), dtype=np.uint32), np.zeros(max(1, nl.value), dtype=np.uint32)
        self._check(self.lib.brmi_debug_read_held(self._h, held.ctypes.data_as(C.POINTER(capi.u32)), len(held), C.byref(nh), late.ctypes.data_as(C.POINTER(capi.u32)), len(late), C.byref(nl)), "brmi_debug_read_held")
        return held[: nh.value], late[: nl.value]

    def lean_clusters(self):
        out = (capi.u32 * 4)()
        self._check(self.lib.brmi_debug_lean_clusters(self._h, out), "brmi_debug_lean_clusters")
        return tuple(int(v) for v in out)

    def wide_triangles(self):
        out = (capi.u32 * 3)()
        self._check(self.lib.brmi_debug_wide_triangles(self._h, out), "brmi_debug_wide_triangles")
        return tuple(int(x) for x in out)

    def algorithmic_bytes_launched(self):
        per = (capi.u64 * len(capi.STAGE_NAMES))()
        total = capi.u64()
        self._check(self.lib.brmi_algorithmic_bytes_launched(self._h, per, C.byref(total)), "brmi_algorithmic_bytes_launched")
        return dict(zip(capi.STAGE_NAMES, [int(x) for x in per])), int(total.value)

    def _img(self, rid, dtype, comps=1):
        self.torch.cuda.synchronize(self.device)
        raw = self.res[capi.RES[rid]].cpu().numpy()
        a = raw.view(dtype)
        n = a.size // comps
        a = a.reshape((n, comps)) if comps > 1 else a.reshape((n,))
        return detile(a, self.W, self.H)

    def visibility(self):
        return self._img("VISIBILITY", np.uint64)

    def depth(self):
        return self._img("LINEAR_DEPTH", np.float32)

    def hdr(self):
        return self._img("HDR_COLOR", np.uint64)

    def gbuffer(self):
        return dict(normals=self._img("GBUF_NORMALS", np.float32, 4), albedo=self._img("GBUF_ALBEDO", np.uint32),
                    coat=self._img("GBUF_COAT", np.uint64), emissive=self._img("GBUF_EMISSIVE", np.uint64),
                    fuzz=self._img("GBUF_FUZZ", np.uint64), mr=self._img("GBUF_METALLIC_ROUGHNESS", np.uint32),
                    motion=self._img("GBUF_MOTION_VECTORS", np.uint32))

    def visible_clusters(self):
        c = self.counters()
        n = c.visibleClusters + c.visibleClustersPhase2
        self.torch.cuda.synchronize(self.device)
        raw = self.res[capi.RES["VISIBLE_CLUSTERS"]][: n * 16].cpu().numpy()
        return raw.view(np.uint32).reshape(n, 4)

    def invalidate_hzb(self):
        self._check(self.lib.brmi_invalidate_hzb(self._h), "brmi_invalidate_hzb")

    def set_shade_slabs(self, slabs, callback=None):
        if callback is None or slabs <= 1:
            self._slab_cb = None
            self._check(self.lib.brmi_set_shade_slabs(self._h, capi.u32(0), None, None), "brmi_set_shade_slabs")
            return
        proto = C.CFUNCTYPE(None, C.c_void_p, C.c_uint32, C.c_uint32, C.c_void_p)

        def trampoline(user, r0, r1, stream):
            try:
# ... 49 lines not shown
```

include/brmi.h:

```cpp
#ifndef BRMI_H
#define BRMI_H

#include <stdint.h>
#include "brmi_types.h"

#ifdef __cplusplus
extern "C" {
#endif

#define BRMI_ABI_VERSION 1u

typedef enum brmi_status {
    BRMI_OK            = 0,
    BRMI_ERR_INVALID   = -1,
    BRMI_ERR_HIP       = -2,
    BRMI_ERR_CAPACITY  = -3,
    BRMI_ERR_STATE     = -4
} brmi_status;

typedef struct brmi_pass brmi_pass;
typedef void* brmi_stream;

typedef struct brmi_config {
    uint32_t structSize;
// ... 51 lines not shown
typedef enum brmi_resource_id {
    BRMI_RES_VISIBILITY = 0,
    BRMI_RES_LINEAR_DEPTH,
    BRMI_RES_GBUF_NORMALS,
    BRMI_RES_GBUF_ALBEDO,
    BRMI_RES_GBUF_COAT,
    BRMI_RES_GBUF_EMISSIVE,
    BRMI_RES_GBUF_FUZZ,
    BRMI_RES_GBUF_METALLIC_ROUGHNESS,
    BRMI_RES_GBUF_MOTION_VECTORS,
    BRMI_RES_HDR_COLOR,
    BRMI_RES_VISIBLE_CLUSTERS,
    BRMI_RES_LIGHT_CLUSTERS,
    BRMI_RES_LIGHT_PAGES,
    BRMI_RES_HZB,
    BRMI_RES_WORKSPACE,
    BRMI_RES_COUNT
} brmi_resource_id;

typedef enum brmi_usage {
    BRMI_USAGE_SHADER_RESOURCE  = 1u << 0,
    BRMI_USAGE_UNORDERED_ACCESS = 1u << 1,
    BRMI_USAGE_INTERNAL         = 1u << 2
} brmi_usage;

typedef struct brmi_resource_desc {
    uint32_t    id;
    const char* name;
    uint64_t    bytes;
    uint32_t    usage;
    uint32_t    width, height;
    uint32_t    bytesPerPixel;
    uint32_t    tileW, tileH;
} brmi_resource_desc;

typedef void (*brmi_declare_cb)(void* user, const brmi_resource_desc* desc);

typedef struct brmi_resource_binding { uint32_t id; void* ptr; uint64_t bytes; } brmi_resource_binding;

typedef struct brmi_frame_update {
    const brmi_camera*    mainCameraHost;
    const brmi_per_frame* perFrameHost;
    uint32_t              frameIndex;
} brmi_frame_update;

typedef struct brmi_counters {
    uint32_t instancesTested, instancesVisible;
    uint32_t nodesVisited, bucketRecords;
    uint32_t meshletsTested, visibleClusters, visibleClustersPhase2;
    uint32_t droppedRecords, droppedClusters;
    uint32_t lightPagesUsed;
    uint32_t replayNodes, replayMeshlets;
    uint32_t reserved[6];
} brmi_counters;

enum brmi_stage {
    BRMI_STAGE_CLEAR = 0, BRMI_STAGE_CULL, BRMI_STAGE_RASTER, BRMI_STAGE_DEPTH_COPY, BRMI_STAGE_HZB,
    BRMI_STAGE_CULL2, BRMI_STAGE_RASTER2, BRMI_STAGE_GBUFFER, BRMI_STAGE_LIGHT_CLUSTER, BRMI_STAGE_SHADE,
    BRMI_STAGE_COUNT
};

uint32_t    brmi_abi_version(void);
int         brmi_create(const brmi_config* cfg, brmi_pass** out);
int         brmi_declare(brmi_pass* pass, brmi_declare_cb cb, void* user);
int         brmi_set_scene(brmi_pass* pass, const brmi_scene_buffers* scene);
int         brmi_setup(brmi_pass* pass, const brmi_resource_binding* b, uint32_t n, brmi_stream stream);
int         brmi_update(brmi_pass* pass, const brmi_frame_update* upd, brmi_stream stream);
int         brmi_execute(brmi_pass* pass, brmi_stream stream);
int         brmi_execute_split(brmi_pass* pass, brmi_stream geometryStream, brmi_stream shadingStream);
void        brmi_destroy(brmi_pass* pass);
const char* brmi_last_error(const brmi_pass* pass);

int brmi_set_band(brmi_pass* pass, uint32_t bandY0, uint32_t bandY1);

int brmi_clear_visibility(brmi_pass* pass, brmi_stream stream);
int brmi_cull(brmi_pass* pass, uint32_t phase, brmi_stream stream);
int brmi_raster(brmi_pass* pass, uint32_t phase, brmi_stream stream);
int brmi_depth_copy(brmi_pass* pass, brmi_stream stream);
int brmi_build_hzb(brmi_pass* pass, brmi_stream stream);
int brmi_invalidate_hzb(brmi_pass* pass);
int brmi_set_history_source(brmi_pass* pass, brmi_pass* source);
int brmi_gbuffer(brmi_pass* pass, brmi_stream stream);
int brmi_light_clustering(brmi_pass* pass, brmi_stream stream);
int brmi_shade(brmi_pass* pass, brmi_stream stream);
typedef void (*brmi_slab_fn)(void* user, uint32_t row0, uint32_t row1, brmi_stream stream);
int brmi_set_shade_slabs(brmi_pass* pass, uint32_t slabs, brmi_slab_fn fn, void* user);

int brmi_read_counters(brmi_pass* pass, brmi_counters* out, brmi_stream stream);
int brmi_stage_times(brmi_pass* pass, float* msOut );
int brmi_set_timed_stages(brmi_pass* pass, uint32_t stageMask);
int brmi_algorithmic_bytes(brmi_pass* pass, uint64_t* perStage , uint64_t* total);
int brmi_algorithmic_bytes_launched(brmi_pass* pass, uint64_t* perStage , uint64_t* total);

int brmi_debug_arith(const float* a, const float* b, float* outDiv, float* outSqrt, uint32_t* outHalfBits, uint32_t n, brmi_stream stream);

int brmi_debug_wide_triangles(brmi_pass* pass, uint32_t out[3]);
int brmi_debug_lean_clusters(brmi_pass* pass, uint32_t out[4]);
int brmi_debug_read_lean_queue(brmi_pass* pass, uint32_t stripe, uint32_t* runs, uint32_t maxRuns, void* entries, uint32_t maxEntries, uint32_t counts[2]);

int brmi_debug_read_held(brmi_pass* pass, uint32_t* held, uint32_t heldCapacity, uint32_t* heldCount, uint32_t* late, uint32_t lateCapacity, uint32_t* lateCount);

int brmi_debug_read_bin_records(brmi_pass* pass, void* dst, uint64_t bytes);

int brmi_debug_arith_in_range(const float* a, float* outRcp, float* outSqrt, float* outRsqrt, uint32_t n, brmi_stream stream);

#ifdef __cplusplus
}
#endif
#endif
```

Before: 17370 Mpixels/s.

## Fuse small phase-2 cull, scan and scatter into one persistent kernel

When the previous frame's phase-2 bucket and visible counts are small, the occlusion phase-2 hierarchy walk, cluster cull, prefix scan and visible scatter are run in a single small-grid kernel. The stages are separated by a grid-wide epoch barrier with a timeout. The hierarchy walk and cluster cull are factored into device functions so the fused kernel can reuse them, with wave-level sync when four walks share one block. This is meant to remove several kernel launches and their serialization for a nearly empty second phase. In exchange the work runs on very few blocks, and a barrier timeout drops the remaining work and is counted in droppedWaits.

Result: slower. 16200 Mpixels/s (-6.7%).

```diff
diff --git a/basicrenderer_amd/capi.py b/basicrenderer_amd/capi.py
--- a/basicrenderer_amd/capi.py
+++ b/basicrenderer_amd/capi.py
@@ -115,7 +115,7 @@
 class Counters(C.Structure):
     _fields_ = [(n, u32) for n in ("instancesTested instancesVisible nodesVisited bucketRecords meshletsTested "
                                    "visibleClusters visibleClustersPhase2 droppedRecords droppedClusters "
-                                   "lightPagesUsed replayNodes replayMeshlets").split()] + [("reserved", u32 * 6)]
+                                   "lightPagesUsed replayNodes replayMeshlets").split()] + [("reserved", u32 * 6), ("droppedWaits", u32)]
 
 
 class ComposeConfig(C.Structure):
@@ -210,7 +210,7 @@
 BRMI_EXPORTS = ["brmi_abi_version", "brmi_default_config", "brmi_create", "brmi_declare", "brmi_set_scene", "brmi_setup", "brmi_set_band",
                 "brmi_update", "brmi_execute", "brmi_execute_split", "brmi_destroy", "brmi_last_error", "brmi_clear_visibility", "brmi_cull",
                 "brmi_raster", "brmi_depth_copy", "brmi_build_hzb", "brmi_invalidate_hzb", "brmi_set_history_source", "brmi_gbuffer", "brmi_light_clustering",
-                "brmi_shade", "brmi_set_shade_slabs", "brmi_read_counters", "brmi_stage_times", "brmi_set_timed_stages", "brmi_algorithmic_bytes", "brmi_algorithmic_bytes_launched", "brmi_debug_arith", "brmi_debug_arith_in_range", "brmi_debug_read_bin_records", "brmi_debug_wide_triangles", "brmi_debug_lean_clusters", "brmi_debug_read_lean_queue", "brmi_debug_read_held"]
+                "brmi_shade", "brmi_set_shade_slabs", "brmi_read_counters", "brmi_stage_times", "brmi_set_timed_stages", "brmi_algorithmic_bytes", "brmi_algorithmic_bytes_launched", "brmi_debug_arith", "brmi_debug_arith_in_range", "brmi_debug_read_bin_records", "brmi_debug_wide_triangles", "brmi_debug_lean_clusters", "brmi_debug_phase2_small", "brmi_debug_read_lean_queue", "brmi_debug_read_held"]
 
 
 def brmi_lib():
diff --git a/basicrenderer_amd/csrc/brmi_api.hip b/basicrenderer_amd/csrc/brmi_api.hip
--- a/basicrenderer_amd/csrc/brmi_api.hip
+++ b/basicrenderer_amd/csrc/brmi_api.hip
@@ -90,6 +90,7 @@
     w.wordPrefix = take((uint64_t)p->totalWords * 4);
     w.blockSums = take((uint64_t)(p->scanBlocks + 1) * 4);
     w.scanAgg = take(65 * 8);
+    w.phase2Barrier = take(128);
     w.instanceBitBase = take((uint64_t)std::max<size_t>(1, p->hostInstanceBitBase.size()) * 4);
     w.segPrefix = take((uint64_t)std::max<size_t>(1, p->hostSegPrefix.size()) * 4);
     w.meshLevelWidth = take((uint64_t)std::max<size_t>(1, p->hostMeshLevelWidth.size()) * 4);
@@ -240,6 +241,9 @@
     p->packedFlat = tuning("flat_packed", 1) != 0;
     p->flatLevelsMinDraws = (uint32_t)std::max(0l, tuning("flat_levels_min_draws", p->flatLevelsMinDraws));
     p->phase2DirectMax = (uint32_t)std::max(0l, tuning("phase2_direct_max", p->phase2DirectMax));
+    p->phase2FusedMax = (uint32_t)std::max(0l, tuning("phase2_fused_max", p->phase2FusedMax));
+    p->phase2FusedMode = (int)tuning("phase2_fused", -1);
+    p->phase2FusedGrid = (uint32_t)std::min(64l, std::max(1l, tuning("phase2_fused_grid", p->phase2FusedGrid)));
     p->resolveInlineMode = (int)tuning("resolve_inline", -1);
     p->wideCapacity = (uint32_t)std::min(1l << 20, std::max(0l, tuning("wide_capacity", p->wideCapacity)));
     p->wideMinTriangles = (uint32_t)std::max(0l, tuning("wide_min_triangles", p->wideMinTriangles));
@@ -832,6 +836,7 @@
     out->reserved[1] = std::min(c[CNT_HELD1], p->cfg.maxVisibleClusters); out->reserved[3] = std::min(c[CNT_LATE1], p->cfg.maxVisibleClusters);
     out->reserved[4] = c[CNT_RASTER_CLUSTERS]; out->reserved[5] = c[CNT_BIN_OVERFLOW] + overflowQueued;
     out->replayNodes = c[CNT_REPLAY_NODES]; out->replayMeshlets = c[CNT_REPLAY_MESHLETS];
+    out->droppedWaits = c[CNT_DROPPED_WAITS];
     return BRMI_OK;
 }
 
@@ -939,6 +944,15 @@
     return BRMI_OK;
 }
 
+int brmi_debug_phase2_small(brmi_pass* p, uint32_t out[4]) {
+    if (!p || !out || !p->setupDone) return BRMI_ERR_INVALID;
+    BRMI_HIP(p, hipDeviceSynchronize());
+    uint32_t dropped = 0u;
+    BRMI_HIP(p, hipMemcpy(&dropped, p->counters() + CNT_DROPPED_WAITS, 4, hipMemcpyDeviceToHost));
+    out[0] = p->phase2SmallLast ? 1u : 0u; out[1] = p->phase2SmallLaunches; out[2] = dropped; out[3] = p->phase2FusedGrid;
+    return BRMI_OK;
+}
+
 int brmi_debug_read_lean_queue(brmi_pass* p, uint32_t stripe, uint32_t* runs, uint32_t maxRuns, void* entries, uint32_t maxEntries, uint32_t counts[2]) {
     if (!p || !counts || !p->setupDone || stripe >= 64u || p->leanMinClusters == 0u) return BRMI_ERR_INVALID;
     BRMI_HIP(p, hipDeviceSynchronize());
diff --git a/basicrenderer_amd/csrc/brmi_cull.hip b/basicrenderer_amd/csrc/brmi_cull.hip
--- a/basicrenderer_amd/csrc/brmi_cull.hip
+++ b/basicrenderer_amd/csrc/brmi_cull.hip
@@ -319,27 +319,22 @@
 #define BRMI_HIER_STAGE_WIDE 128
 #endif
 constexpr uint32_t HIER_CAP_MAX = 1024;
-struct NoSide {};
-struct SideJobs { ulonglong2* vis2; uint64_t n2; uint32_t walkBlocks, clearBlocks; ClusterArgs lc; };
-template <bool REPLAY, uint32_t HIER_CAP, uint32_t HIER_STAGE, bool SIDE = false>
-__global__ void __launch_bounds__(64) k_cull_hierarchy(CullArgs a, BucketRecord* buckets, const uint32_t* meshLevelWidth, uint32_t widthLo, uint32_t widthHi, uint32_t spillAbove, NodeRecord* spillOut,
-                                                    typename std::conditional<SIDE, SideJobs, NoSide>::type sj) {
-    uint32_t walkBlocks = gridDim.x;
-    if constexpr (SIDE) {
-        walkBlocks = sj.walkBlocks;
-        if (blockIdx.x >= sj.walkBlocks + sj.clearBlocks) { lc_count_wave(sj.lc, blockIdx.x - sj.walkBlocks - sj.clearBlocks, threadIdx.x); return; }
-        if (blockIdx.x >= sj.walkBlocks) {
-            const uint64_t stride = (uint64_t)sj.clearBlocks * 64u;
-            for (uint64_t i = (uint64_t)(blockIdx.x - sj.walkBlocks) * 64u + threadIdx.x; i < sj.n2; i += stride) sj.vis2[i] = make_ulonglong2(BRMI_VIS_EMPTY, BRMI_VIS_EMPTY);
-            return;
-        }
-    }
-    __shared__ uint32_t frontier[2][HIER_CAP];
-    __shared__ uint32_t counts[2];
-    __shared__ uint32_t childOff[65], childFirst[64];
-    __shared__ BucketRecord stage[HIER_STAGE];
+template <uint32_t HIER_CAP, uint32_t HIER_STAGE>
+struct HierLds {
+    uint32_t frontier[2][HIER_CAP];
+    uint32_t counts[2];
+    uint32_t childOff[65], childFirst[64];
+    BucketRecord stage[HIER_STAGE];
+};
+template <bool WAVE_SYNC> BRMI_DEV void hier_sync() {
+    if constexpr (WAVE_SYNC) { __builtin_amdgcn_fence(__ATOMIC_RELEASE, "workgroup"); __builtin_amdgcn_wave_barrier(); __builtin_amdgcn_fence(__ATOMIC_ACQUIRE, "workgroup"); }
+    else __syncthreads();
+}
+template <bool REPLAY, uint32_t HIER_CAP, uint32_t HIER_STAGE, bool WAVE_SYNC>
+BRMI_DEV void hierarchy_walk(const CullArgs& a, BucketRecord* buckets, const uint32_t* meshLevelWidth, uint32_t widthLo, uint32_t widthHi, uint32_t spillAbove, NodeRecord* spillOut,
+                             HierLds<HIER_CAP, HIER_STAGE>& lds, const uint32_t walkBlock, const uint32_t walkBlocks, const uint32_t lane) {
+    auto& frontier = lds.frontier; auto& counts = lds.counts; auto& childOff = lds.childOff; auto& childFirst = lds.childFirst; auto& stage = lds.stage;
     const brmi_scene_buffers& sc = a.sc;
-    const uint32_t lane = threadIdx.x;
     const uint32_t viewId = sc.perFrame->mainCameraIndex;
     const brmi_camera* cam = sc.cameras + viewId;
     const brmi_culling_camera* lodCam = sc.cullingCameras + viewId;
@@ -355,20 +350,20 @@
         uint32_t baseSlot = 0;
         if (lane == 0) baseSlot = atomicAdd(&a.counters[a.bucketCounter], staged);
         baseSlot = (uint32_t)__shfl((int)baseSlot, 0);
-        __syncthreads();
+        hier_sync<WAVE_SYNC>();
         for (uint32_t k = lane; k < staged; k += 64u) {
             if (baseSlot + k < a.recordCapacity) buckets[baseSlot + k] = stage[k];
             else atomicAdd(&a.counters[CNT_DROPPED_RECORDS], 1u);
         }
-        __syncthreads();
+        hier_sync<WAVE_SYNC>();
         staged = 0u;
     };
-    uint32_t firstSeed = blockIdx.x, seedStride = walkBlocks;
+    uint32_t firstSeed = walkBlock, seedStride = walkBlocks;
     if (!REPLAY && a.packedFlat) {
         const uint32_t packedWaves = (seeds + 7u) >> 3;
-        if (blockIdx.x < packedWaves) {
+        if (walkBlock < packedWaves) {
             const uint32_t g8 = lane & ~7u, j = lane & 7u;
-            const uint32_t seed = blockIdx.x * 8u + (lane >> 3);
+            const uint32_t seed = walkBlock * 8u + (lane >> 3);
             const bool haveSeed = seed < seeds;
             const uint32_t instIndex = haveSeed ? sc.activeDraws[seed] : 0u;
             brmi_per_mesh_instance inst{}; InstanceWalk iw{0u, 0u, 0u, 0u};
@@ -462,7 +457,7 @@
                 buckets[slot] = b;
             }
             firstSeed = seeds;
-        } else { firstSeed = blockIdx.x - packedWaves; seedStride = walkBlocks - packedWaves; }
+        } else { firstSeed = walkBlock - packedWaves; seedStride = walkBlocks - packedWaves; }
     }
     for (uint32_t seed = firstSeed; seed < seeds; seed += seedStride) {
         uint32_t instIndex, startNode;
@@ -609,9 +604,9 @@
         }
         const bool skinned = (sc.perMesh[inst.perMeshBufferIndex].vertexFlags & BRMI_VERTEX_SKINNED) != 0;
         const uint32_t bitBase = a.instanceBitBase[instIndex];
-        __syncthreads();
+        hier_sync<WAVE_SYNC>();
         if (lane == 0) { frontier[0][0] = startNode; counts[0] = 1u; counts[1] = 0u; }
-        __syncthreads();
+        hier_sync<WAVE_SYNC>();
         for (uint32_t level = 0; level < 64u; level++) {
             const uint32_t cur = level & 1u, nxt = cur ^ 1u;
             const uint32_t n = min(counts[cur], HIER_CAP);
@@ -725,7 +720,7 @@
                     if (total != 0u) {
                         childOff[lane] = incl - myChildren; childFirst[lane] = childBase;
                         if (lane == 63) childOff[64] = total;
-                        __syncthreads();
+                        hier_sync<WAVE_SYNC>();
                         for (uint32_t task = lane; task < ((total + 63u) & ~63u); task += 64u) {
                             bool emit = false;
                             uint32_t childId = 0;
@@ -751,24 +746,43 @@
                                 else atomicAdd(&a.counters[CNT_DROPPED_RECORDS], 1u);
                             }
                         }
-                        __syncthreads();
-                    }
-                }
-            }
-            __syncthreads();
+                        hier_sync<WAVE_SYNC>();
+                    }
+                }
+            }
+            hier_sync<WAVE_SYNC>();
             if (lane == 0) counts[cur] = 0u;
-            __syncthreads();
+            hier_sync<WAVE_SYNC>();
         }
     }
     flush();
 #pragma unroll
     for (int o = 32; o > 0; o >>= 1) nNodes += (uint32_t)__shfl_xor((int)nNodes, o);
     if (lane == 0) {
-        uint32_t* stripe = a.counters + CNT_STRIPES + (blockIdx.x & (CNT_STRIPE_COUNT - 1u)) * CNT_STRIPE_WORDS;
+        uint32_t* stripe = a.counters + CNT_STRIPES + (walkBlock & (CNT_STRIPE_COUNT - 1u)) * CNT_STRIPE_WORDS;
         if (nTested) atomicAdd(&stripe[0], nTested);
         if (nVisible) atomicAdd(&stripe[1], nVisible);
         if (nNodes) atomicAdd(&stripe[2], nNodes);
     }
+}
+
+struct NoSide {};
+struct SideJobs { ulonglong2* vis2; uint64_t n2; uint32_t walkBlocks, clearBlocks; ClusterArgs lc; };
+template <bool REPLAY, uint32_t HIER_CAP, uint32_t HIER_STAGE, bool SIDE = false>
+__global__ void __launch_bounds__(64) k_cull_hierarchy(CullArgs a, BucketRecord* buckets, const uint32_t* meshLevelWidth, uint32_t widthLo, uint32_t widthHi, uint32_t spillAbove, NodeRecord* spillOut,
+                                                    typename std::conditional<SIDE, SideJobs, NoSide>::type sj) {
+    uint32_t walkBlocks = gridDim.x;
+    if constexpr (SIDE) {
+        walkBlocks = sj.walkBlocks;
+        if (blockIdx.x >= sj.walkBlocks + sj.clearBlocks) { lc_count_wave(sj.lc, blockIdx.x - sj.walkBlocks - sj.clearBlocks, threadIdx.x); return; }
+        if (blockIdx.x >= sj.walkBlocks) {
+            const uint64_t stride = (uint64_t)sj.clearBlocks * 64u;
+            for (uint64_t i = (uint64_t)(blockIdx.x - sj.walkBlocks) * 64u + threadIdx.x; i < sj.n2; i += stride) sj.vis2[i] = make_ulonglong2(BRMI_VIS_EMPTY, BRMI_VIS_EMPTY);
+            return;
+        }
+    }
+    __shared__ HierLds<HIER_CAP, HIER_STAGE> lds;
+    hierarchy_walk<REPLAY, HIER_CAP, HIER_STAGE, false>(a, buckets, meshLevelWidth, widthLo, widthHi, spillAbove, spillOut, lds, blockIdx.x, walkBlocks, threadIdx.x);
 }
 
 constexpr uint32_t FLAT_WIDE_MAX = 8192;
@@ -1072,25 +1086,10 @@
 
 struct LcRide { uint32_t mainBlocks; ClusterArgs lc; };
 struct ClearRide { uint32_t mainBlocks; ulonglong2* vis2; uint64_t n2; uint32_t clearBlocks; };
-template <int SIDE>
-__global__ void __launch_bounds__(256) k_cull_clusters(CullArgs a, const BucketRecord* buckets, TempVisible* temp, uint32_t* bitmask, uint8_t* blockDirty,
-                                                       typename std::conditional<SIDE == 1, LcRide, typename std::conditional<SIDE == 2, ClearRide, NoSide>::type>::type ride) {
-    uint32_t mainBlocks = gridDim.x;
-    if constexpr (SIDE == 1) {
-        mainBlocks = ride.mainBlocks;
-        if (blockIdx.x >= ride.mainBlocks) { lc_fill_block(ride.lc, blockIdx.x - ride.mainBlocks, threadIdx.x); return; }
-    }
-    if constexpr (SIDE == 2) {
-        mainBlocks = ride.mainBlocks;
-        if (blockIdx.x >= ride.mainBlocks) {
-            const uint64_t stride = (uint64_t)ride.clearBlocks * 256u;
-            for (uint64_t i = (uint64_t)(blockIdx.x - ride.mainBlocks) * 256u + threadIdx.x; i < ride.n2; i += stride) ride.vis2[i] = make_ulonglong2(BRMI_VIS_EMPTY, BRMI_VIS_EMPTY);
-            return;
-        }
-    }
+BRMI_DEV void cull_clusters_block(const CullArgs& a, const BucketRecord* buckets, TempVisible* temp, uint32_t* bitmask, uint8_t* blockDirty, const uint32_t block, const uint32_t mainBlocks) {
     const brmi_scene_buffers& sc = a.sc;
     const uint32_t bucketCount = min(a.counters[a.bucketCounter], a.recordCapacity);
-    if (a.feedback && blockIdx.x == 0u && threadIdx.x == 0u) __hip_atomic_store(a.feedback + (a.phase == 1u ? 2 : 4), bucketCount, __ATOMIC_RELAXED, __HIP_MEMORY_SCOPE_SYSTEM);
+    if (a.feedback && block == 0u && threadIdx.x == 0u) __hip_atomic_store(a.feedback + (a.phase == 1u ? 2 : 4), bucketCount, __ATOMIC_RELAXED, __HIP_MEMORY_SCOPE_SYSTEM);
     const uint32_t viewId = sc.perFrame->mainCameraIndex;
     const brmi_camera* cam = sc.cameras + viewId;
     const brmi_culling_camera* lodCam = sc.cullingCameras + viewId;
@@ -1102,7 +1101,7 @@
     const uint64_t totalLanes = (uint64_t)bucketCount * a.factor;
     const uint64_t rounded = (totalLanes + 255ull) & ~255ull;
     __shared__ uint32_t waveSurv[4], waveOccl[4], blockSlots[2];
-    for (uint64_t idx = (uint64_t)blockIdx.x * blockDim.x + threadIdx.x; idx < rounded; idx += (uint64_t)mainBlocks * blockDim.x) {
+    for (uint64_t idx = (uint64_t)block * blockDim.x + threadIdx.x; idx < rounded; idx += (uint64_t)mainBlocks * blockDim.x) {
         bool survives = false, occluded = false, tested = false;
         uint4 packed = make_uint4(0, 0, 0, 0);
         uint32_t bit = 0;
@@ -1156,7 +1155,7 @@
         }
         {
             const uint64_t tm = __ballot(tested);
-            if (tm != 0ull && (threadIdx.x & 63u) == 0u) atomicAdd(&a.counters[CNT_STRIPES + (blockIdx.x & (CNT_STRIPE_COUNT - 1u)) * CNT_STRIPE_WORDS + STRIPE_MESHLETS_TESTED], (uint32_t)__popcll(tm));
+            if (tm != 0ull && (threadIdx.x & 63u) == 0u) atomicAdd(&a.counters[CNT_STRIPES + (block & (CNT_STRIPE_COUNT - 1u)) * CNT_STRIPE_WORDS + STRIPE_MESHLETS_TESTED], (uint32_t)__popcll(tm));
         }
         occluded = occluded && a.occlusion && a.phase == 1u;
         const uint64_t survM = __ballot(survives), occlM = __ballot(occluded);
@@ -1185,6 +1184,25 @@
             } else atomicAdd(&a.counters[CNT_DROPPED_CLUSTERS], 1u);
         }
     }
+}
+
+template <int SIDE>
+__global__ void __launch_bounds__(256) k_cull_clusters(CullArgs a, const BucketRecord* buckets, TempVisible* temp, uint32_t* bitmask, uint8_t* blockDirty,
+                                                       typename std::conditional<SIDE == 1, LcRide, typename std::conditional<SIDE == 2, ClearRide, NoSide>::type>::type ride) {
+    uint32_t mainBlocks = gridDim.x;
+    if constexpr (SIDE == 1) {
+        mainBlocks = ride.mainBlocks;
+        if (blockIdx.x >= ride.mainBlocks) { lc_fill_block(ride.lc, blockIdx.x - ride.mainBlocks, threadIdx.x); return; }
+    }
+    if constexpr (SIDE == 2) {
+        mainBlocks = ride.mainBlocks;
+        if (blockIdx.x >= ride.mainBlocks) {
+            const uint64_t stride = (uint64_t)ride.clearBlocks * 256u;
+            for (uint64_t i = (uint64_t)(blockIdx.x - ride.mainBlocks) * 256u + threadIdx.x; i < ride.n2; i += stride) ride.vis2[i] = make_ulonglong2(BRMI_VIS_EMPTY, BRMI_VIS_EMPTY);
+            return;
+        }
+    }
+    cull_clusters_block(a, buckets, temp, bitmask, blockDirty, blockIdx.x, mainBlocks);
 }
 
 constexpr uint32_t SCAN_BLOCK_WORDS = 2048;
@@ -1255,6 +1273,22 @@
     }
 }
 
+BRMI_DEV void scan_block_popcounts(const uint32_t* bitmask, uint32_t totalWords, uint32_t block, uint32_t* waveTotals, uint32_t (&pc)[8], uint32_t& before, uint32_t& blockSum) {
+    const uint32_t base = block * SCAN_BLOCK_WORDS + threadIdx.x * 8u;
+    uint32_t sum = 0;
+#pragma unroll
+    for (uint32_t k = 0; k < 8u; k++) { const uint32_t w = base + k; pc[k] = w < totalWords ? (uint32_t)__popc(bitmask[w]) : 0u; sum += pc[k]; }
+    uint32_t incl = sum;
+#pragma unroll
+    for (int o = 1; o < 64; o <<= 1) { const uint32_t t = (uint32_t)__shfl_up((int)incl, o); if ((threadIdx.x & 63u) >= (uint32_t)o) incl += t; }
+    if ((threadIdx.x & 63u) == 63u) waveTotals[threadIdx.x >> 6] = incl;
+    __syncthreads();
+    uint32_t waveBase = 0;
+    blockSum = 0;
+    for (uint32_t k = 0; k < 4u; k++) { if (k < (threadIdx.x >> 6)) waveBase += waveTotals[k]; blockSum += waveTotals[k]; }
+    before = waveBase + incl - sum;
+}
+
 constexpr uint32_t SCAN_CHAIN_BLOCKS = 64;
 __global__ void __launch_bounds__(256) k_scan_chained(const uint32_t* bitmask, uint32_t totalWords, unsigned long long* agg, uint32_t epoch, uint32_t* wordPrefix,
                                                      uint32_t* counters, uint32_t outIndex, uint32_t capacity, uint32_t usedIndex, uint32_t* hostFeedback) {
@@ -1264,16 +1298,8 @@
     __syncthreads();
     const uint32_t block = ticket;
     const uint32_t base = block * SCAN_BLOCK_WORDS + threadIdx.x * 8u;
-    uint32_t pc[8], sum = 0;
-#pragma unroll
-    for (uint32_t k = 0; k < 8u; k++) { const uint32_t w = base + k; pc[k] = w < totalWords ? (uint32_t)__popc(bitmask[w]) : 0u; sum += pc[k]; }
-    uint32_t incl = sum;
-#pragma unroll
-    for (int o = 1; o < 64; o <<= 1) { const uint32_t t = (uint32_t)__shfl_up((int)incl, o); if ((threadIdx.x & 63u) >= (uint32_t)o) incl += t; }
-    if ((threadIdx.x & 63u) == 63u) waveTotals[threadIdx.x >> 6] = incl;
-    __syncthreads();
-    uint32_t waveBase = 0, blockSum = 0;
-    for (uint32_t k = 0; k < 4u; k++) { if (k < (threadIdx.x >> 6)) waveBase += waveTotals[k]; blockSum += waveTotals[k]; }
+    uint32_t pc[8], before, blockSum;
+    scan_block_popcounts(bitmask, totalWords, block, waveTotals, pc, before, blockSum);
     if (threadIdx.x == 0) __hip_atomic_store(&agg[block], ((unsigned long long)epoch << 32) | blockSum, __ATOMIC_RELAXED, __HIP_MEMORY_SCOPE_AGENT);
     if (threadIdx.x < 64u) {
         uint32_t mine = 0;
@@ -1287,7 +1313,7 @@
         if (threadIdx.x == 0) blockPrefix = mine;
     }
     __syncthreads();
-    uint32_t run = blockPrefix + waveBase + incl - sum;
+    uint32_t run = blockPrefix + before;
 #pragma unroll
     for (uint32_t k = 0; k < 8u; k++) { const uint32_t w = base + k; if (w < totalWords) wordPrefix[w] = run; run += pc[k]; }
     if (block == gridDim.x - 1u && threadIdx.x == 0) {
@@ -1307,18 +1333,19 @@
     uint32_t* drawList; HeldRecord* held; uint32_t countAll;
     const MeshletBox* boxes; const uint32_t* pageBoxBase; const float* objConst; uint32_t maxTexels; BoxViewport vp; HzbDesc hzb;
 };
-template <bool LOCAL_RANK, bool HOLD>
-__global__ void __launch_bounds__(256) k_scatter_visible(const TempVisible* temp, uint32_t* counters, uint32_t tempCountIndex, const uint32_t* bitmask,
-                                                        const uint32_t* wordPrefix, uint4* visible, uint32_t baseIndexCounter, uint32_t capacity, uint32_t visibleCapacity,
-                                                        brmi_scene_buffers sc, ClusterSetup* setup, uint32_t resolveCapacity, ClusterUv* clusterUv, LocalRank lr, DrawLists dl) {
+template <int RANK, bool HOLD>
+BRMI_DEV void scatter_visible_block(const TempVisible* temp, uint32_t* counters, uint32_t tempCountIndex, const uint32_t* bitmask,
+                                    const uint32_t* wordPrefix, uint4* visible, uint32_t baseIndexCounter, uint32_t capacity, uint32_t visibleCapacity,
+                                    const brmi_scene_buffers& sc, ClusterSetup* setup, uint32_t resolveCapacity, ClusterUv* clusterUv, const LocalRank& lr, const DrawLists& dl,
+                                    const uint32_t block, const uint32_t nBlocks, const uint32_t* blockSums, const uint32_t scanBlocks) {
     const uint8_t* const* slabs = sc.slabs;
     const uint32_t n = min(counters[tempCountIndex], visibleCapacity);
     const uint32_t base = baseIndexCounter == 0xFFFFFFFFu ? 0u : counters[baseIndexCounter];
     const uint32_t rounded = (n + 63u) & ~63u;
-    __shared__ uint32_t prefixLds[LOCAL_RANK ? LOCAL_RANK_WORDS : 1];
+    __shared__ uint32_t prefixLds[RANK == 1 ? LOCAL_RANK_WORDS : (RANK == 2 ? SCAN_CHAIN_BLOCKS + 1u : 1u)];
     __shared__ uint32_t waveTotals[4];
-    if (LOCAL_RANK) {
-        if (blockIdx.x != 0u && blockIdx.x * blockDim.x >= rounded) return;
+    if (RANK == 1) {
+        if (block != 0u && block * blockDim.x >= rounded) return;
         const uint32_t span = (lr.totalWords + 255u) / 256u;
         const uint32_t w0 = threadIdx.x * span, w1 = min(w0 + span, lr.totalWords);
         uint32_t sum = 0;
@@ -1332,19 +1359,35 @@
         for (uint32_t w = 0; w < 4; w++) { if (w < (threadIdx.x >> 6)) waveBase += waveTotals[w]; all += waveTotals[w]; }
         uint32_t run = waveBase + incl - sum;
         for (uint32_t w = w0; w < w1; w++) { prefixLds[w] = run; run += __popc(bitmask[w]); }
-        if (blockIdx.x == 0u && threadIdx.x == 0u) {
+        if (block == 0u && threadIdx.x == 0u) {
             const uint32_t placed = min(all, capacity - (lr.usedIndex == 0xFFFFFFFFu ? 0u : min(counters[lr.usedIndex], capacity)));
             counters[lr.outIndex] = placed;
             if (lr.hostFeedback) __hip_atomic_store(lr.hostFeedback, placed, __ATOMIC_RELAXED, __HIP_MEMORY_SCOPE_SYSTEM);
         }
         __syncthreads();
     }
+    if (RANK == 2) {
+        if (threadIdx.x < 64u) {
+            const uint32_t v = threadIdx.x < scanBlocks ? blockSums[threadIdx.x] : 0u;
+            uint32_t incl = v;
+#pragma unroll
+            for (int o = 1; o < 64; o <<= 1) { const uint32_t t = (uint32_t)__shfl_up((int)incl, o); if (threadIdx.x >= (uint32_t)o) incl += t; }
+            prefixLds[threadIdx.x] = incl - v;
+            if (threadIdx.x == 63u) prefixLds[SCAN_CHAIN_BLOCKS] = incl;
+        }
+        __syncthreads();
+        if (block == 0u && threadIdx.x == 0u) {
+            const uint32_t placed = min(prefixLds[SCAN_CHAIN_BLOCKS], capacity - (lr.usedIndex == 0xFFFFFFFFu ? 0u : min(counters[lr.usedIndex], capacity)));
+            counters[lr.outIndex] = placed;
+            if (lr.hostFeedback) __hip_atomic_store(lr.hostFeedback, placed, __ATOMIC_RELAXED, __HIP_MEMORY_SCOPE_SYSTEM);
+        }
+    }
     __shared__ unsigned long long blockBase;
     __shared__ uint32_t waveV[4], waveT[4], waveD[4], waveH[4], blockDraw, blockHeld;
     unsigned long long drawnVT = 0ull;
-    if (blockIdx.x == 0u && threadIdx.x == 0u) { const uint32_t room = base < capacity ? capacity - base : 0u; atomicAdd(&counters[CNT_RASTER_CLUSTERS], min(n, room)); if (resolveCapacity == 0u && n != 0u) atomicOr(&counters[CNT_RESOLVE_SPILL], 1u); }
+    if (block == 0u && threadIdx.x == 0u) { const uint32_t room = base < capacity ? capacity - base : 0u; atomicAdd(&counters[CNT_RASTER_CLUSTERS], min(n, room)); if (resolveCapacity == 0u && n != 0u) atomicOr(&counters[CNT_RESOLVE_SPILL], 1u); }
     const uint32_t rounded256 = (n + 255u) & ~255u;
-    for (uint32_t i = blockIdx.x * blockDim.x + threadIdx.x; i < rounded256; i += gridDim.x * blockDim.x) {
+    for (uint32_t i = block * blockDim.x + threadIdx.x; i < rounded256; i += nBlocks * blockDim.x) {
         uint32_t verts = 0, tris = 0, placed = 0, dst = 0;
         TempVisible t{};
         const uint8_t* slab = nullptr; uint32_t pageOff = 0;
@@ -1353,7 +1396,7 @@
         if (i < n) {
             t = temp[i];
             const uint32_t w = t.bit >> 5, b = t.bit & 31u;
-            const uint32_t rank = (LOCAL_RANK ? prefixLds[w] : wordPrefix[w]) + __popc(bitmask[w] & ((1u << b) - 1u));
+            const uint32_t rank = (RANK == 1 ? prefixLds[w] : (RANK == 2 ? prefixLds[w / SCAN_BLOCK_WORDS] + wordPrefix[w] : wordPrefix[w])) + __popc(bitmask[w] & ((1u << b) - 1u));
             dst = base + rank;
             if (dst < capacity) {
                 visible[dst] = t.packed;
@@ -1448,6 +1491,70 @@
     }
 }
 
+template <bool LOCAL_RANK, bool HOLD>
+__global__ void __launch_bounds__(256) k_scatter_visible(const TempVisible* temp, uint32_t* counters, uint32_t tempCountIndex, const uint32_t* bitmask,
+                                                        const uint32_t* wordPrefix, uint4* visible, uint32_t baseIndexCounter, uint32_t capacity, uint32_t visibleCapacity,
+                                                        brmi_scene_buffers sc, ClusterSetup* setup, uint32_t resolveCapacity, ClusterUv* clusterUv, LocalRank lr, DrawLists dl) {
+    scatter_visible_block<LOCAL_RANK ? 1 : 0, HOLD>(temp, counters, tempCountIndex, bitmask, wordPrefix, visible, baseIndexCounter, capacity, visibleCapacity, sc, setup, resolveCapacity, clusterUv, lr, dl,
+                                                    blockIdx.x, gridDim.x, nullptr, 0u);
+}
+
+constexpr uint32_t PHASE2_SMALL_MAX_GRID = 64;
+constexpr uint32_t PHASE2_WAIT_POLLS = 1u << 21;
+struct Phase2Small {
+    unsigned long long* barrier; uint32_t epoch;
+    const uint32_t* meshLevelWidth; NodeRecord* spillOut;
+    BucketRecord* buckets; TempVisible* temp; uint32_t* bitmask; uint8_t* blockDirty;
+    uint32_t totalWords, scanBlocks; uint32_t* wordPrefix; uint32_t* blockSums;
+    uint4* visible; ClusterSetup* setup; uint32_t resolveCapacity; ClusterUv* clusterUv; uint32_t* hostFeedback; uint32_t countAll;
+};
+BRMI_DEV bool phase2_handoff(const Phase2Small& f, uint32_t* counters, uint32_t k) {
+    __shared__ uint32_t arrived;
+    __syncthreads();
+    if (threadIdx.x == 0u) {
+        const unsigned long long start = (unsigned long long)f.epoch << 32;
+        __builtin_amdgcn_fence(__ATOMIC_RELEASE, "agent");
+        if (k == 1u) (void)__hip_atomic_fetch_max(f.barrier, start, __ATOMIC_RELAXED, __HIP_MEMORY_SCOPE_AGENT);
+        (void)__hip_atomic_fetch_add(f.barrier, 1ull, __ATOMIC_RELAXED, __HIP_MEMORY_SCOPE_AGENT);
+        const unsigned long long want = start + (unsigned long long)k * gridDim.x;
+        uint32_t ok = 0u;
+        for (uint32_t poll = 0; poll < PHASE2_WAIT_POLLS; poll++) {
+            const unsigned long long v = __hip_atomic_load(f.barrier, __ATOMIC_RELAXED, __HIP_MEMORY_SCOPE_AGENT);
+            if ((uint32_t)(v >> 32) == f.epoch && v >= want) { ok = 1u; break; }
+            __builtin_amdgcn_s_sleep(2);
+        }
+        if (!ok) atomicAdd(&counters[CNT_DROPPED_WAITS], 1u);
+        arrived = ok;
+    }
+    __syncthreads();
+    __builtin_amdgcn_fence(__ATOMIC_ACQUIRE, "agent");
+    return arrived != 0u;
+}
+__global__ void __launch_bounds__(256) k_phase2_small(CullArgs a, Phase2Small f) {
+    __shared__ HierLds<256, 128> walkLds[4];
+    __shared__ uint32_t waveTotals[4];
+    uint32_t* counters = a.counters;
+    hierarchy_walk<true, 256, 128, true>(a, f.buckets, f.meshLevelWidth, 0u, 256u, 0xFFFFFFFFu, f.spillOut, walkLds[threadIdx.x >> 6], blockIdx.x * 4u + (threadIdx.x >> 6), gridDim.x * 4u, threadIdx.x & 63u);
+    if (!phase2_handoff(f, counters, 1u)) return;
+    cull_clusters_block(a, f.buckets, f.temp, f.bitmask, f.blockDirty, blockIdx.x, gridDim.x);
+    if (!phase2_handoff(f, counters, 2u)) return;
+    for (uint32_t block = blockIdx.x; block < f.scanBlocks; block += gridDim.x) {
+        if (f.blockDirty[block] == 0) { if (threadIdx.x == 0u) f.blockSums[block] = 0u; continue; }
+        uint32_t pc[8], before, blockSum;
+        scan_block_popcounts(f.bitmask, f.totalWords, block, waveTotals, pc, before, blockSum);
+        const uint32_t base = block * SCAN_BLOCK_WORDS + threadIdx.x * 8u;
+        uint32_t run = before;
+#pragma unroll
+        for (uint32_t k = 0; k < 8u; k++) { const uint32_t w = base + k; if (w < f.totalWords) f.wordPrefix[w] = run; run += pc[k]; }
+        if (threadIdx.x == 0u) f.blockSums[block] = blockSum;
+        __syncthreads();
+    }
+    if (!phase2_handoff(f, counters, 3u)) return;
+    scatter_visible_block<2, false>(f.temp, counters, (uint32_t)CNT_TEMP_VISIBLE2, f.bitmask, f.wordPrefix, f.visible, (uint32_t)CNT_VISIBLE, a.visibleCapacity, a.visibleCapacity, a.sc, f.setup, f.resolveCapacity, f.clusterUv,
+                                    LocalRank{f.totalWords, (uint32_t)CNT_VISIBLE2, (uint32_t)CNT_VISIBLE, f.hostFeedback},
+                                    DrawLists{nullptr, nullptr, f.countAll, nullptr, nullptr, nullptr, 0u, BoxViewport{}, HzbDesc{}}, blockIdx.x, gridDim.x, f.blockSums, f.scanBlocks);
+}
+
 static inline uint32_t grid_for(uint64_t items, uint32_t block, uint32_t maxBlocks) {
     uint64_t g = (items + block - 1) / block;
     if (g < 1) g = 1;
@@ -1544,6 +1651,28 @@
         if (!p->phase2Seeded) hipLaunchKernelGGL(k_seed_phase2, dim3(1), dim3(128), 0, s, p->counters(), a.recordCapacity);
         p->phase2Seeded = false;
         const NoSide none{};
+        p->phase2SmallLast = false;
+        if (hierarchy && p->maxLevelWidth <= 256u && !levelKernels && p->scanBlocks <= SCAN_CHAIN_BLOCKS && p->phase2FusedMode != 0) {
+            const volatile uint32_t* hint = reinterpret_cast<volatile uint32_t*>(p->phase2FeedbackHost);
+            const uint32_t lastBuckets = hint ? hint[4] : 0xFFFFFFFFu, lastVisible = hint ? hint[0] : 0xFFFFFFFFu;
+            if (p->phase2FusedMode == 1 || (p->phase2FusedMax != 0u && lastVisible != 0xFFFFFFFFu && lastBuckets <= p->phase2FusedMax && lastVisible <= p->phase2FusedMax)) {
+                if (++p->phase2Epoch == 0u) { BRMI_HIP(p, hipMemsetAsync(p->wsPtr<unsigned long long>(p->ws.phase2Barrier), 0, 8, s)); p->phase2Epoch = 1u; }
+                if (p->phase2DirectMax != 0u) (void)p->ensureFeedback();
+                Phase2Small f;
+                f.barrier = p->wsPtr<unsigned long long>(p->ws.phase2Barrier); f.epoch = p->phase2Epoch;
+                f.meshLevelWidth = meshWidth; f.spillOut = fa;
+                f.buckets = buckets; f.temp = temp; f.bitmask = bitmask; f.blockDirty = blockDirty;
+                f.totalWords = p->totalWords; f.scanBlocks = p->scanBlocks; f.wordPrefix = wordPrefix; f.blockSums = blockSums;
+                f.visible = static_cast<uint4*>(p->res[BRMI_RES_VISIBLE_CLUSTERS]); f.setup = p->wsPtr<ClusterSetup>(p->ws.clusterSetup);
+                f.resolveCapacity = p->inlineResolve ? 0u : p->resolveCapacity;
+                f.clusterUv = (p->sceneHasTextures || p->sceneHasAlphaTest || p->sceneHasVertexColors) ? p->wsPtr<ClusterUv>(p->ws.clusterUv) : nullptr;
+                f.hostFeedback = p->phase2FeedbackDev; f.countAll = p->holdThisFrame ? 1u : 0u;
+                hipLaunchKernelGGL(k_phase2_small, dim3(std::min(std::max(1u, p->phase2FusedGrid), PHASE2_SMALL_MAX_GRID)), dim3(256), 0, s, a, f);
+                BRMI_LAUNCH_CHECK(p, "k_phase2_small");
+                p->phase2SmallLast = true; p->phase2SmallLaunches++;
+                return BRMI_OK;
+            }
+        }
         if (hierarchy && p->maxLevelWidth <= 256u) hipLaunchKernelGGL((k_cull_hierarchy<true, 256, 128>), dim3(2048), dim3(64), 0, s, a, buckets, meshWidth, 0u, 256u, spillAbove, fa, none);
         else if (hierarchy) hipLaunchKernelGGL((k_cull_hierarchy<true, 1024, BRMI_HIER_STAGE_WIDE>), dim3(2048), dim3(64), 0, s, a, buckets, meshWidth, 0u, spillMode ? widthAll : HIER_CAP_MAX, spillAbove, fa, none);
     }
diff --git a/basicrenderer_amd/csrc/brmi_internal.h b/basicrenderer_amd/csrc/brmi_internal.h
--- a/basicrenderer_amd/csrc/brmi_internal.h
+++ b/basicrenderer_amd/csrc/brmi_internal.h
@@ -24,6 +24,7 @@
     CNT_NODES_VISITED,
     CNT_MESHLETS_TESTED,
     CNT_LIGHT_PAGES,
+    CNT_DROPPED_WAITS,
     CNT_SUM_VERTS_LO = 14, CNT_SUM_VERTS_HI,
     CNT_SUM_TRIS_LO, CNT_SUM_TRIS_HI,
     CNT_RASTER_CLUSTERS,
@@ -185,7 +186,7 @@
 
 struct Workspace {
     uint64_t counters, frontierA, frontierB, buckets, tempVisible, bitmask1, bitmask2, blockDirty, chainDirty, wordPrefix, blockSums,
-             instanceBitBase, segPrefix, meshLevelWidth, scanAgg, flatNodes, flatLeaves, instanceWalk, planes, replayNodes, replayBuckets, lightVS, lightMeta, clusterPages, clusterHits, pageTotal, lightHitMasks, binCounts, binRecords, binOverflow, binPlan, binItems, binScratch, clusterSetup, resolveVerts, resolveTris, matWords, shadeTables, lutF, frameConst, objConst, matConst, deferredPixels,
+             instanceBitBase, segPrefix, meshLevelWidth, scanAgg, phase2Barrier, flatNodes, flatLeaves, instanceWalk, planes, replayNodes, replayBuckets, lightVS, lightMeta, clusterPages, clusterHits, pageTotal, lightHitMasks, binCounts, binRecords, binOverflow, binPlan, binItems, binScratch, clusterSetup, resolveVerts, resolveTris, matWords, shadeTables, lutF, frameConst, objConst, matConst, deferredPixels,
              frameSnapshot, clusterUv, binAlpha, overflowAlpha, resolveUVs, resolveColors, alphaMats, shadeRows, shadeAvgs, ggxQuads, shadeLights, clusterList, listEntries, listRecords, layerUniform,
              meshletBoxes, pageBoxBase, pageRefs, drawList, heldRecords, lateList, wideQueue, wideAlpha, generalList, bigQueue, bigRuns, frameClearBytes, total;
 };
@@ -243,6 +244,9 @@
         return true;
     }
     uint32_t phase2DirectMax = 128;
+    uint32_t phase2FusedMax = 16384, phase2FusedGrid = 32; int phase2FusedMode = -1;
+    uint32_t phase2Epoch = 0;
+    bool phase2SmallLast = false; uint32_t phase2SmallLaunches = 0;
     static constexpr uint32_t clearRiderBlocks = 8192;
     bool splitFrame = false;
     uint32_t shadeSlabs = 0; brmi_slab_fn shadeSlabFn = nullptr; void* shadeSlabUser = nullptr;
diff --git a/basicrenderer_amd/renderer.py b/basicrenderer_amd/renderer.py
--- a/basicrenderer_amd/renderer.py
+++ b/basicrenderer_amd/renderer.py
@@ -172,6 +172,11 @@
         self._check(self.lib.brmi_debug_lean_clusters(self._h, out), "brmi_debug_lean_clusters")
         return tuple(int(v) for v in out)
 
+    def phase2_small(self):
+        out = (capi.u32 * 4)()
+        self._check(self.lib.brmi_debug_phase2_small(self._h, out), "brmi_debug_phase2_small")
+        return tuple(int(v) for v in out)
+
     def wide_triangles(self):
         out = (capi.u32 * 3)()
         self._check(self.lib.brmi_debug_wide_triangles(self._h, out), "brmi_debug_wide_triangles")
diff --git a/include/brmi.h b/include/brmi.h
--- a/include/brmi.h
+++ b/include/brmi.h
@@ -127,6 +127,7 @@
     uint32_t lightPagesUsed;
     uint32_t replayNodes, replayMeshlets;
     uint32_t reserved[6];
+    uint32_t droppedWaits;
 } brmi_counters;
 
 enum brmi_stage {
@@ -171,6 +172,7 @@
 
 int brmi_debug_wide_triangles(brmi_pass* pass, uint32_t out[3]);
 int brmi_debug_lean_clusters(brmi_pass* pass, uint32_t out[4]);
+int brmi_debug_phase2_small(brmi_pass* pass, uint32_t out[4]);
 int brmi_debug_read_lean_queue(brmi_pass* pass, uint32_t stripe, uint32_t* runs, uint32_t maxRuns, void* entries, uint32_t maxEntries, uint32_t counts[2]);
 
 int brmi_debug_read_held(brmi_pass* pass, uint32_t* held, uint32_t heldCapacity, uint32_t* heldCount, uint32_t* late, uint32_t lateCapacity, uint32_t* lateCount);
```
